# LuoweiZhou/VLP

Measured on AMD Instinct MI355X. Metric: samples/sec/node (COCO 100-region, seq64, bs64xN) fp16, higher is better.
Workload: dtype f16; 1 GPU; COCO Captions fine-tune shape: BERT-base 12L, 100 regions x 2048-d, seq_len 64 (L=167), bs 64/GPU, fwd+bwd+FP16 FusedAdam, dropout 0.1, dynamic loss scale; global_batch=64, parallelism=dp1, batch_pool=8, skipped_steps=0, rccl_ranks=1, optimizer=replicated, first_leg_packed=False

## Files before the change

include/vlp_hip.h:

```cpp
#ifndef VLP_HIP_H
#define VLP_HIP_H

#include <stdint.h>

#ifdef __cplusplus
extern "C" {
#endif

#define VLP_ABI_VERSION 5

typedef enum {
    VLP_OK = 0,
    VLP_ERR_BAD_ARG = -1,
    VLP_ERR_HIP = -2,
    VLP_ERR_WORKSPACE = -3
} vlp_status;

enum { VLP_ACT_NONE = 0, VLP_ACT_GELU = 1, VLP_ACT_RELU = 2, VLP_ACT_TANH = 3,
       VLP_ACT_GELU_SAVE_GRAD = 4  };
enum { VLP_MUL_NONE = 0, VLP_MUL_GELU_GRAD = 1, VLP_MUL_RELU_MASK = 2, VLP_MUL_PLAIN = 3  };

int vlp_version(void);
const char* vlp_last_error_string(void);
int vlp_lab_build(void);
void vlp_debug_device_lookup_stats(unsigned long long* lookups, unsigned long long* driver_queries);

typedef struct {
    const void* X; int64_t ldx;
    const void* W; int64_t ldw;
    void* Y; int64_t ldy;
    const void* bias;
    const void* residual; int64_t ldr;
    void* preact; int64_t ldp;
    const void* mul_src; int64_t ldm;
    int32_t M, N, K;
    int32_t act;
    int32_t mul_mode;
    float alpha;
    float dropout_p; uint64_t seed; uint32_t rng_stream;
    int32_t variant;
    const int32_t* row_map;
} vlp_gemm_nt_args;
int vlp_gemm_nt(const vlp_gemm_nt_args* a, void* stream);
int vlp_gemm_nt_resolved_variant(void);
int64_t vlp_gemm_nt_splitk_workspace_bytes(int32_t M, int32_t N, int32_t splits);
int vlp_gemm_nt_splitk(const vlp_gemm_nt_args* a, int32_t splits, void* workspace, int64_t workspace_bytes, void* stream);

typedef struct {
    const void* A; int64_t lda;
    const void* B; int64_t ldb;
    void* C; int64_t ldc;
    int32_t M, N, K;
    int32_t beta;
    void* workspace; int64_t workspace_bytes;
    int32_t variant;
    int32_t splits;
    void* bias_out;
} vlp_gemm_tn_args;
int64_t vlp_gemm_tn_workspace_bytes(int32_t M, int32_t N, int32_t K);
int vlp_gemm_tn(const vlp_gemm_tn_args* a, void* stream);
int vlp_gemm_tn_grouped(const vlp_gemm_tn_args* list, int32_t count, void* stream);
int64_t vlp_gemm_tn_grouped_workspace_bytes(int32_t tiles);

typedef struct {
    const void* A; int64_t lda; int32_t M, N;
    void* out;
    int32_t beta;
    void* workspace; int64_t workspace_bytes;
} vlp_colsum_args;
int64_t vlp_colsum_workspace_bytes(int32_t M, int32_t N);
int vlp_colsum(const vlp_colsum_args* a, void* stream);

typedef struct {
    const void* qkv; int64_t ld_qkv;
    const uint8_t* mask;
    void* ctx; int64_t ld_ctx;
    float* lse;
    int32_t B, L, heads;
    float scale;
    float dropout_p; uint64_t seed; uint32_t rng_stream;
    const int32_t* row_off;
} vlp_attn_fwd_args;
int vlp_attn_fwd(const vlp_attn_fwd_args* a, void* stream);

typedef struct {
    const void* q; int64_t ld_q; int64_t q_rows_per_batch;
    const void* k; const void* v; int64_t ld_kv; int64_t kv_rows_per_batch;
    const uint8_t* mask;
    void* ctx; int64_t ld_ctx;
    int32_t B, Lq, Lk, heads;
    float scale;
    const void* k_prefix; const void* v_prefix;
    int64_t prefix_rows_per_batch;
    int32_t n_prefix, beams;
} vlp_attn_decode_args;
int vlp_attn_decode(const vlp_attn_decode_args* a, void* stream);

typedef struct {
    const void* qkv; int64_t ld_qkv;
    const uint8_t* mask;
    const uint8_t* mask_t;
    const void* ctx; int64_t ld_ctx;
    const void* dctx; int64_t ld_dctx;
    const float* lse;
    void* dqkv; int64_t ld_dqkv;
    float* delta;
    int32_t B, L, heads;
    float scale;
    float dropout_p; uint64_t seed; uint32_t rng_stream;
    const int32_t* row_off;
} vlp_attn_bwd_args;
int vlp_attn_bwd(const vlp_attn_bwd_args* a, void* stream);

int vlp_mask_pack(const int64_t* mask, uint8_t* out, uint8_t* out_t, int32_t B, int32_t L, int32_t Lp, void* stream);

typedef struct {
    const void* x; int64_t ldx;
    const void* gamma; const void* beta;
    void* y; int64_t ldy;
    float* mean; float* rstd;
    int32_t M, H; float eps;
    float dropout_p; uint64_t seed; uint32_t rng_stream;
    const int32_t* row_map;
} vlp_layernorm_fwd_args;
int vlp_layernorm_fwd(const vlp_layernorm_fwd_args* a, void* stream);

typedef struct {
    const void* dy; int64_t lddy;
    const void* x; int64_t ldx;
    const void* gamma;
    const float* mean; const float* rstd;
    void* dx; int64_t lddx;
    void* dx_drop; int64_t lddxd;
    void* dgamma; void* dbeta;
    int32_t M, H; int32_t beta;
    float dy_drop_p; uint64_t dy_seed; uint32_t dy_stream;
    float out_drop_p; uint64_t out_seed; uint32_t out_stream;
    void* workspace; int64_t workspace_bytes;
    int32_t defer_reduce;
    const int32_t* row_map;
} vlp_layernorm_bwd_args;
int64_t vlp_layernorm_bwd_workspace_bytes(int32_t H);
int vlp_layernorm_bwd(const vlp_layernorm_bwd_args* a, void* stream);
int vlp_layernorm_bwd_reduce_batched(const float* parts, const void* const* dst, int32_t count, int32_t M, int32_t H, int32_t beta, void* stream);

int vlp_region_mask_build(const int64_t* vis_masked_pos, int32_t B, int32_t Pm, int32_t Nv, uint8_t* out, void* stream);
typedef struct {
    const void* vis_h; const void* vispe_h;
    const void* pooled;
    const int64_t* vis_masked_pos;
    float* probs;
    float* sample_loss;
    float* loss;
    int32_t B, Nv, Pm, H;
} vlp_pretext_fwd_args;
int vlp_pretext_fwd(const vlp_pretext_fwd_args* a, void* stream);
typedef struct {
    const void* vis_h; const void* vispe_h; const void* pooled;
    const int64_t* vis_masked_pos;
    const float* probs;
    const float* gscale;
    void* d_vis_h; void* d_vispe_h;
    void* d_pooled_pre;
    int32_t B, Nv, Pm, H;
    float drop_p; uint64_t seed; uint32_t vis_stream; uint32_t vispe_stream;
} vlp_pretext_bwd_args;
int vlp_pretext_bwd(const vlp_pretext_bwd_args* a, void* stream);

typedef struct {
    const int64_t* input_ids; const int64_t* segment_ids;
    const void* word_emb; const void* pos_emb; const void* type_emb;
    const void* vis_h; const void* vispe_h;
    void* pre;
    int32_t B, L, Nv, H, vocab, type_vocab;
    const int64_t* position_ids;
    int32_t max_pos;
    const uint8_t* region_mask;
    const int32_t* row_map; int32_t rows;
} vlp_embed_fwd_args;
int vlp_embed_fwd(const vlp_embed_fwd_args* a, void* stream);

int64_t vlp_embed_bwd_workspace_floats(int32_t B, int32_t L, int32_t Nv, int32_t H);
typedef struct {
    const void* dpre;
    const int64_t* input_ids; const int64_t* segment_ids;
    const void* vis_h; const void* vispe_h;
    void* d_word_emb; void* d_pos_emb; void* d_type_emb;
    void* d_vis_h; void* d_vispe_h;
    float* acc32;
    int32_t B, L, Nv, H, vocab, type_vocab;
    float drop_p; uint64_t seed; uint32_t vis_stream; uint32_t vispe_stream;
    const uint8_t* region_mask;
    int32_t parts;
} vlp_embed_bwd_args;
int vlp_embed_bwd(const vlp_embed_bwd_args* a, void* stream);
typedef struct {
    vlp_embed_bwd_args base;
    const int64_t* position_ids;
    int32_t max_pos;
} vlp_embed_bwd_pos_args;
int vlp_embed_bwd_pos(const vlp_embed_bwd_pos_args* a, void* stream);

int vlp_copy2d(const void* src, int64_t lds, int32_t src_f32, void* dst, int64_t ldd, int32_t rows,
               int32_t cols_src, int32_t cols_dst, int32_t beta, void* stream);
int vlp_transpose(const void* src, int64_t lds, void* dst, int64_t ldd, int32_t rows, int32_t cols,
                  int32_t rows_pad, void* stream);
typedef struct {
    const void* src; void* dst;
    int64_t lds, ldd;
    int32_t rows, cols, rows_pad, reserved;
} vlp_transpose_desc;
int vlp_transpose_batched(const vlp_transpose_desc* descs_dev, const int32_t* tile_start_dev, int32_t n, int32_t total_tiles, void* stream);
int vlp_gather_rows(const void* src, int64_t lds, const int64_t* pos, void* out, int64_t ldo,
                    int32_t B, int32_t P, int32_t L, int32_t H, const int32_t* row_off, void* stream);
int vlp_scatter_add_rows(const void* src, int64_t lds, const int64_t* pos, void* dst, int64_t ldd,
                         int32_t B, int32_t P, int32_t L, int32_t H, const int32_t* row_off, void* stream);
int vlp_rowmap_build(const int32_t* row_off, int32_t B, int32_t L, int32_t* row_map, void* stream);
int vlp_rows_unpack(const void* src, int64_t lds, const int32_t* row_map, int32_t rows, void* dst, int64_t ldd, int32_t H, void* stream);
int vlp_rows_pack(const void* src, int64_t lds, const int32_t* row_map, int32_t rows, void* dst, int64_t ldd, int32_t H, void* stream);
int vlp_mask_pack_rect(const int64_t* mask, int64_t batch_stride, int64_t row_stride, uint8_t* out, int32_t B, int32_t Lq, int32_t Lk,
                       int32_t Lkp, void* stream);
int vlp_kv_append(const void* qkv_new, int64_t ld, void* cache, int32_t Lcap, int32_t B, int32_t T, int32_t start, int32_t H, void* stream);
int vlp_argmax_rows(const void* logits, int64_t ld, int32_t rows, int32_t V, int64_t* ids, int64_t ids_stride, float* vals, int64_t vals_stride,
                    void* stream);
typedef struct {
    const void* X; int64_t ldx;
    const void* W; int64_t ldw;
    const void* bias;
    void* Y; int64_t ldy;
    float* slab; int64_t ldslab;
    void* kv_cache; int64_t kv_ld;
    int32_t kv_col0, kv_Lcap, kv_T, kv_start;
    int32_t M, N, K, splits;
    int32_t act;
    const void* residual; int64_t ldr;
    const void* ln_gamma; const void* ln_beta; float ln_eps;
    void* ln_out; int64_t ld_ln_out;
} vlp_dec_gemm_args;
int vlp_dec_gemm(const vlp_dec_gemm_args* a, void* stream);
typedef struct {
    const float* slab; int64_t ldslab; int32_t splits;
    const void* bias;
    const void* residual; int64_t ldr;
    const void* gamma; const void* beta;
    float eps;
    void* Y; int64_t ldy;
    int32_t M, H;
} vlp_dec_reduce_ln_args;
int vlp_dec_reduce_ln(const vlp_dec_reduce_ln_args* a, void* stream);
int vlp_argmax_rows2(const void* logits, int64_t ld, int32_t rows, int32_t V, int64_t* ids_a, int64_t ids_a_stride, int64_t* ids_b, int64_t ids_b_stride,
                     float* vals, int64_t vals_stride, void* stream);
int vlp_mask_build(const int32_t* second_st, const int32_t* second_end, const int32_t* is_s2s, uint8_t* out, uint8_t* out_t, int32_t B, int32_t L,
                   int32_t Lp, const uint8_t* region_mask, int32_t Nv, void* stream);
typedef struct {
    const float* bbox;
    const void* cls;
    int64_t ld_cls;
    void* out;
    int64_t ld_out;
    int32_t B, Nv, n_cls, pad_to, cls_is_f32;
    float eps;
} vlp_vis_pe_prep_args;
int vlp_vis_pe_prep(const vlp_vis_pe_prep_args* a, void* stream);
int vlp_sample_rows(const void* logits, int64_t ld, int32_t rows, int32_t V, uint64_t seed, uint32_t rng_stream, int64_t* ids,
                    int64_t ids_stride, float* logp, int64_t logp_stride, void* stream);
typedef struct {
    const int64_t* prefix_ids; const int64_t* sample_ids;
    const int64_t* segment_ids; const int64_t* position_ids; const int64_t* mask;
    int64_t* out_ids; int64_t* out_segment_ids; int64_t* out_position_ids; int64_t* out_mask; int64_t* masked_pos;
    int32_t B, L, in_len, T;
    int64_t mask_word_id;
} vlp_scst_layout_args;
int vlp_scst_layout(const vlp_scst_layout_args* a, void* stream);
int vlp_logsoftmax_topk(const void* logits, int64_t ld, int32_t rows, int32_t V, int32_t K, const uint8_t* forbid, int32_t eos_id,
                        int32_t block_eos, float* out_scores, int64_t* out_ids, void* stream);
typedef struct {
    const float* kk_scores;
    const int64_t* kk_ids;
    const float* last_total;
    const float* last_eos;
    float* out_scores;
    int64_t* out_ids;
    int64_t* out_ptrs;
    float* out_eos;
    int64_t* src_rows;
    int64_t* next_ids;
    int64_t next_ids_stride;
    int32_t B, K, first;
    int64_t eos_id;
} vlp_beam_select_args;
int vlp_beam_select(const vlp_beam_select_args* a, void* stream);
int vlp_ngram_candidates(const int64_t* wids, const int64_t* ptrs, int32_t B, int32_t K, int32_t s, int32_t ngram_size, const int64_t* ignore_ids,
                         int32_t n_ignore, int32_t* cand_ids, int64_t cand_ld, int32_t* cand_cnt, void* stream);
int vlp_logsoftmax_topk_list(const void* logits, int64_t ld, int32_t rows, int32_t V, int32_t K, const int32_t* cand_ids, int64_t cand_ld,
                             const int32_t* cand_cnt, int32_t eos_id, int32_t block_eos, float* out_scores, int64_t* out_ids, void* stream);
int vlp_kv_gather(const void* src, int64_t src_rows_per_batch, void* dst, int64_t dst_rows_per_batch, const int64_t* idx, int32_t R, int32_t lo,
                  int32_t hi, int32_t row_elems, void* stream);
int vlp_vqa_mul_fwd(const void* h, void* out, int32_t B, int32_t L, int32_t Nv, int32_t H, const int32_t* row_off, void* stream);
int vlp_vqa_mul_bwd(const void* h, const void* dout, void* dh, int32_t B, int32_t L, int32_t Nv, int32_t H, const int32_t* row_off, void* stream);
int vlp_relu_dropout_bwd(const void* dy, const void* y, void* dz, int64_t n, int64_t ncols, float drop_p,
                         uint64_t seed, uint32_t rng_stream, void* stream);

int vlp_gelu_bwd(const void* dy, const void* z, void* dz, int64_t n, void* stream);

typedef struct {
    const void* logits; int64_t ld_logits;
    const int64_t* labels;
    const int64_t* weights;
    float* loss;
    float* lse; float* coef;
    float* row_loss;
    int32_t B, P, V;
    float drop_worst_ratio;
} vlp_mlm_loss_fwd_args;
int vlp_mlm_loss_fwd(const vlp_mlm_loss_fwd_args* a, void* stream);
typedef struct {
    const void* logits; int64_t ld_logits;
    const int64_t* labels;
    const float* lse; const float* coef;
    const float* grad_scale;
    void* dlogits; int64_t ld_dlogits;
    int32_t rows, V;
} vlp_mlm_loss_bwd_args;
int vlp_mlm_loss_bwd(const vlp_mlm_loss_bwd_args* a, void* stream);

typedef struct {
    const void* logits; int64_t ld_logits;
    const int64_t* labels;
    const int64_t* weights;
    float* loss;
    float* lse; float* coef;
    float* row_loss;
    int32_t B, P, V;
    float drop_worst_ratio;
    float smooth, confidence, q_sum, q_log_q;
    int32_t ignore_index;
} vlp_mlm_loss_ls_fwd_args;
int vlp_mlm_loss_ls_fwd(const vlp_mlm_loss_ls_fwd_args* a, void* stream);
typedef struct {
    const void* logits; int64_t ld_logits;
    const int64_t* labels;
    const float* lse; const float* coef;
    const float* grad_scale;
    void* dlogits; int64_t ld_dlogits;
    int32_t rows, V;
    float smooth, confidence, q_sum;
    int32_t ignore_index;
} vlp_mlm_loss_ls_bwd_args;
int vlp_mlm_loss_ls_bwd(const vlp_mlm_loss_ls_bwd_args* a, void* stream);

typedef struct {
    const void* logits; int64_t ld_logits;
    const int64_t* ids;
    float* logp; float* lse;
    int32_t rows, V;
} vlp_token_logprob_fwd_args;
int vlp_token_logprob_fwd(const vlp_token_logprob_fwd_args* a, void* stream);
typedef struct {
    const void* logits; int64_t ld_logits;
    const int64_t* ids;
    const float* lse;
    const float* g;
    void* dlogits; int64_t ld_dlogits;
    int32_t rows, V;
} vlp_token_logprob_bwd_args;
int vlp_token_logprob_bwd(const vlp_token_logprob_bwd_args* a, void* stream);

typedef struct {
    const int64_t* hyp; int64_t hyp_ld;
    const int64_t* ref; int64_t ref_group_stride, ref_ld;
    const int32_t* ref_count;
    int32_t G, R, T, mult;
    float sigma;
    float* scores;
    float* reward;
    void* workspace; int64_t workspace_bytes;
} vlp_cider_d_args;
int64_t vlp_cider_d_workspace_bytes(int32_t G, int32_t R, int32_t T, int32_t mult);
int vlp_cider_d(const vlp_cider_d_args* a, void* stream);

typedef struct {
    vlp_cider_d_args s;
    const uint64_t* df_keys;
    const int32_t* df_vals;
    int64_t df_n;
    int64_t n_docs;
} vlp_cider_d_df_args;
int64_t vlp_cider_d_df_workspace_bytes(int32_t G, int32_t R, int32_t T, int32_t mult);
int vlp_cider_d_df(const vlp_cider_d_df_args* a, void* stream);

int vlp_bce_loss_fwd(const void* logits, int64_t ld, const void* labels_f32, int64_t ldl, int32_t B, int32_t N,
                     float* loss, void* stream);
int vlp_bce_loss_bwd(const void* logits, int64_t ld, const void* labels_f32, int64_t ldl, int32_t B, int32_t N,
                     const float* grad_scale, void* dlogits, int64_t ldd, void* stream);
int vlp_bce_sparse_loss_fwd(const void* logits, int64_t ld, const int32_t* ans_idx, const float* ans_score, int32_t S, int32_t B, int32_t N,
                            float* loss, void* stream);
int vlp_bce_sparse_loss_bwd(const void* logits, int64_t ld, const int32_t* ans_idx, const float* ans_score, int32_t S, int32_t B, int32_t N,
                            const float* grad_scale, void* dlogits, int64_t ldd, void* stream);
int vlp_vqa_answer_rows(const void* logits, int64_t ld, int32_t rows, int32_t N, int32_t first_col, const int32_t* ans_idx,
                        const float* ans_score, int32_t S, int64_t* out_ids, float* out_vals, float* out_scores, void* stream);

int vlp_sumsq(const void* g_f16, int64_t n, float* out2, float* partial, void* stream);
int vlp_sumsq_acc(const void* g_f16, int64_t n, float* out2, float* partial, void* stream);

typedef struct {
    float* p32; float* m; float* v;
    const void* g16;
    void* p16;
    int64_t n;
    float b1, b2, eps, decay;
    int32_t eps_inside_sqrt;
    const float* hyper;
} vlp_fused_adam_args;
int vlp_fused_adam(const vlp_fused_adam_args* a, void* stream);
int vlp_adam_hyper(const float* sumsq2, const float* any_overflow, const float* scale_state, float max_grad_norm,
                   float step_size, float* hyper3, void* stream);
int vlp_loss_scale_update(float* scale_state, const float* overflow, void* stream);

int64_t vlp_bert_adam_norms_floats(int64_t n, int32_t ntensors);
typedef struct {
    float* p32; float* m; float* v;
    const void* g; int32_t g_is_f32;
    void* p16;
    const int64_t* seg_off; int32_t ntensors; int64_t n;
    float* norms; int64_t norms_floats;
    float lr, b1, b2, eps, decay, max_grad_norm;
    float grad_scale;
    const int32_t* active;
} vlp_bert_adam_args;
int vlp_bert_adam(const vlp_bert_adam_args* a, void* stream);

#ifdef __cplusplus
}
#endif
#endif
```

vlp_amd/_lib.py:

```python
import ctypes as C
import os

import torch

_HERE = os.path.dirname(os.path.abspath(__file__))
LIB_PATH = os.environ.get("VLP_HIP_LIB") or os.path.join(_HERE, "libvlp_hip.so")

ACT_NONE, ACT_GELU, ACT_RELU, ACT_TANH, ACT_GELU_SAVE_GRAD = 0, 1, 2, 3, 4
MUL_NONE, MUL_GELU_GRAD, MUL_RELU_MASK, MUL_PLAIN = 0, 1, 2, 3

vp, i64, i32, f32, u64, u32 = C.c_void_p, C.c_int64, C.c_int32, C.c_float, C.c_uint64, C.c_uint32


class GemmNtArgs(C.Structure):
    _fields_ = [("X", vp), ("ldx", i64), ("W", vp), ("ldw", i64), ("Y", vp), ("ldy", i64), ("bias", vp),
                ("residual", vp), ("ldr", i64), ("preact", vp), ("ldp", i64), ("mul_src", vp), ("ldm", i64),
                ("M", i32), ("N", i32), ("K", i32), ("act", i32), ("mul_mode", i32), ("alpha", f32),
                ("dropout_p", f32), ("seed", u64), ("rng_stream", u32), ("variant", i32), ("row_map", vp)]


class GemmTnArgs(C.Structure):
    _fields_ = [("A", vp), ("lda", i64), ("B", vp), ("ldb", i64), ("C", vp), ("ldc", i64),
                ("M", i32), ("N", i32), ("K", i32), ("beta", i32), ("workspace", vp), ("workspace_bytes", i64),
                ("variant", i32), ("splits", i32), ("bias_out", vp)]


class ColsumArgs(C.Structure):
    _fields_ = [("A", vp), ("lda", i64), ("M", i32), ("N", i32), ("out", vp), ("beta", i32),
                ("workspace", vp), ("workspace_bytes", i64)]


class AttnFwdArgs(C.Structure):
    _fields_ = [("qkv", vp), ("ld_qkv", i64), ("mask", vp), ("ctx", vp), ("ld_ctx", i64), ("lse", vp),
                ("B", i32), ("L", i32), ("heads", i32), ("scale", f32),
                ("dropout_p", f32), ("seed", u64), ("rng_stream", u32), ("row_off", vp)]


class AttnBwdArgs(C.Structure):
    _fields_ = [("qkv", vp), ("ld_qkv", i64), ("mask", vp), ("mask_t", vp), ("ctx", vp), ("ld_ctx", i64), ("dctx", vp), ("ld_dctx", i64),
                ("lse", vp), ("dqkv", vp), ("ld_dqkv", i64), ("delta", vp),
                ("B", i32), ("L", i32), ("heads", i32), ("scale", f32),
                ("dropout_p", f32), ("seed", u64), ("rng_stream", u32), ("row_off", vp)]


class LayerNormFwdArgs(C.Structure):
    _fields_ = [("x", vp), ("ldx", i64), ("gamma", vp), ("beta", vp), ("y", vp), ("ldy", i64), ("mean", vp), ("rstd", vp),
                ("M", i32), ("H", i32), ("eps", f32), ("dropout_p", f32), ("seed", u64), ("rng_stream", u32), ("row_map", vp)]


class LayerNormBwdArgs(C.Structure):
    _fields_ = [("dy", vp), ("lddy", i64), ("x", vp), ("ldx", i64), ("gamma", vp), ("mean", vp), ("rstd", vp),
                ("dx", vp), ("lddx", i64), ("dx_drop", vp), ("lddxd", i64), ("dgamma", vp), ("dbeta", vp),
                ("M", i32), ("H", i32), ("beta", i32),
                ("dy_drop_p", f32), ("dy_seed", u64), ("dy_stream", u32),
                ("out_drop_p", f32), ("out_seed", u64), ("out_stream", u32),
                ("workspace", vp), ("workspace_bytes", i64), ("defer_reduce", i32), ("row_map", vp)]


class EmbedFwdArgs(C.Structure):
    _fields_ = [("input_ids", vp), ("segment_ids", vp), ("word_emb", vp), ("pos_emb", vp), ("type_emb", vp),
                ("vis_h", vp), ("vispe_h", vp), ("pre", vp),
                ("B", i32), ("L", i32), ("Nv", i32), ("H", i32), ("vocab", i32), ("type_vocab", i32),
                ("position_ids", vp), ("max_pos", i32), ("region_mask", vp), ("row_map", vp), ("rows", i32)]


class AttnDecodeArgs(C.Structure):
    _fields_ = [("q", vp), ("ld_q", i64), ("q_rows_per_batch", i64), ("k", vp), ("v", vp), ("ld_kv", i64), ("kv_rows_per_batch", i64),
                ("mask", vp), ("ctx", vp), ("ld_ctx", i64), ("B", i32), ("Lq", i32), ("Lk", i32), ("heads", i32), ("scale", f32),
                ("k_prefix", vp), ("v_prefix", vp), ("prefix_rows_per_batch", i64), ("n_prefix", i32), ("beams", i32)]


class DecGemmArgs(C.Structure):
    _fields_ = [("X", vp), ("ldx", i64), ("W", vp), ("ldw", i64), ("bias", vp), ("Y", vp), ("ldy", i64), ("slab", vp), ("ldslab", i64),
                ("kv_cache", vp), ("kv_ld", i64), ("kv_col0", i32), ("kv_Lcap", i32), ("kv_T", i32), ("kv_start", i32),
                ("M", i32), ("N", i32), ("K", i32), ("splits", i32), ("act", i32),
                ("residual", vp), ("ldr", i64), ("ln_gamma", vp), ("ln_beta", vp), ("ln_eps", f32), ("ln_out", vp), ("ld_ln_out", i64)]


class DecReduceLnArgs(C.Structure):
    _fields_ = [("slab", vp), ("ldslab", i64), ("splits", i32), ("bias", vp), ("residual", vp), ("ldr", i64), ("gamma", vp), ("beta", vp),
                ("eps", f32), ("Y", vp), ("ldy", i64), ("M", i32), ("H", i32)]


class VisPePrepArgs(C.Structure):
    _fields_ = [("bbox", vp), ("cls", vp), ("ld_cls", i64), ("out", vp), ("ld_out", i64), ("B", i32), ("Nv", i32), ("n_cls", i32),
                ("pad_to", i32), ("cls_is_f32", i32), ("eps", f32)]


class BeamSelectArgs(C.Structure):
    _fields_ = [("kk_scores", vp), ("kk_ids", vp), ("last_total", vp), ("last_eos", vp), ("out_scores", vp), ("out_ids", vp),
                ("out_ptrs", vp), ("out_eos", vp), ("src_rows", vp), ("next_ids", vp), ("next_ids_stride", i64),
                ("B", i32), ("K", i32), ("first", i32), ("eos_id", i64)]


class EmbedBwdArgs(C.Structure):
    _fields_ = [("dpre", vp), ("input_ids", vp), ("segment_ids", vp), ("vis_h", vp), ("vispe_h", vp),
                ("d_word_emb", vp), ("d_pos_emb", vp), ("d_type_emb", vp), ("d_vis_h", vp), ("d_vispe_h", vp), ("acc32", vp),
                ("B", i32), ("L", i32), ("Nv", i32), ("H", i32), ("vocab", i32), ("type_vocab", i32),
                ("drop_p", f32), ("seed", u64), ("vis_stream", u32), ("vispe_stream", u32), ("region_mask", vp), ("parts", i32)]


class EmbedBwdPosArgs(C.Structure):
    _fields_ = [("base", EmbedBwdArgs), ("position_ids", vp), ("max_pos", i32)]


class ScstLayoutArgs(C.Structure):
    _fields_ = [("prefix_ids", vp), ("sample_ids", vp), ("segment_ids", vp), ("position_ids", vp), ("mask", vp),
                ("out_ids", vp), ("out_segment_ids", vp), ("out_position_ids", vp), ("out_mask", vp), ("masked_pos", vp),
                ("B", i32), ("L", i32), ("in_len", i32), ("T", i32), ("mask_word_id", i64)]


class TokenLogprobFwdArgs(C.Structure):
    _fields_ = [("logits", vp), ("ld_logits", i64), ("ids", vp), ("logp", vp), ("lse", vp), ("rows", i32), ("V", i32)]


class TokenLogprobBwdArgs(C.Structure):
    _fields_ = [("logits", vp), ("ld_logits", i64), ("ids", vp), ("lse", vp), ("g", vp), ("dlogits", vp), ("ld_dlogits", i64),
                ("rows", i32), ("V", i32)]


class PretextFwdArgs(C.Structure):
    _fields_ = [("vis_h", vp), ("vispe_h", vp), ("pooled", vp), ("vis_masked_pos", vp), ("probs", vp), ("sample_loss", vp), ("loss", vp),
                ("B", i32), ("Nv", i32), ("Pm", i32), ("H", i32)]


class PretextBwdArgs(C.Structure):
    _fields_ = [("vis_h", vp), ("vispe_h", vp), ("pooled", vp), ("vis_masked_pos", vp), ("probs", vp), ("gscale", vp),
                ("d_vis_h", vp), ("d_vispe_h", vp), ("d_pooled_pre", vp), ("B", i32), ("Nv", i32), ("Pm", i32), ("H", i32),
                ("drop_p", f32), ("seed", u64), ("vis_stream", u32), ("vispe_stream", u32)]


class TransposeDesc(C.Structure):
    _fields_ = [("src", vp), ("dst", vp), ("lds", i64), ("ldd", i64), ("rows", i32), ("cols", i32), ("rows_pad", i32), ("reserved", i32)]


class CiderDArgs(C.Structure):
    _fields_ = [("hyp", vp), ("hyp_ld", i64), ("ref", vp), ("ref_group_stride", i64), ("ref_ld", i64), ("ref_count", vp),
                ("G", i32), ("R", i32), ("T", i32), ("mult", i32), ("sigma", f32), ("scores", vp), ("reward", vp),
                ("workspace", vp), ("workspace_bytes", i64)]


class CiderDDfArgs(C.Structure):
    _fields_ = [("s", CiderDArgs), ("df_keys", vp), ("df_vals", vp), ("df_n", i64), ("n_docs", i64)]


class MlmLossFwdArgs(C.Structure):
    _fields_ = [("logits", vp), ("ld_logits", i64), ("labels", vp), ("weights", vp), ("loss", vp), ("lse", vp), ("coef", vp),
                ("row_loss", vp), ("B", i32), ("P", i32), ("V", i32), ("drop_worst_ratio", f32)]


class MlmLossBwdArgs(C.Structure):
    _fields_ = [("logits", vp), ("ld_logits", i64), ("labels", vp), ("lse", vp), ("coef", vp), ("grad_scale", vp),
                ("dlogits", vp), ("ld_dlogits", i64), ("rows", i32), ("V", i32)]


class MlmLossLsFwdArgs(C.Structure):
    _fields_ = MlmLossFwdArgs._fields_ + [("smooth", f32), ("confidence", f32), ("q_sum", f32), ("q_log_q", f32), ("ignore_index", i32)]


class MlmLossLsBwdArgs(C.Structure):
    _fields_ = MlmLossBwdArgs._fields_ + [("smooth", f32), ("confidence", f32), ("q_sum", f32), ("ignore_index", i32)]


class FusedAdamArgs(C.Structure):
    _fields_ = [("p32", vp), ("m", vp), ("v", vp), ("g16", vp), ("p16", vp), ("n", i64),
                ("b1", f32), ("b2", f32), ("eps", f32), ("decay", f32), ("eps_inside_sqrt", i32), ("hyper", vp)]


class BertAdamArgs(C.Structure):
    _fields_ = [("p32", vp), ("m", vp), ("v", vp), ("g", vp), ("g_is_f32", i32), ("p16", vp),
                ("seg_off", vp), ("ntensors", i32), ("n", i64), ("norms", vp), ("norms_floats", i64),
                ("lr", f32), ("b1", f32), ("b2", f32), ("eps", f32), ("decay", f32), ("max_grad_norm", f32), ("grad_scale", f32),
                ("active", vp)]


SYMBOLS = {
    "vlp_version": (C.c_int, []),
    "vlp_last_error_string": (C.c_char_p, []),
    "vlp_lab_build": (C.c_int, []),
    "vlp_debug_device_lookup_stats": (None, [vp, vp]),
    "vlp_gemm_nt": (C.c_int, [C.POINTER(GemmNtArgs), vp]),
    "vlp_gemm_nt_resolved_variant": (C.c_int, []),
    "vlp_gemm_nt_splitk_workspace_bytes": (C.c_int64, [i32, i32, i32]),
    "vlp_gemm_nt_splitk": (C.c_int, [C.POINTER(GemmNtArgs), i32, vp, i64, vp]),
    "vlp_gemm_tn_workspace_bytes": (i64, [i32, i32, i32]),
    "vlp_gemm_tn": (C.c_int, [C.POINTER(GemmTnArgs), vp]),
    "vlp_gemm_tn_grouped": (C.c_int, [C.POINTER(GemmTnArgs), i32, vp]),
    "vlp_gemm_tn_grouped_workspace_bytes": (i64, [i32]),
    "vlp_colsum_workspace_bytes": (i64, [i32, i32]),
    "vlp_colsum": (C.c_int, [C.POINTER(ColsumArgs), vp]),
    "vlp_attn_fwd": (C.c_int, [C.POINTER(AttnFwdArgs), vp]),
    "vlp_attn_bwd": (C.c_int, [C.POINTER(AttnBwdArgs), vp]),
    "vlp_attn_decode": (C.c_int, [C.POINTER(AttnDecodeArgs), vp]),
    "vlp_mask_pack_rect": (C.c_int, [vp, i64, i64, vp, i32, i32, i32, i32, vp]),
    "vlp_kv_append": (C.c_int, [vp, i64, vp, i32, i32, i32, i32, i32, vp]),
    "vlp_dec_gemm": (C.c_int, [C.POINTER(DecGemmArgs), vp]),
    "vlp_dec_reduce_ln": (C.c_int, [C.POINTER(DecReduceLnArgs), vp]),
    "vlp_argmax_rows2": (C.c_int, [vp, i64, i32, i32, vp, i64, vp, i64, vp, i64, vp]),
    "vlp_logsoftmax_topk": (C.c_int, [vp, i64, i32, i32, i32, vp, i32, i32, vp, vp, vp]),
    "vlp_beam_select": (C.c_int, [C.POINTER(BeamSelectArgs), vp]),
    "vlp_ngram_candidates": (C.c_int, [vp, vp, i32, i32, i32, i32, vp, i32, vp, i64, vp, vp]),
    "vlp_logsoftmax_topk_list": (C.c_int, [vp, i64, i32, i32, i32, vp, i64, vp, i32, i32, vp, vp, vp]),
    "vlp_kv_gather": (C.c_int, [vp, i64, vp, i64, vp, i32, i32, i32, i32, vp]),
    "vlp_embed_bwd_workspace_floats": (C.c_int64, [i32, i32, i32, i32]),
    "vlp_mask_build": (C.c_int, [vp, vp, vp, vp, vp, i32, i32, i32, vp, i32, vp]),
    "vlp_vis_pe_prep": (C.c_int, [C.POINTER(VisPePrepArgs), vp]),
    "vlp_sample_rows": (C.c_int, [vp, i64, i32, i32, C.c_uint64, C.c_uint32, vp, i64, vp, i64, vp]),
    "vlp_argmax_rows": (C.c_int, [vp, i64, i32, i32, vp, i64, vp, i64, vp]),
    "vlp_mask_pack": (C.c_int, [vp, vp, vp, i32, i32, i32, vp]),
    "vlp_layernorm_fwd": (C.c_int, [C.POINTER(LayerNormFwdArgs), vp]),
    "vlp_layernorm_bwd_workspace_bytes": (i64, [i32]),
    "vlp_layernorm_bwd": (C.c_int, [C.POINTER(LayerNormBwdArgs), vp]),
    "vlp_layernorm_bwd_reduce_batched": (C.c_int, [vp, vp, i32, i32, i32, i32, vp]),
    "vlp_embed_fwd": (C.c_int, [C.POINTER(EmbedFwdArgs), vp]),
    "vlp_embed_bwd": (C.c_int, [C.POINTER(EmbedBwdArgs), vp]),
    "vlp_embed_bwd_pos": (C.c_int, [C.POINTER(EmbedBwdPosArgs), vp]),
    "vlp_scst_layout": (C.c_int, [C.POINTER(ScstLayoutArgs), vp]),
    "vlp_token_logprob_fwd": (C.c_int, [C.POINTER(TokenLogprobFwdArgs), vp]),
    "vlp_token_logprob_bwd": (C.c_int, [C.POINTER(TokenLogprobBwdArgs), vp]),
    "vlp_region_mask_build": (C.c_int, [vp, i32, i32, i32, vp, vp]),
    "vlp_pretext_fwd": (C.c_int, [C.POINTER(PretextFwdArgs), vp]),
    "vlp_pretext_bwd": (C.c_int, [C.POINTER(PretextBwdArgs), vp]),
    "vlp_copy2d": (C.c_int, [vp, i64, i32, vp, i64, i32, i32, i32, i32, vp]),
    "vlp_transpose": (C.c_int, [vp, i64, vp, i64, i32, i32, i32, vp]),
    "vlp_transpose_batched": (C.c_int, [vp, vp, i32, i32, vp]),
    "vlp_gather_rows": (C.c_int, [vp, i64, vp, vp, i64, i32, i32, i32, i32, vp, vp]),
    "vlp_scatter_add_rows": (C.c_int, [vp, i64, vp, vp, i64, i32, i32, i32, i32, vp, vp]),
    "vlp_rowmap_build": (C.c_int, [vp, i32, i32, vp, vp]),
    "vlp_rows_unpack": (C.c_int, [vp, i64, vp, i32, vp, i64, i32, vp]),
    "vlp_rows_pack": (C.c_int, [vp, i64, vp, i32, vp, i64, i32, vp]),
    "vlp_vqa_mul_fwd": (C.c_int, [vp, vp, i32, i32, i32, i32, vp, vp]),
    "vlp_vqa_mul_bwd": (C.c_int, [vp, vp, vp, i32, i32, i32, i32, vp, vp]),
    "vlp_relu_dropout_bwd": (C.c_int, [vp, vp, vp, i64, i64, f32, u64, u32, vp]),
    "vlp_gelu_bwd": (C.c_int, [vp, vp, vp, i64, vp]),
    "vlp_cider_d_workspace_bytes": (i64, [i32, i32, i32, i32]),
    "vlp_cider_d": (C.c_int, [C.POINTER(CiderDArgs), vp]),
    "vlp_cider_d_df_workspace_bytes": (i64, [i32, i32, i32, i32]),
    "vlp_cider_d_df": (C.c_int, [C.POINTER(CiderDDfArgs), vp]),
    "vlp_mlm_loss_fwd": (C.c_int, [C.POINTER(MlmLossFwdArgs), vp]),
    "vlp_mlm_loss_bwd": (C.c_int, [C.POINTER(MlmLossBwdArgs), vp]),
    "vlp_mlm_loss_ls_fwd": (C.c_int, [C.POINTER(MlmLossLsFwdArgs), vp]),
    "vlp_mlm_loss_ls_bwd": (C.c_int, [C.POINTER(MlmLossLsBwdArgs), vp]),
    "vlp_bce_loss_fwd": (C.c_int, [vp, i64, vp, i64, i32, i32, vp, vp]),
    "vlp_bce_loss_bwd": (C.c_int, [vp, i64, vp, i64, i32, i32, vp, vp, i64, vp]),
    "vlp_bce_sparse_loss_fwd": (C.c_int, [vp, i64, vp, vp, i32, i32, i32, vp, vp]),
    "vlp_bce_sparse_loss_bwd": (C.c_int, [vp, i64, vp, vp, i32, i32, i32, vp, vp, i64, vp]),
    "vlp_vqa_answer_rows": (C.c_int, [vp, i64, i32, i32, i32, vp, vp, i32, vp, vp, vp, vp]),
    "vlp_sumsq": (C.c_int, [vp, i64, vp, vp, vp]),
    "vlp_sumsq_acc": (C.c_int, [vp, i64, vp, vp, vp]),
    "vlp_fused_adam": (C.c_int, [C.POINTER(FusedAdamArgs), vp]),
    "vlp_adam_hyper": (C.c_int, [vp, vp, vp, f32, f32, vp, vp]),
    "vlp_loss_scale_update": (C.c_int, [vp, vp, vp]),
    "vlp_bert_adam": (C.c_int, [C.POINTER(BertAdamArgs), vp]),
    "vlp_bert_adam_norms_floats": (i64, [i64, i32]),
}

_lib = None


_recording = None


class _Recorder(object):

    def __init__(self, lib, plan):
        self._lib, self._plan = lib, plan

    def __getattr__(self, name):
        fn = getattr(self._lib, name)

        def call(*args):
            self._plan.append((fn, args))
            return fn(*args)
        return call


class record(object):

    def __enter__(self):
        global _recording
        if _recording is not None:
            raise RuntimeError("vlp_amd._lib.record(): already recording")
        self.plan = []
        _recording = _Recorder(load(), self.plan)
        return self.plan

    def __exit__(self, *exc):
        global _recording
        _recording = None
        return False


def replay(plan):
    for fn, args in plan:
        rc = fn(*args)
        if rc:
            _check(rc)


def load():
    global _lib
    if _recording is not None:
        return _recording
    if _lib is not None:
        return _lib
    if not os.path.exists(LIB_PATH):
        raise RuntimeError("libvlp_hip.so not found at %s -- run `python -m vlp_amd.build` (or "
                           "__graft_entry__.build()).  vlp_amd has no CPU / torch fallback." % LIB_PATH)
    lib = C.CDLL(LIB_PATH)
    for name, (res, args) in SYMBOLS.items():
        fn = getattr(lib, name)
        fn.restype = res
        fn.argtypes = args
    if lib.vlp_version() != 5:
        raise RuntimeError("libvlp_hip.so ABI version mismatch")
    _lib = lib
    return lib


def lab_build():
    return bool(load().vlp_lab_build())


def _check(rc):
    if rc != 0:
        lib = _lib if _lib is not None else load()
        raise RuntimeError("libvlp_hip: %s (status %d)" % (lib.vlp_last_error_string().decode(), rc))


def stream_ptr():
    return C.c_void_p(torch.cuda.current_stream().cuda_stream)


def ptr(t):
    return None if t is None else C.c_void_p(t.data_ptr())


def _nbytes(t):
    return 0 if t is None else t.numel() * t.element_size()


def _req_cuda(*ts):
    for t in ts:
        if t is not None and not t.is_cuda:
            raise RuntimeError("vlp_amd kernels need device tensors (got a CPU tensor); there is no CPU fallback")


def _gemm_nt_args(x, w, y, M, N, K, ldx, ldw, ldy, bias, residual, ldr, preact, ldp, mul_src, ldm, act, mul_mode, alpha, dropout_p, seed, rng_stream,
                  variant=0, row_map=None):
    return GemmNtArgs(ptr(x), ldx if ldx is not None else x.stride(0), ptr(w), ldw if ldw is not None else w.stride(0),
                      ptr(y), ldy if ldy is not None else y.stride(0), ptr(bias),
                      ptr(residual), (ldr if ldr is not None else (residual.stride(0) if residual is not None else 0)),
                      ptr(preact), (ldp if ldp is not None else (preact.stride(0) if preact is not None else 0)),
                      ptr(mul_src), (ldm if ldm is not None else (mul_src.stride(0) if mul_src is not None else 0)),
                      M, N, K, act, mul_mode, alpha, dropout_p, seed, rng_stream, variant, ptr(row_map))


def gemm_nt(x, w, y, M, N, K, ldx=None, ldw=None, ldy=None, bias=None, residual=None, ldr=None, preact=None, ldp=None,
            mul_src=None, ldm=None, act=ACT_NONE, mul_mode=MUL_NONE, alpha=1.0, dropout_p=0.0, seed=0, rng_stream=0,
            variant=0, row_map=None):
    _req_cuda(x, w, y, row_map)
    a = _gemm_nt_args(x, w, y, M, N, K, ldx, ldw, ldy, bias, residual, ldr, preact, ldp, mul_src, ldm, act, mul_mode, alpha, dropout_p, seed,
                      rng_stream, variant, row_map)
    _check(load().vlp_gemm_nt(C.byref(a), stream_ptr()))


def gemm_nt_resolved_variant():
    return int(load().vlp_gemm_nt_resolved_variant())


def gemm_nt_splitk_workspace_bytes(M, N, splits):
    return int(load().vlp_gemm_nt_splitk_workspace_bytes(M, N, splits))


def gemm_nt_splitk(x, w, y, M, N, K, splits, workspace, ldx=None, ldw=None, ldy=None, bias=None, residual=None, ldr=None, preact=None, ldp=None,
                   mul_src=None, ldm=None, act=ACT_NONE, mul_mode=MUL_NONE, alpha=1.0, dropout_p=0.0, seed=0, rng_stream=0):
    _req_cuda(x, w, y, workspace)
    a = _gemm_nt_args(x, w, y, M, N, K, ldx, ldw, ldy, bias, residual, ldr, preact, ldp, mul_src, ldm, act, mul_mode, alpha, dropout_p, seed,
                      rng_stream)
    _check(load().vlp_gemm_nt_splitk(C.byref(a), splits, ptr(workspace), _nbytes(workspace), stream_ptr()))


def gemm_tn_workspace_bytes(M, N, K):
    return int(load().vlp_gemm_tn_workspace_bytes(M, N, K))


def gemm_tn(a_, b_, c_, M, N, K, lda=None, ldb=None, ldc=None, beta=0, workspace=None, variant=0, splits=0, bias_out=None):
    _req_cuda(a_, b_, c_)
    a = GemmTnArgs(ptr(a_), lda if lda is not None else a_.stride(0), ptr(b_), ldb if ldb is not None else b_.stride(0),
                   ptr(c_), ldc if ldc is not None else c_.stride(0), M, N, K, beta,
                   ptr(workspace), _nbytes(workspace), variant, splits,
                   ptr(bias_out))
    _check(load().vlp_gemm_tn(C.byref(a), stream_ptr()))


def gemm_tn_grouped_workspace_bytes(tiles):
    return int(load().vlp_gemm_tn_grouped_workspace_bytes(tiles))


def gemm_tn_grouped(problems, workspace=None):
    arr = (GemmTnArgs * len(problems))()
    for i, (a_, b_, c_, M, N, K, beta, bias_out) in enumerate(problems):
        _req_cuda(a_, b_, c_, bias_out)
        w = workspace if i == 0 else None
        if w is not None:
            _req_cuda(w)
        arr[i] = GemmTnArgs(ptr(a_), a_.stride(0), ptr(b_), b_.stride(0), ptr(c_), c_.stride(0), M, N, K, beta, ptr(w),
                            _nbytes(w), 0, 0, ptr(bias_out))
    _check(load().vlp_gemm_tn_grouped(arr, len(problems), stream_ptr()))


def colsum_workspace_bytes(M, N):
    return int(load().vlp_colsum_workspace_bytes(M, N))


def colsum(a_, out, M, N, lda=None, beta=0, workspace=None):
    _req_cuda(a_, out)
    a = ColsumArgs(ptr(a_), lda if lda is not None else a_.stride(0), M, N, ptr(out), beta, ptr(workspace),
                   _nbytes(workspace))
    _check(load().vlp_colsum(C.byref(a), stream_ptr()))


def attn_fwd(qkv, mask, ctx, lse, B, L, heads, scale, dropout_p=0.0, seed=0, rng_stream=0, row_off=None):
    _req_cuda(qkv, mask, ctx, lse, row_off)
    a = AttnFwdArgs(ptr(qkv), qkv.stride(0), ptr(mask), ptr(ctx), ctx.stride(0), ptr(lse), B, L, heads, scale, dropout_p, seed, rng_stream,
                    ptr(row_off))
    _check(load().vlp_attn_fwd(C.byref(a), stream_ptr()))


def attn_bwd(qkv, mask, mask_t, ctx, dctx, lse, dqkv, delta, B, L, heads, scale, dropout_p=0.0, seed=0, rng_stream=0, row_off=None):
    _req_cuda(qkv, mask, mask_t, ctx, dctx, lse, dqkv, delta, row_off)
    a = AttnBwdArgs(ptr(qkv), qkv.stride(0), ptr(mask), ptr(mask_t), ptr(ctx), ctx.stride(0), ptr(dctx), dctx.stride(0), ptr(lse),
                    ptr(dqkv), dqkv.stride(0), ptr(delta), B, L, heads, scale, dropout_p, seed, rng_stream, ptr(row_off))
    _check(load().vlp_attn_bwd(C.byref(a), stream_ptr()))


def attn_decode(q, ld_q, q_rows, k, v, ld_kv, kv_rows, mask, ctx, B, Lq, Lk, heads, scale, k_prefix=None, v_prefix=None, prefix_rows=0,
                n_prefix=0, beams=1):
    _req_cuda(q, k, v, mask, ctx, k_prefix, v_prefix)
    a = AttnDecodeArgs(ptr(q), ld_q, q_rows, ptr(k), ptr(v), ld_kv, kv_rows, ptr(mask), ptr(ctx), ctx.stride(0), B, Lq, Lk, heads, scale,
                       ptr(k_prefix), ptr(v_prefix), prefix_rows, n_prefix, beams)
    _check(load().vlp_attn_decode(C.byref(a), stream_ptr()))


def dec_gemm(x, w, M, N, Kd, y=None, bias=None, act=0, slab=None, splits=1, kv_cache=None, kv_col0=0, kv_Lcap=0, kv_T=1, kv_start=0,
             residual=None, ln_gamma=None, ln_beta=None, ln_eps=1e-5, ln_out=None):
    _req_cuda(x, w, y, bias, slab, kv_cache, residual, ln_gamma, ln_beta, ln_out)
    a = DecGemmArgs(ptr(x), x.stride(0), ptr(w), w.stride(0), ptr(bias), ptr(y), y.stride(0) if y is not None else 0,
                    ptr(slab), slab.stride(1) if slab is not None else 0, ptr(kv_cache), kv_cache.stride(1) if kv_cache is not None else 0,
                    kv_col0, kv_Lcap, kv_T, kv_start, M, N, Kd, splits, act,
                    ptr(residual), residual.stride(0) if residual is not None else 0, ptr(ln_gamma), ptr(ln_beta), ln_eps,
                    ptr(ln_out), ln_out.stride(0) if ln_out is not None else 0)
    _check(load().vlp_dec_gemm(C.byref(a), stream_ptr()))


def dec_reduce_ln(slab, splits, bias, residual, gamma, beta, y, M, H, eps=1e-5):
    _req_cuda(slab, bias, residual, gamma, beta, y)
    a = DecReduceLnArgs(ptr(slab), slab.stride(1), splits, ptr(bias), ptr(residual), residual.stride(0) if residual is not None else 0,
                        ptr(gamma), ptr(beta), eps, ptr(y), y.stride(0), M, H)
    _check(load().vlp_dec_reduce_ln(C.byref(a), stream_ptr()))


def argmax_rows2(logits, ld, rows, V, ids_a, ids_b, vals):
    _req_cuda(logits, ids_a, ids_b, vals)
    _check(load().vlp_argmax_rows2(ptr(logits), ld, rows, V, ptr(ids_a), ids_a.stride(0), ptr(ids_b), ids_b.stride(0) if ids_b is not None else 0,
                                   ptr(vals), vals.stride(0), stream_ptr()))


def mask_pack_rect(mask_view, out_u8, B, Lq, Lk, Lkp):
    _req_cuda(mask_view, out_u8)
    assert mask_view.stride(2) == 1 and mask_view.dtype == torch.int64
    _check(load().vlp_mask_pack_rect(ptr(mask_view), mask_view.stride(0), mask_view.stride(1), ptr(out_u8), B, Lq, Lk, Lkp, stream_ptr()))


def kv_append(qkv_new, ld, cache, Lcap, B, T, start, H):
    _req_cuda(qkv_new, cache)
    _check(load().vlp_kv_append(ptr(qkv_new), ld, ptr(cache), Lcap, B, T, start, H, stream_ptr()))


def argmax_rows(logits, ld, rows, V, ids, vals):
    _req_cuda(logits, ids, vals)
    _check(load().vlp_argmax_rows(ptr(logits), ld, rows, V, ptr(ids), ids.stride(0), ptr(vals), vals.stride(0), stream_ptr()))


def logsoftmax_topk(logits, ld, rows, V, K, out_scores, out_ids, forbid=None, eos_id=0, block_eos=False):
    _req_cuda(logits, out_scores, out_ids, forbid)
    _check(load().vlp_logsoftmax_topk(ptr(logits), ld, rows, V, K, ptr(forbid), eos_id, 1 if block_eos else 0, ptr(out_scores), ptr(out_ids),
                                      stream_ptr()))


def ngram_candidates(wids, ptrs, B, K, s, ngram_size, cand_ids, cand_cnt, ignore_ids=None):
    _req_cuda(wids, ptrs, cand_ids, cand_cnt, ignore_ids)
    assert wids.dtype == torch.int64 and ptrs.dtype == torch.int64 and wids.is_contiguous() and ptrs.is_contiguous()
    assert tuple(wids.shape[1:]) == (B, K) and tuple(ptrs.shape[1:]) == (B, K) and s < wids.shape[0] and s < ptrs.shape[0]
    assert cand_ids.dtype == torch.int32 and cand_cnt.dtype == torch.int32 and cand_ids.stride(1) == 1 and cand_cnt.is_contiguous()
    assert cand_ids.shape[0] >= B * K and cand_cnt.numel() >= B * K
    n_ignore = 0
    if ignore_ids is not None:
        assert ignore_ids.dtype == torch.int64 and ignore_ids.is_contiguous()
        n_ignore = ignore_ids.numel()
    _check(load().vlp_ngram_candidates(ptr(wids), ptr(ptrs), B, K, s, ngram_size, ptr(ignore_ids) if n_ignore else None, n_ignore, ptr(cand_ids),
                                       cand_ids.stride(0), ptr(cand_cnt), stream_ptr()))


def logsoftmax_topk_list(logits, ld, rows, V, K, out_scores, out_ids, cand_ids, cand_cnt, eos_id=0, block_eos=False):
    _req_cuda(logits, out_scores, out_ids, cand_ids, cand_cnt)
    assert cand_ids.dtype == torch.int32 and cand_cnt.dtype == torch.int32 and cand_ids.stride(1) == 1 and cand_cnt.is_contiguous()
    assert cand_ids.shape[0] >= rows and cand_cnt.numel() >= rows
    _check(load().vlp_logsoftmax_topk_list(ptr(logits), ld, rows, V, K, ptr(cand_ids), cand_ids.stride(0), ptr(cand_cnt), eos_id, 1 if block_eos else 0,
                                           ptr(out_scores), ptr(out_ids), stream_ptr()))


def beam_select(kk_scores, kk_ids, last_total, last_eos, out_scores, out_ids, out_ptrs, out_eos, src_rows, next_ids, B, K, first, eos_id):
    _req_cuda(kk_scores, kk_ids, last_total, last_eos, out_scores, out_ids, out_ptrs, out_eos, src_rows, next_ids)
    a = BeamSelectArgs(ptr(kk_scores), ptr(kk_ids), ptr(last_total), ptr(last_eos), ptr(out_scores), ptr(out_ids), ptr(out_ptrs), ptr(out_eos),
                       ptr(src_rows), ptr(next_ids), next_ids.stride(0), B, K, 1 if first else 0, eos_id)
    _check(load().vlp_beam_select(C.byref(a), stream_ptr()))


def kv_gather(src, src_rows, dst, dst_rows, idx, R, lo, hi, row_elems):
    _req_cuda(src, dst, idx)
    _check(load().vlp_kv_gather(ptr(src), src_rows, ptr(dst), dst_rows, ptr(idx), R, lo, hi, row_elems, stream_ptr()))


def mask_build(second_st, second_end, is_s2s, out_u8, B, L, Lp, out_t=None, region_mask=None, Nv=0):
    _req_cuda(second_st, second_end, is_s2s, out_u8, out_t, region_mask)
    for t in (second_st, second_end, is_s2s):
        assert t.dtype == torch.int32 and t.is_contiguous() and t.numel() == B
    _check(load().vlp_mask_build(ptr(second_st), ptr(second_end), ptr(is_s2s), ptr(out_u8), ptr(out_t), B, L, Lp, ptr(region_mask), Nv, stream_ptr()))


def vis_pe_prep(bbox, cls, out, B, Nv, n_cls, pad_to, eps=1e-5):
    _req_cuda(bbox, cls, out)
    assert bbox.dtype == torch.float32 and bbox.is_contiguous() and cls.dtype in (torch.float16, torch.float32) and cls.stride(-1) == 1
    a = VisPePrepArgs(ptr(bbox), ptr(cls), cls.stride(0), ptr(out), out.stride(0), B, Nv, n_cls, pad_to, 1 if cls.dtype == torch.float32 else 0, eps)
    _check(load().vlp_vis_pe_prep(C.byref(a), stream_ptr()))


def sample_rows(logits, ld, rows, V, seed, rng_stream, ids, logp):
    _req_cuda(logits, ids, logp)
    _check(load().vlp_sample_rows(ptr(logits), ld, rows, V, seed, rng_stream, ptr(ids), ids.stride(0), ptr(logp), logp.stride(0), stream_ptr()))


def mask_pack(mask_i64, out_u8, B, L, Lp, out_t=None):
    _req_cuda(mask_i64, out_u8, out_t)
    _check(load().vlp_mask_pack(ptr(mask_i64), ptr(out_u8), ptr(out_t), B, L, Lp, stream_ptr()))


def layernorm_fwd(x, gamma, beta, y, M, H, mean=None, rstd=None, eps=1e-5, dropout_p=0.0, seed=0, rng_stream=0, ldx=None, ldy=None, row_map=None):
    _req_cuda(x, gamma, beta, y, row_map)
    a = LayerNormFwdArgs(ptr(x), ldx if ldx is not None else x.stride(0), ptr(gamma), ptr(beta), ptr(y),
                         ldy if ldy is not None else y.stride(0), ptr(mean), ptr(rstd), M, H, eps, dropout_p, seed, rng_stream, ptr(row_map))
    _check(load().vlp_layernorm_fwd(C.byref(a), stream_ptr()))


def layernorm_bwd_workspace_bytes(H):
    return int(load().vlp_layernorm_bwd_workspace_bytes(H))


def layernorm_bwd(dy, x, gamma, mean, rstd, dx, dgamma, dbeta, M, H, workspace, beta=0, dx_drop=None,
                  dy_drop=(0.0, 0, 0), out_drop=(0.0, 0, 0), defer_reduce=False, row_map=None):
    _req_cuda(dy, x, gamma, mean, rstd, dx, dgamma, dbeta, workspace, row_map)
    a = LayerNormBwdArgs(ptr(dy), dy.stride(0), ptr(x), x.stride(0), ptr(gamma), ptr(mean), ptr(rstd), ptr(dx), dx.stride(0),
                         ptr(dx_drop), dx_drop.stride(0) if dx_drop is not None else 0, ptr(dgamma), ptr(dbeta), M, H, beta,
                         dy_drop[0], dy_drop[1], dy_drop[2], out_drop[0], out_drop[1], out_drop[2],
                         ptr(workspace), _nbytes(workspace), 1 if defer_reduce else 0, ptr(row_map))
    _check(load().vlp_layernorm_bwd(C.byref(a), stream_ptr()))


def layernorm_bwd_reduce_batched(parts, dst_table, count, M, H, beta=0):
    _req_cuda(parts, dst_table)
    _check(load().vlp_layernorm_bwd_reduce_batched(ptr(parts), ptr(dst_table), count, M, H, beta, stream_ptr()))


def embed_fwd(input_ids, segment_ids, word_emb, pos_emb, type_emb, vis_h, vispe_h, pre, B, L, Nv, H, position_ids=None, region_mask=None,
              row_map=None, rows=0):
    _req_cuda(input_ids, segment_ids, word_emb, pos_emb, type_emb, pre, position_ids, region_mask, row_map)
    a = EmbedFwdArgs(ptr(input_ids), ptr(segment_ids), ptr(word_emb), ptr(pos_emb), ptr(type_emb), ptr(vis_h), ptr(vispe_h),
                     ptr(pre), B, L, Nv, H, word_emb.shape[0], type_emb.shape[0], ptr(position_ids), pos_emb.shape[0], ptr(region_mask),
                     ptr(row_map), rows)
    _check(load().vlp_embed_fwd(C.byref(a), stream_ptr()))


def embed_bwd_workspace_floats(B, L, Nv, H):
    return int(load().vlp_embed_bwd_workspace_floats(B, L, Nv, H))


def _embed_bwd_args(dpre, input_ids, segment_ids, vis_h, vispe_h, d_word, d_pos, d_type, d_vis_h, d_vispe_h, acc32,
                    B, L, Nv, H, vocab, type_vocab, drop_p, seed, vis_stream, vispe_stream, region_mask, parts):
    _req_cuda(dpre, input_ids, segment_ids, d_word, d_pos, d_type, acc32, region_mask)
    return EmbedBwdArgs(ptr(dpre), ptr(input_ids), ptr(segment_ids), ptr(vis_h), ptr(vispe_h), ptr(d_word), ptr(d_pos), ptr(d_type),
                        ptr(d_vis_h), ptr(d_vispe_h), ptr(acc32), B, L, Nv, H, vocab, type_vocab, drop_p, seed, vis_stream, vispe_stream,
                        ptr(region_mask), parts)


def embed_bwd(dpre, input_ids, segment_ids, vis_h, vispe_h, d_word, d_pos, d_type, d_vis_h, d_vispe_h, acc32,
              B, L, Nv, H, vocab, type_vocab, drop_p=0.0, seed=0, vis_stream=0, vispe_stream=0, region_mask=None, parts=0):
    a = _embed_bwd_args(dpre, input_ids, segment_ids, vis_h, vispe_h, d_word, d_pos, d_type, d_vis_h, d_vispe_h, acc32,
                        B, L, Nv, H, vocab, type_vocab, drop_p, seed, vis_stream, vispe_stream, region_mask, parts)
    _check(load().vlp_embed_bwd(C.byref(a), stream_ptr()))


def embed_bwd_pos(dpre, input_ids, segment_ids, position_ids, vis_h, vispe_h, d_word, d_pos, d_type, d_vis_h, d_vispe_h, acc32,
                  B, L, Nv, H, vocab, type_vocab, drop_p=0.0, seed=0, vis_stream=0, vispe_stream=0, region_mask=None, parts=0):
    _req_cuda(position_ids)
    base = _embed_bwd_args(dpre, input_ids, segment_ids, vis_h, vispe_h, d_word, d_pos, d_type, d_vis_h, d_vispe_h, acc32,
                           B, L, Nv, H, vocab, type_vocab, drop_p, seed, vis_stream, vispe_stream, region_mask, parts)
    a = EmbedBwdPosArgs(base, ptr(position_ids), d_pos.shape[0])
    _check(load().vlp_embed_bwd_pos(C.byref(a), stream_ptr()))


def scst_layout(prefix_ids, sample_ids, segment_ids, position_ids, mask, out_ids, out_segment_ids, out_position_ids, out_mask, masked_pos,
                mask_word_id):
    _req_cuda(prefix_ids, sample_ids, segment_ids, position_ids, mask, out_ids, out_segment_ids, out_position_ids, out_mask, masked_pos)
    B, in_len = prefix_ids.shape
    T, L = sample_ids.shape[1], segment_ids.shape[1]
    for t in (prefix_ids, sample_ids, segment_ids, position_ids, mask, out_ids, out_segment_ids, out_position_ids, out_mask, masked_pos):
        if t.dtype != torch.long or not t.is_contiguous():
            raise RuntimeError("vlp_amd.scst_layout: operands must be contiguous int64")
    Lo = in_len + 2 * T - 1
    if (tuple(sample_ids.shape) != (B, T) or tuple(position_ids.shape) != (B, L) or tuple(mask.shape) != (B, L, L) or
            tuple(out_ids.shape) != (B, Lo) or tuple(out_segment_ids.shape) != (B, Lo) or tuple(out_position_ids.shape) != (B, Lo) or
            tuple(out_mask.shape) != (B, Lo, Lo) or tuple(masked_pos.shape) != (B, T)):
        raise RuntimeError("vlp_amd.scst_layout: shape mismatch")
    a = ScstLayoutArgs(ptr(prefix_ids), ptr(sample_ids), ptr(segment_ids), ptr(position_ids), ptr(mask), ptr(out_ids), ptr(out_segment_ids),
                       ptr(out_position_ids), ptr(out_mask), ptr(masked_pos), B, L, in_len, T, int(mask_word_id))
    _check(load().vlp_scst_layout(C.byref(a), stream_ptr()))


def token_logprob_fwd(logits, ld, ids, logp, lse, rows, V):
    _req_cuda(logits, ids, logp, lse)
    a = TokenLogprobFwdArgs(ptr(logits), ld, ptr(ids), ptr(logp), ptr(lse), rows, V)
    _check(load().vlp_token_logprob_fwd(C.byref(a), stream_ptr()))


def token_logprob_bwd(logits, ld, ids, lse, g, dlogits, ldd, rows, V):
    _req_cuda(logits, ids, lse, g, dlogits)
    a = TokenLogprobBwdArgs(ptr(logits), ld, ptr(ids), ptr(lse), ptr(g), ptr(dlogits), ldd, rows, V)
    _check(load().vlp_token_logprob_bwd(C.byref(a), stream_ptr()))


def cider_d_workspace_bytes(G, R, T, mult):
    return int(load().vlp_cider_d_workspace_bytes(G, R, T, mult))


def cider_d(hyp, ref, ref_count, mult, scores, reward=None, sigma=6.0, workspace=None):
    a = _cider_d_args(hyp, ref, ref_count, mult, scores, reward, sigma, workspace, cider_d_workspace_bytes)
    _check(load().vlp_cider_d(C.byref(a), stream_ptr()))


def _cider_d_args(hyp, ref, ref_count, mult, scores, reward, sigma, workspace, workspace_bytes):
    _req_cuda(hyp, ref, ref_count, scores, reward, workspace)
    if hyp.dtype != torch.int64 or ref.dtype != torch.int64 or hyp.dim() != 2 or ref.dim() != 3 or hyp.stride(1) != 1 or ref.stride(2) != 1:
        raise RuntimeError("vlp_amd.cider_d: hyp int64 [mult*G, T] and ref int64 [G, R, T] with contiguous rows")
    G, R, T = ref.shape
    if hyp.shape[0] != mult * G or hyp.shape[1] != T:
        raise RuntimeError("vlp_amd.cider_d: hyp must be [%d, %d]" % (mult * G, T))
    if ref_count is not None and (ref_count.dtype != torch.int32 or not ref_count.is_contiguous() or ref_count.numel() != G):
        raise RuntimeError("vlp_amd.cider_d: ref_count must be contiguous int32 [%d]" % G)
    if scores.dtype != torch.float32 or not scores.is_contiguous() or scores.numel() < mult * G:
        raise RuntimeError("vlp_amd.cider_d: scores must be contiguous f32 [%d]" % (mult * G))
    if reward is not None and (reward.dtype != torch.float32 or not reward.is_contiguous() or reward.numel() < G):
        raise RuntimeError("vlp_amd.cider_d: reward must be contiguous f32 [%d]" % G)
    if workspace is None:
        workspace = torch.empty(max(workspace_bytes(G, R, T, mult), 1), device=hyp.device, dtype=torch.uint8)
    a = CiderDArgs(ptr(hyp), hyp.stride(0), ptr(ref), ref.stride(0), ref.stride(1), ptr(ref_count), G, R, T, mult, sigma, ptr(scores), ptr(reward),
                   ptr(workspace), _nbytes(workspace))
    a._keep = workspace
    return a


def cider_d_df_workspace_bytes(G, R, T, mult):
    return int(load().vlp_cider_d_df_workspace_bytes(G, R, T, mult))


def cider_d_df(hyp, ref, ref_count, mult, scores, df_keys, df_vals, n_docs, reward=None, sigma=6.0, workspace=None):
    _req_cuda(df_keys, df_vals)
    if (df_keys.dtype not in (torch.int64, torch.uint64) or df_vals.dtype != torch.int32 or df_keys.dim() != 1 or df_vals.dim() != 1
            or not df_keys.is_contiguous() or not df_vals.is_contiguous() or df_keys.numel() != df_vals.numel()):
        raise RuntimeError("vlp_amd.cider_d_df: df_keys int64 [N] (the uint64 keys' bits) and df_vals int32 [N], contiguous")
    s = _cider_d_args(hyp, ref, ref_count, mult, scores, reward, sigma, workspace, cider_d_df_workspace_bytes)
    n = df_keys.numel()
    a = CiderDDfArgs(s, ptr(df_keys) if n else None, ptr(df_vals) if n else None, n, int(n_docs))
    _check(load().vlp_cider_d_df(C.byref(a), stream_ptr()))


def region_mask_build(vis_masked_pos, out, B, Pm, Nv):
    _req_cuda(vis_masked_pos, out)
    _check(load().vlp_region_mask_build(ptr(vis_masked_pos), B, Pm, Nv, ptr(out), stream_ptr()))


def pretext_fwd(vis_h, vispe_h, pooled, vis_masked_pos, probs, sample_loss, loss, B, Nv, Pm, H):
    _req_cuda(vis_h, vispe_h, pooled, vis_masked_pos, probs, sample_loss, loss)
    a = PretextFwdArgs(ptr(vis_h), ptr(vispe_h), ptr(pooled), ptr(vis_masked_pos), ptr(probs), ptr(sample_loss), ptr(loss), B, Nv, Pm, H)
    _check(load().vlp_pretext_fwd(C.byref(a), stream_ptr()))


def pretext_bwd(vis_h, vispe_h, pooled, vis_masked_pos, probs, gscale, d_vis_h, d_vispe_h, d_pooled_pre, B, Nv, Pm, H,
                drop_p=0.0, seed=0, vis_stream=0, vispe_stream=0):
    _req_cuda(vis_h, vispe_h, pooled, vis_masked_pos, probs, gscale, d_vis_h, d_vispe_h, d_pooled_pre)
    a = PretextBwdArgs(ptr(vis_h), ptr(vispe_h), ptr(pooled), ptr(vis_masked_pos), ptr(probs), ptr(gscale), ptr(d_vis_h), ptr(d_vispe_h),
                       ptr(d_pooled_pre), B, Nv, Pm, H, drop_p, seed, vis_stream, vispe_stream)
    _check(load().vlp_pretext_bwd(C.byref(a), stream_ptr()))


def copy2d(src, lds, src_f32, dst, ldd, rows, cols_src, cols_dst, beta=0):
    _req_cuda(src, dst)
    _check(load().vlp_copy2d(ptr(src), lds, int(src_f32), ptr(dst), ldd, rows, cols_src, cols_dst, beta, stream_ptr()))


def transpose(src, lds, dst, ldd, rows, cols, rows_pad):
    _req_cuda(src, dst)
    _check(load().vlp_transpose(ptr(src), lds, ptr(dst), ldd, rows, cols, rows_pad, stream_ptr()))


def make_transpose_batch(items, device):
    import numpy as np
    arr = (TransposeDesc * len(items))()
    starts, tot = [], 0
    for i, (src, lds, dst, ldd, rows, cols, rows_pad) in enumerate(items):
        _req_cuda(src, dst)
        arr[i] = TransposeDesc(src.data_ptr(), dst.data_ptr(), lds, ldd, rows, cols, rows_pad, 0)
        starts.append(tot)
        tot += ((rows_pad + 63) // 64) * ((cols + 63) // 64)
    raw = np.frombuffer(bytes(arr), dtype=np.uint8).copy()
    descs = torch.from_numpy(raw).to(device)
    ts = torch.tensor(starts, dtype=torch.int32, device=device)
    return descs, ts, len(items), tot


def transpose_batched(batch):
    descs, ts, n, tot = batch
    _check(load().vlp_transpose_batched(ptr(descs), ptr(ts), n, tot, stream_ptr()))


def gather_rows(src, lds, pos, out, ldo, B, P, L, H, row_off=None):
    _req_cuda(src, pos, out, row_off)
    _check(load().vlp_gather_rows(ptr(src), lds, ptr(pos), ptr(out), ldo, B, P, L, H, ptr(row_off), stream_ptr()))


def scatter_add_rows(src, lds, pos, dst, ldd, B, P, L, H, row_off=None):
    _req_cuda(src, pos, dst, row_off)
    _check(load().vlp_scatter_add_rows(ptr(src), lds, ptr(pos), ptr(dst), ldd, B, P, L, H, ptr(row_off), stream_ptr()))


def rowmap_build(row_off, B, L, row_map):
    _req_cuda(row_off, row_map)
    _check(load().vlp_rowmap_build(ptr(row_off), B, L, ptr(row_map), stream_ptr()))


def rows_unpack(src, row_map, rows, dst, H):
    _req_cuda(src, row_map, dst)
    _check(load().vlp_rows_unpack(ptr(src), src.stride(0), ptr(row_map), rows, ptr(dst), dst.stride(0), H, stream_ptr()))


def rows_pack(src, row_map, rows, dst, H):
    _req_cuda(src, row_map, dst)
    _check(load().vlp_rows_pack(ptr(src), src.stride(0), ptr(row_map), rows, ptr(dst), dst.stride(0), H, stream_ptr()))


def vqa_mul_fwd(h, out, B, L, Nv, H, row_off=None):
    _req_cuda(h, out, row_off)
    _check(load().vlp_vqa_mul_fwd(ptr(h), ptr(out), B, L, Nv, H, ptr(row_off), stream_ptr()))


def vqa_mul_bwd(h, dout, dh, B, L, Nv, H, row_off=None):
    _req_cuda(h, dout, dh, row_off)
    _check(load().vlp_vqa_mul_bwd(ptr(h), ptr(dout), ptr(dh), B, L, Nv, H, ptr(row_off), stream_ptr()))


def relu_dropout_bwd(dy, y, dz, n, ncols, drop_p=0.0, seed=0, rng_stream=0):
    _req_cuda(dy, y, dz)
    _check(load().vlp_relu_dropout_bwd(ptr(dy), ptr(y), ptr(dz), n, ncols, drop_p, seed, rng_stream, stream_ptr()))


def gelu_bwd(dy, z, dz, n):
    _req_cuda(dy, z, dz)
    _check(load().vlp_gelu_bwd(ptr(dy), ptr(z), ptr(dz), n, stream_ptr()))


def mlm_loss_fwd(logits, ld, labels, weights, loss, lse, coef, row_loss, B, P, V, drop_worst_ratio=0.0):
    _req_cuda(logits, labels, weights, loss, lse, coef, row_loss)
    a = MlmLossFwdArgs(ptr(logits), ld, ptr(labels), ptr(weights), ptr(loss), ptr(lse), ptr(coef), ptr(row_loss), B, P, V, drop_worst_ratio)
    _check(load().vlp_mlm_loss_fwd(C.byref(a), stream_ptr()))


def mlm_loss_bwd(logits, ld, labels, lse, coef, grad_scale, dlogits, ldd, rows, V):
    _req_cuda(logits, labels, lse, coef, grad_scale, dlogits)
    a = MlmLossBwdArgs(ptr(logits), ld, ptr(labels), ptr(lse), ptr(coef), ptr(grad_scale), ptr(dlogits), ldd, rows, V)
    _check(load().vlp_mlm_loss_bwd(C.byref(a), stream_ptr()))


def mlm_loss_ls_fwd(logits, ld, labels, weights, loss, lse, coef, row_loss, B, P, V, smooth, confidence, q_sum, q_log_q, ignore_index=0,
                    drop_worst_ratio=0.0):
    _req_cuda(logits, labels, weights, loss, lse, coef, row_loss)
    a = MlmLossLsFwdArgs(ptr(logits), ld, ptr(labels), ptr(weights), ptr(loss), ptr(lse), ptr(coef), ptr(row_loss), B, P, V, drop_worst_ratio,
                         smooth, confidence, q_sum, q_log_q, ignore_index)
    _check(load().vlp_mlm_loss_ls_fwd(C.byref(a), stream_ptr()))


def mlm_loss_ls_bwd(logits, ld, labels, lse, coef, grad_scale, dlogits, ldd, rows, V, smooth, confidence, q_sum, ignore_index=0):
    _req_cuda(logits, labels, lse, coef, grad_scale, dlogits)
    a = MlmLossLsBwdArgs(ptr(logits), ld, ptr(labels), ptr(lse), ptr(coef), ptr(grad_scale), ptr(dlogits), ldd, rows, V,
                         smooth, confidence, q_sum, ignore_index)
    _check(load().vlp_mlm_loss_ls_bwd(C.byref(a), stream_ptr()))


def bce_loss_fwd(logits, ld, labels, ldl, B, N, loss257):
    _req_cuda(logits, labels, loss257)
    _check(load().vlp_bce_loss_fwd(ptr(logits), ld, ptr(labels), ldl, B, N, ptr(loss257), stream_ptr()))


def bce_loss_bwd(logits, ld, labels, ldl, B, N, grad_scale, dlogits, ldd):
    _req_cuda(logits, labels, grad_scale, dlogits)
    _check(load().vlp_bce_loss_bwd(ptr(logits), ld, ptr(labels), ldl, B, N, ptr(grad_scale), ptr(dlogits), ldd, stream_ptr()))


def _req_answers(ans_idx, ans_score, B):
    _req_cuda(ans_idx, ans_score)
    if ans_idx.dtype != torch.int32 or ans_score.dtype != torch.float32 or ans_idx.dim() != 2 or ans_idx.shape != ans_score.shape \
            or ans_idx.shape[0] != B or not (ans_idx.is_contiguous() and ans_score.is_contiguous()):
        raise RuntimeError("vlp_amd: sparse answers must be contiguous idx int32 / score f32 [%d, S]" % B)
    return ans_idx.shape[1]


def bce_sparse_loss_fwd(logits, ld, ans_idx, ans_score, B, N, loss257):
    _req_cuda(logits, loss257)
    S = _req_answers(ans_idx, ans_score, B)
    _check(load().vlp_bce_sparse_loss_fwd(ptr(logits), ld, ptr(ans_idx), ptr(ans_score), S, B, N, ptr(loss257), stream_ptr()))


def bce_sparse_loss_bwd(logits, ld, ans_idx, ans_score, B, N, grad_scale, dlogits, ldd):
    _req_cuda(logits, grad_scale, dlogits)
    S = _req_answers(ans_idx, ans_score, B)
    _check(load().vlp_bce_sparse_loss_bwd(ptr(logits), ld, ptr(ans_idx), ptr(ans_score), S, B, N, ptr(grad_scale), ptr(dlogits), ldd, stream_ptr()))


def vqa_answer_rows(logits, ld, rows, N, first_col, out_ids, out_vals, ans_idx=None, ans_score=None, out_scores=None):
    _req_cuda(logits, out_ids, out_vals)
    if out_ids.dtype != torch.int64 or out_vals.dtype != torch.float32 or out_ids.numel() < rows or out_vals.numel() < rows \
            or not (out_ids.is_contiguous() and out_vals.is_contiguous()):
        raise RuntimeError("vlp_amd: vqa_answer_rows needs contiguous out_ids int64 [rows] and out_vals f32 [rows]")
    S = 0
    if ans_idx is not None:
        S = _req_answers(ans_idx, ans_score, rows)
        _req_cuda(out_scores)
        if out_scores.dtype != torch.float32 or out_scores.numel() < rows or not out_scores.is_contiguous():
            raise RuntimeError("vlp_amd: vqa_answer_rows needs contiguous out_scores f32 [rows]")
    _check(load().vlp_vqa_answer_rows(ptr(logits), ld, rows, N, first_col, ptr(ans_idx), ptr(ans_score) if ans_idx is not None else None, S,
                                      ptr(out_ids), ptr(out_vals), ptr(out_scores) if ans_idx is not None else None, stream_ptr()))


def sumsq(g16, n, out2, partial, accumulate=False):
    _req_cuda(g16, out2, partial)
    fn = load().vlp_sumsq_acc if accumulate else load().vlp_sumsq
    _check(fn(ptr(g16), n, ptr(out2), ptr(partial), stream_ptr()))


def adam_hyper(sumsq2, any_overflow, scale_state, max_grad_norm, step_size, hyper3):
    _req_cuda(sumsq2, hyper3, scale_state)
    _check(load().vlp_adam_hyper(ptr(sumsq2), ptr(any_overflow), ptr(scale_state), max_grad_norm, step_size, ptr(hyper3), stream_ptr()))


def loss_scale_update(scale_state, overflow):
    _req_cuda(scale_state, overflow)
    _check(load().vlp_loss_scale_update(ptr(scale_state), ptr(overflow), stream_ptr()))


def fused_adam(p32, m, v, g16, p16, n, hyper, b1=0.9, b2=0.999, eps=1e-8, decay=0.0, eps_inside_sqrt=False):
    _req_cuda(p32, m, v, g16, p16, hyper)
    a = FusedAdamArgs(ptr(p32), ptr(m), ptr(v), ptr(g16), ptr(p16), n, b1, b2, eps, decay, int(eps_inside_sqrt), ptr(hyper))
    _check(load().vlp_fused_adam(C.byref(a), stream_ptr()))


def bert_adam_norms_floats(n, ntensors):
    return int(load().vlp_bert_adam_norms_floats(n, ntensors))


def bert_adam(p32, m, v, g, g_is_f32, p16, seg_off, ntensors, n, norms, lr, b1=0.9, b2=0.999, eps=1e-6, decay=0.01,
              max_grad_norm=1.0, grad_scale=1.0, active=None):
    _req_cuda(p32, m, v, g, seg_off, norms)
    a = BertAdamArgs(ptr(p32), ptr(m), ptr(v), ptr(g), int(g_is_f32), ptr(p16), ptr(seg_off), ntensors, n, ptr(norms), norms.numel(),
                     lr, b1, b2, eps, decay, max_grad_norm, grad_scale, ptr(active))
    _check(load().vlp_bert_adam(C.byref(a), stream_ptr()))
```

vlp_amd/csrc/adam.hip:

```cpp
#include "common.h"
#include <stdlib.h>

#define SQ_BLOCKS 1024

__global__ __launch_bounds__(256) void sumsq_kernel(const f16* __restrict__ g, int64_t n, float* __restrict__ partial) {
    __shared__ float sh[4], shb[4];
    float s = 0.f, bad = 0.f;
    const int64_t n8 = n >> 3;
    for (int64_t i = (int64_t)blockIdx.x * blockDim.x + threadIdx.x; i < n8; i += (int64_t)gridDim.x * blockDim.x) {
        f16x8 v = ld8(g + i * 8);
#pragma unroll
        for (int e = 0; e < 8; ++e) {
            const float f = (float)v[e];
            s += f * f;
            if (!(fabsf(f) <= 65504.f)) bad = 1.f;
        }
    }
    if (blockIdx.x == 0)
        for (int64_t i = n8 * 8 + threadIdx.x; i < n; i += blockDim.x) {
            const float f = (float)g[i];
            s += f * f;
            if (!(fabsf(f) <= 65504.f)) bad = 1.f;
        }
    s = wave_sum(s);
    bad = wave_max(bad);
    const int w = threadIdx.x >> 6, l = threadIdx.x & 63;
    if (l == 0) { sh[w] = s; shb[w] = bad; }
    __syncthreads();
    if (threadIdx.x == 0) {
        partial[blockIdx.x] = sh[0] + sh[1] + sh[2] + sh[3];
        partial[SQ_BLOCKS + blockIdx.x] = fmaxf(fmaxf(shb[0], shb[1]), fmaxf(shb[2], shb[3]));
    }
}
__global__ __launch_bounds__(256) void sumsq_finish_kernel(const float* __restrict__ partial, int nblocks, float* __restrict__ out2, int accumulate) {
    __shared__ float sh[4], shb[4];
    float s = 0.f, bad = 0.f;
    for (int i = threadIdx.x; i < nblocks; i += blockDim.x) { s += partial[i]; bad = fmaxf(bad, partial[SQ_BLOCKS + i]); }
    s = wave_sum(s);
    bad = wave_max(bad);
    const int w = threadIdx.x >> 6, l = threadIdx.x & 63;
    if (l == 0) { sh[w] = s; shb[w] = bad; }
    __syncthreads();
    if (threadIdx.x == 0) {
        const float tot = sh[0] + sh[1] + sh[2] + sh[3];
        float b = fmaxf(fmaxf(shb[0], shb[1]), fmaxf(shb[2], shb[3]));
        if (!(tot <= 3.0e38f)) b = 1.f;
        out2[0] = accumulate ? out2[0] + tot : tot;
        out2[1] = accumulate ? fmaxf(out2[1], b) : b;
    }
}
static int sumsq_launch(const void* g, int64_t n, float* out2, float* partial, int accumulate, void* stream);
extern "C" int vlp_sumsq(const void* g, int64_t n, float* out2, float* partial, void* stream) { return sumsq_launch(g, n, out2, partial, 0, stream); }
extern "C" int vlp_sumsq_acc(const void* g, int64_t n, float* out2, float* partial, void* stream) { return sumsq_launch(g, n, out2, partial, 1, stream); }
static int sumsq_launch(const void* g, int64_t n, float* out2, float* partial, int accumulate, void* stream) {
    VLP_CHECK_ARG(g && out2 && partial && n > 0 && (uintptr_t)g % 16 == 0, "vlp_sumsq: bad args (partial must hold 2048 floats)");
    VLP_ENTER(g, "vlp_sumsq");
    int blocks = (int)((n / 8 + 255) / 256);
    if (blocks > SQ_BLOCKS) blocks = SQ_BLOCKS;
    if (blocks < 1) blocks = 1;
    hipStream_t s = (hipStream_t)stream;
    hipLaunchKernelGGL(sumsq_kernel, dim3(blocks), dim3(256), 0, s, (const f16*)g, n, partial);
    VLP_CHECK_LAUNCH("vlp_sumsq");
    hipLaunchKernelGGL(sumsq_finish_kernel, dim3(1), dim3(256), 0, s, partial, blocks, out2, accumulate);
    VLP_CHECK_LAUNCH("vlp_sumsq(finish)");
    return VLP_OK;
}

__global__ void adam_hyper_kernel(const float* sumsq2, const float* any_overflow, const float* scale_state, float max_grad_norm, float step_size,
                                  float* hyper) {
    if (threadIdx.x != 0 || blockIdx.x != 0) return;
    const float scale = scale_state[0];
    float overflow = sumsq2[1];
    if (any_overflow) overflow = fmaxf(overflow, any_overflow[0]);
    const float norm = sqrtf(sumsq2[0]);
    float combined = scale;
    if (max_grad_norm > 0.f) {
        const float clip = (norm / scale + 1e-6f) / max_grad_norm;
        if (clip > 1.f) combined = clip * scale;
    }
    hyper[0] = combined;
    hyper[1] = step_size;
    hyper[2] = overflow;
}
extern "C" int vlp_adam_hyper(const float* sumsq2, const float* any_overflow, const float* scale_state, float max_grad_norm, float step_size,
                              float* hyper3, void* stream) {
    VLP_CHECK_ARG(sumsq2 && hyper3 && scale_state, "vlp_adam_hyper: bad args");
    VLP_ENTER(sumsq2, "vlp_adam_hyper");
    hipLaunchKernelGGL(adam_hyper_kernel, dim3(1), dim3(64), 0, (hipStream_t)stream, sumsq2, any_overflow, scale_state, max_grad_norm, step_size, hyper3);
    VLP_CHECK_LAUNCH("vlp_adam_hyper");
    return VLP_OK;
}

__global__ void loss_scale_update_kernel(float* st, const float* overflow) {
    if (threadIdx.x != 0 || blockIdx.x != 0) return;
    const bool skip = overflow[0] != 0.f;
    if (st[5] != 0.f) {
        if (skip) {
            st[0] = fmaxf(st[0] / st[3], 1.f);
            st[2] = st[1];
        } else if (fmodf(st[1] - st[2], st[4]) == 0.f) {
            st[0] = st[0] * st[3];
        }
    }
    if (skip) st[6] += 1.f;
    st[1] += 1.f;
}
extern "C" int vlp_loss_scale_update(float* scale_state, const float* overflow, void* stream) {
    VLP_CHECK_ARG(scale_state && overflow, "vlp_loss_scale_update: bad args");
    VLP_ENTER(scale_state, "vlp_loss_scale_update");
    hipLaunchKernelGGL(loss_scale_update_kernel, dim3(1), dim3(64), 0, (hipStream_t)stream, scale_state, overflow);
    VLP_CHECK_LAUNCH("vlp_loss_scale_update");
    return VLP_OK;
}

DEVFN f32x4 adam_ld4(const float* p) { return __builtin_nontemporal_load(reinterpret_cast<const f32x4*>(p)); }
DEVFN void adam_st4(float* p, f32x4 v) { __builtin_nontemporal_store(v, reinterpret_cast<f32x4*>(p)); }
__global__ __launch_bounds__(256) void fused_adam_kernel(vlp_fused_adam_args a) {
    const float combined = a.hyper[0], step_size = a.hyper[1], skip = a.hyper[2];
    if (skip != 0.f) return;
    const float inv = 1.f / combined;
    const f16* g = (const f16*)a.g16;
    f16* p16 = (f16*)a.p16;
    const int lane = threadIdx.x & 63;
    const int64_t wave = ((int64_t)blockIdx.x * blockDim.x + threadIdx.x) >> 6, nwaves = ((int64_t)gridDim.x * blockDim.x) >> 6;
    for (int64_t base = wave * 512; base < a.n; base += nwaves * 512) {
        f16x4 gv[2];
        f32x4 p0[2], m0[2], v0[2];
        bool ok[2];
#pragma unroll
        for (int h = 0; h < 2; ++h) {
            const int64_t i = base + 256 * h + 4 * lane;
            ok[h] = i < a.n;
            if (ok[h]) {
                gv[h] = __builtin_nontemporal_load(reinterpret_cast<const f16x4*>(g + i));
                p0[h] = adam_ld4(a.p32 + i);
                m0[h] = adam_ld4(a.m + i);
                v0[h] = adam_ld4(a.v + i);
            }
        }
#pragma unroll
        for (int h = 0; h < 2; ++h) {
            if (!ok[h]) continue;
            const int64_t i = base + 256 * h + 4 * lane;
            float pp[4], mm[4], vv[4];
#pragma unroll
            for (int e = 0; e < 4; ++e) { pp[e] = p0[h][e]; mm[e] = m0[h][e]; vv[e] = v0[h][e]; }
            f16x4 o;
#pragma unroll
            for (int e = 0; e < 4; ++e) {
                const float sg = (float)gv[h][e] * inv;
                mm[e] = a.b1 * mm[e] + (1.f - a.b1) * sg;
                vv[e] = a.b2 * vv[e] + (1.f - a.b2) * sg * sg;
                const float denom = a.eps_inside_sqrt ? sqrtf(vv[e] + a.eps) : sqrtf(vv[e]) + a.eps;
                pp[e] = pp[e] - step_size * (mm[e] / denom + a.decay * pp[e]);
                asm volatile("" : "+v"(pp[e]));
                o[e] = (f16)pp[e];
            }
            adam_st4(a.p32 + i, (f32x4){pp[0], pp[1], pp[2], pp[3]});
            adam_st4(a.m + i, (f32x4){mm[0], mm[1], mm[2], mm[3]});
            adam_st4(a.v + i, (f32x4){vv[0], vv[1], vv[2], vv[3]});
            st4(p16 + i, o);
        }
    }
}
extern "C" int vlp_fused_adam(const vlp_fused_adam_args* a, void* stream) {
    VLP_CHECK_ARG(a && a->p32 && a->m && a->v && a->g16 && a->p16 && a->hyper, "vlp_fused_adam: null operand");
    VLP_ENTER(a->p32, "vlp_fused_adam");
    VLP_CHECK_ARG(a->n > 0 && a->n % 8 == 0, "vlp_fused_adam: n must be a positive multiple of 8 (pad the flat buffer)");
    VLP_CHECK_ARG(((uintptr_t)a->p32 | (uintptr_t)a->m | (uintptr_t)a->v | (uintptr_t)a->g16 | (uintptr_t)a->p16) % 16 == 0, "vlp_fused_adam: alignment");
    static const int ncu = [] { int dev = 0, n = 256; (void)hipGetDevice(&dev); if (hipDeviceGetAttribute(&n, hipDeviceAttributeMultiprocessorCount, dev) != hipSuccess) n = 256; return n; }();
    int blocks = (int)((a->n / 8 + 255) / 256);
    if (blocks > 2 * ncu) blocks = 2 * ncu;
    hipLaunchKernelGGL(fused_adam_kernel, dim3(blocks), dim3(256), 0, (hipStream_t)stream, *a);
    VLP_CHECK_LAUNCH("vlp_fused_adam");
    return VLP_OK;
}

#define BA_CHUNK 4096

DEVFN float ba_load(const void* g, int g_is_f32, int64_t i) { return g_is_f32 ? ((const float*)g)[i] : (float)((const f16*)g)[i]; }

DEVFN int ba_find(const int64_t* seg_off, int nt, int64_t i) {
    int lo = 0, hi = nt - 1;
    while (lo < hi) {
        const int mid = (lo + hi + 1) >> 1;
        if (seg_off[mid] <= i) lo = mid; else hi = mid - 1;
    }
    return lo;
}

__global__ __launch_bounds__(256) void bert_adam_norm_kernel(vlp_bert_adam_args a) {
    __shared__ float sh[4];
    const int64_t start = (int64_t)blockIdx.x * BA_CHUNK;
    const int64_t end = min(a.n, start + BA_CHUNK);
    int t = ba_find(a.seg_off, a.ntensors, start);
    int64_t pos = start;
    while (pos < end) {
        if (t >= a.ntensors) break;
        const int64_t tend = min(end, a.seg_off[t + 1]);
        if (a.active && !a.active[t]) { pos = tend; ++t; continue; }
        float s = 0.f;
        for (int64_t i = pos + threadIdx.x; i < tend; i += blockDim.x) {
            const float f = ba_load(a.g, a.g_is_f32, i) / a.grad_scale;
            s += f * f;
        }
        s = wave_sum(s);
        const int w = threadIdx.x >> 6, l = threadIdx.x & 63;
        __syncthreads();
        if (l == 0) sh[w] = s;
        __syncthreads();
        if (threadIdx.x == 0) a.norms[a.ntensors + (int64_t)blockIdx.x + t] = sh[0] + sh[1] + sh[2] + sh[3];
        pos = tend;
        ++t;
    }
}
__global__ __launch_bounds__(64) void bert_adam_norm_finish_kernel(vlp_bert_adam_args a) {
    const int t = blockIdx.x;
    if (a.active && !a.active[t]) { if (threadIdx.x == 0) a.norms[t] = 0.f; return; }
    const int64_t lo = a.seg_off[t], hi = a.seg_off[t + 1];
    if (hi <= lo) { if (threadIdx.x == 0) a.norms[t] = 0.f; return; }
    const int64_t c0 = lo / BA_CHUNK, c1 = (hi - 1) / BA_CHUNK;
    const float* part = a.norms + a.ntensors + t;
    float s = 0.f;
    for (int64_t c = c0 + threadIdx.x; c <= c1; c += 64) s += part[c];
    s = wave_sum(s);
    if (threadIdx.x == 0) a.norms[t] = s;
}
extern "C" int64_t vlp_bert_adam_norms_floats(int64_t n, int32_t ntensors) {
    return (int64_t)ntensors + (n + BA_CHUNK - 1) / BA_CHUNK + (int64_t)ntensors;
}
__global__ __launch_bounds__(256) void bert_adam_update_kernel(vlp_bert_adam_args a) {
    const int64_t start = (int64_t)blockIdx.x * BA_CHUNK;
    const int64_t end = min(a.n, start + BA_CHUNK);
    int t = ba_find(a.seg_off, a.ntensors, start);
    int64_t pos = start;
    f16* p16 = (f16*)a.p16;
    while (pos < end) {
        if (t >= a.ntensors) break;
        const int64_t tend = min(end, a.seg_off[t + 1]);
        if (a.active && !a.active[t]) { pos = tend; ++t; continue; }
        float coef = 1.f;
        if (a.max_grad_norm > 0.f) {
            const float c = a.max_grad_norm / (sqrtf(a.norms[t]) + 1e-6f);
            if (c < 1.f) coef = c;
        }
        coef /= a.grad_scale;
        for (int64_t i = pos + threadIdx.x; i < tend; i += blockDim.x) {
            const float g = ba_load(a.g, a.g_is_f32, i) * coef;
            const float m = a.b1 * a.m[i] + (1.f - a.b1) * g;
            const float v = a.b2 * a.v[i] + (1.f - a.b2) * g * g;
            float p = a.p32[i];
            float upd = m / (sqrtf(v) + a.eps);
            if (a.decay > 0.f) upd += a.decay * p;
            p -= a.lr * upd;
            a.m[i] = m; a.v[i] = v; a.p32[i] = p;
            if (p16) p16[i] = (f16)p;
        }
        pos = tend;
        ++t;
    }
}
extern "C" int vlp_bert_adam(const vlp_bert_adam_args* a, void* stream) {
    VLP_CHECK_ARG(a && a->p32 && a->m && a->v && a->g && a->seg_off && a->norms, "vlp_bert_adam: null operand");
    VLP_ENTER(a->p32, "vlp_bert_adam");
    VLP_CHECK_ARG(a->n > 0 && a->ntensors > 0 && a->grad_scale > 0.f, "vlp_bert_adam: bad sizes");
    VLP_CHECK_ARG(a->norms_floats >= vlp_bert_adam_norms_floats(a->n, a->ntensors),
                  "vlp_bert_adam: norms_floats=%lld < vlp_bert_adam_norms_floats(n, ntensors)=%lld", (long long)a->norms_floats,
                  (long long)vlp_bert_adam_norms_floats(a->n, a->ntensors));
    hipStream_t s = (hipStream_t)stream;
    const int blocks = (int)((a->n + BA_CHUNK - 1) / BA_CHUNK);
    if (a->max_grad_norm > 0.f) {
        hipLaunchKernelGGL(bert_adam_norm_kernel, dim3(blocks), dim3(256), 0, s, *a);
        hipLaunchKernelGGL(bert_adam_norm_finish_kernel, dim3(a->ntensors), dim3(64), 0, s, *a);
        VLP_CHECK_LAUNCH("vlp_bert_adam(norm)");
    }
    hipLaunchKernelGGL(bert_adam_update_kernel, dim3(blocks), dim3(256), 0, s, *a);
    VLP_CHECK_LAUNCH("vlp_bert_adam(update)");
    return VLP_OK;
}
```

vlp_amd/csrc/elementwise.hip:

```cpp
#include <hip/hip_fp16.h>
#include "vocab_row.h"

__global__ __launch_bounds__(256) void embed_fwd_kernel(vlp_embed_fwd_args a) {
    const int nch = a.H >> 3;
    const int64_t total = (a.row_map ? (int64_t)a.rows : (int64_t)a.B * a.L) * nch;
    const f16* word = (const f16*)a.word_emb;
    const f16* pos = (const f16*)a.pos_emb;
    const f16* typ = (const f16*)a.type_emb;
    const f16* vis = (const f16*)a.vis_h;
    const f16* vpe = (const f16*)a.vispe_h;
    f16* pre = (f16*)a.pre;
    for (int64_t i = (int64_t)blockIdx.x * blockDim.x + threadIdx.x; i < total; i += (int64_t)gridDim.x * blockDim.x) {
        const int c = (int)(i % nch);
        const int64_t prow = i / nch;
        const int64_t row = a.row_map ? (int64_t)a.row_map[prow] : prow;
        const int l = (int)(row % a.L);
        const int b = (int)(row / a.L);
        f16x8 w, p;
        if (l >= 1 && l <= a.Nv) {
            const int64_t vr = (int64_t)b * a.Nv + (l - 1);
            if (a.region_mask && a.region_mask[vr]) {
#pragma unroll
                for (int e = 0; e < 8; ++e) { w[e] = (f16)0.f; p[e] = (f16)0.f; }
            } else {
                w = ld8(vis + vr * a.H + c * 8);
                p = ld8(vpe + vr * a.H + c * 8);
            }
        } else {
            int64_t id = a.input_ids[row];
            id = id < 0 ? 0 : (id >= a.vocab ? a.vocab - 1 : id);
            w = ld8(word + id * a.H + c * 8);
            int64_t pi = a.position_ids ? a.position_ids[row] : (int64_t)l;
            pi = pi < 0 ? 0 : (pi >= a.max_pos ? a.max_pos - 1 : pi);
            p = ld8(pos + pi * a.H + c * 8);
        }
        int64_t sg = a.segment_ids[row];
        sg = sg < 0 ? 0 : (sg >= a.type_vocab ? a.type_vocab - 1 : sg);
        f16x8 t = ld8(typ + sg * a.H + c * 8), o;
#pragma unroll
        for (int e = 0; e < 8; ++e) o[e] = (f16)((float)w[e] + (float)p[e] + (float)t[e]);
        st8(pre + prow * a.H + c * 8, o);
    }
}
extern "C" int vlp_embed_fwd(const vlp_embed_fwd_args* a, void* stream) {
    VLP_CHECK_ARG(a && a->input_ids && a->segment_ids && a->word_emb && a->pos_emb && a->type_emb && a->pre, "vlp_embed_fwd: null operand");
    VLP_ENTER(a->pre, "vlp_embed_fwd");
    VLP_CHECK_ARG(a->H % 8 == 0 && a->B > 0 && a->L > 0 && a->Nv >= 0 && a->Nv + 1 < a->L + 1, "vlp_embed_fwd: bad shape");
    VLP_CHECK_ARG(a->Nv == 0 || (a->vis_h && a->vispe_h), "vlp_embed_fwd: region rows need vis_h / vispe_h");
    VLP_CHECK_ARG(a->row_map == nullptr || (a->rows > 0 && (int64_t)a->rows <= (int64_t)a->B * a->L), "vlp_embed_fwd: packed output needs 0 < rows <= B*L");
    const int64_t total = (a->row_map ? (int64_t)a->rows : (int64_t)a->B * a->L) * (a->H / 8);
    int blocks = (int)((total + 255) / 256);
    if (blocks > 4096) blocks = 4096;
    hipLaunchKernelGGL(embed_fwd_kernel, dim3(blocks), dim3(256), 0, (hipStream_t)stream, *a);
    VLP_CHECK_LAUNCH("vlp_embed_fwd");
    return VLP_OK;
}

#define EMB_TSPLITS 64
#define EMB_MAXT 8
__global__ __launch_bounds__(256) void embed_bwd_kernel(vlp_embed_bwd_args a, DropCtx dvis, DropCtx dvpe) {
    const int nch = a.H >> 3;
    const int64_t total = (int64_t)a.B * a.L * nch;
    const f16* dpre = (const f16*)a.dpre;
    for (int64_t i = (int64_t)blockIdx.x * blockDim.x + threadIdx.x; i < total; i += (int64_t)gridDim.x * blockDim.x) {
        const int c = (int)(i % nch);
        const int64_t row = i / nch;
        const int l = (int)(row % a.L);
        const int b = (int)(row / a.L);
        const f16x8 d = ld8(dpre + row * a.H + c * 8);
        if (l >= 1 && l <= a.Nv) {
            const int64_t vr = (int64_t)b * a.Nv + (l - 1);
            if (a.region_mask && a.region_mask[vr]) continue;
            const f16x8 yv = ld8((const f16*)a.vis_h + vr * a.H + c * 8);
            const f16x8 yp = ld8((const f16*)a.vispe_h + vr * a.H + c * 8);
            f16x8 ov, op;
            const uint32_t kv = dvis.thresh ? drop_rowkey(dvis, (uint64_t)vr) : 0u;
            const uint32_t kp = dvpe.thresh ? drop_rowkey(dvpe, (uint64_t)vr) : 0u;
#pragma unroll
            for (int e = 0; e < 8; ++e) {
                const uint32_t col = (uint32_t)(c * 8 + e);
                float gv = ((float)yv[e] > 0.f) ? (float)d[e] : 0.f;
                float gp = ((float)yp[e] > 0.f) ? (float)d[e] : 0.f;
                if (dvis.thresh) gv *= drop_mult(dvis, kv, col);
                if (dvpe.thresh) gp *= drop_mult(dvpe, kp, col);
                ov[e] = (f16)gv;
                op[e] = (f16)gp;
            }
            st8((f16*)a.d_vis_h + vr * a.H + c * 8, ov);
            st8((f16*)a.d_vispe_h + vr * a.H + c * 8, op);
        }
    }
}
#define EWB_G 32
#define EWB_LIST 1024
struct EwbGeom {
    const int64_t* ids;
    int L, Nv, T, NT, vocab;
    DEVFN int64_t row_of(int u) const { const int b = u / T, j = u - b * T; return (int64_t)b * L + (j == 0 ? 0 : Nv + j); }
    DEVFN int id_of(int u) const { const int64_t id = ids[row_of(u)]; return (int)(id < 0 ? 0 : (id >= vocab ? vocab - 1 : id)); }
};
template <typename Pred>
DEVFN int ewb_compact(int* list, int* wcnt, int n, int u0, int NT, Pred pred) {
    const int tid = threadIdx.x, lane = tid & 63, wv = tid >> 6;
    const int u = u0 + tid;
    const bool m = u < NT && pred(u);
    const uint64_t bal = __ballot(m);
    if (lane == 0) wcnt[wv] = __popcll(bal);
    __syncthreads();
    int off = n;
    for (int w = 0; w < wv; ++w) off += wcnt[w];
    if (m) list[off + __popcll(bal & ((1ull << lane) - 1ull))] = u;
    n += wcnt[0] + wcnt[1] + wcnt[2] + wcnt[3];
    __syncthreads();
    return n;
}
__global__ __launch_bounds__(256) void embed_word_partial_kernel(EwbGeom g, const f16* dpre, int H, int* rank, float* partial) {
    __shared__ int list[256 + EWB_G];
    __shared__ int wcnt[4];
    __shared__ float wsum[4];
    const int tid = threadIdx.x, t = blockIdx.x;
    const int id = g.id_of(t);
    float c = 0.f;
    for (int u = tid; u < t; u += 256) c += (g.id_of(u) == id) ? 1.f : 0.f;
    c = wave_sum(c);
    if ((tid & 63) == 0) wsum[tid >> 6] = c;
    __syncthreads();
    const int r = (int)(wsum[0] + wsum[1] + wsum[2] + wsum[3]);
    if (tid == 0) rank[t] = r;
    if (r % EWB_G) return;
    int n = 0;
    for (int u0 = t; u0 < g.NT && n < EWB_G; u0 += 256) n = ewb_compact(list, wcnt, n, u0, g.NT, [&](int u) { return g.id_of(u) == id; });
    n = min(n, EWB_G);
    const int nch = H >> 3;
    if (tid < nch) {
        float acc[8];
#pragma unroll
        for (int e = 0; e < 8; ++e) acc[e] = 0.f;
        int i = 0;
        for (; i + 4 <= n; i += 4) {
            f16x8 d[4];
#pragma unroll
            for (int k = 0; k < 4; ++k) d[k] = ld8(dpre + g.row_of(list[i + k]) * H + tid * 8);
#pragma unroll
            for (int k = 0; k < 4; ++k)
#pragma unroll
                for (int e = 0; e < 8; ++e) acc[e] += (float)d[k][e];
        }
        for (; i < n; ++i) {
            const f16x8 d = ld8(dpre + g.row_of(list[i]) * H + tid * 8);
#pragma unroll
            for (int e = 0; e < 8; ++e) acc[e] += (float)d[e];
        }
        float* dst = partial + (int64_t)t * H + tid * 8;
        *reinterpret_cast<f32x4*>(dst) = (f32x4){acc[0], acc[1], acc[2], acc[3]};
        *reinterpret_cast<f32x4*>(dst + 4) = (f32x4){acc[4], acc[5], acc[6], acc[7]};
    }
}
__global__ __launch_bounds__(256) void embed_word_reduce_kernel(EwbGeom g, int H, const int* rank, const float* partial, f16* dword) {
    __shared__ int list[EWB_LIST + 256];
    __shared__ int wcnt[4];
    const int tid = threadIdx.x, t = blockIdx.x;
    if (rank[t] != 0) return;
    const int id = g.id_of(t);
    const int nch = H >> 3;
    float acc[8];
#pragma unroll
    for (int e = 0; e < 8; ++e) acc[e] = 0.f;
    int start = t;
    while (start < g.NT) {
        int n = 0, u0 = start;
        for (; u0 < g.NT && n < EWB_LIST; u0 += 256)
            n = ewb_compact(list, wcnt, n, u0, g.NT, [&](int u) { return (rank[u] % EWB_G) == 0 && g.id_of(u) == id; });
        start = u0;
        if (tid < nch) {
            for (int i = 0; i < n; ++i) {
                const float* src = partial + (int64_t)list[i] * H + tid * 8;
                const f32x4 a0 = *reinterpret_cast<const f32x4*>(src), a1 = *reinterpret_cast<const f32x4*>(src + 4);
#pragma unroll
                for (int e = 0; e < 4; ++e) { acc[e] += a0[e]; acc[4 + e] += a1[e]; }
            }
        }
        __syncthreads();
    }
    if (tid < nch) {
        f16* dst = dword + (int64_t)id * H + tid * 8;
        f16x8 o = ld8(dst);
#pragma unroll
        for (int e = 0; e < 8; ++e) o[e] = (f16)((float)o[e] + acc[e]);
        st8(dst, o);
    }
}
__global__ void embed_bwd_pos_kernel(const f16* dpre, f16* dpos, int B, int L, int Nv, int H) {
    const int nch = H >> 3;
    const int64_t total = (int64_t)L * nch;
    for (int64_t i = (int64_t)blockIdx.x * blockDim.x + threadIdx.x; i < total; i += (int64_t)gridDim.x * blockDim.x) {
        const int c = (int)(i % nch);
        const int l = (int)(i / nch);
        if (l >= 1 && l <= Nv) continue;
        float acc[8];
#pragma unroll
        for (int e = 0; e < 8; ++e) acc[e] = 0.f;
        for (int b = 0; b < B; ++b) {
            const f16x8 d = ld8(dpre + ((int64_t)b * L + l) * H + c * 8);
#pragma unroll
            for (int e = 0; e < 8; ++e) acc[e] += (float)d[e];
        }
        f16* dst = dpos + (int64_t)l * H + c * 8;
        f16x8 o = ld8(dst);
#pragma unroll
        for (int e = 0; e < 8; ++e) o[e] = (f16)((float)o[e] + acc[e]);
        st8(dst, o);
    }
}
__global__ __launch_bounds__(256) void embed_bwd_type_kernel(const f16* dpre, const int64_t* seg, float* part, int64_t rows, int H, int T) {
    __shared__ float red[8][256];
    const int tx = threadIdx.x & 31, ty = threadIdx.x >> 5;
    const int c0 = blockIdx.x * 256 + tx * 8;
    const int64_t rows_per = (rows + gridDim.y - 1) / gridDim.y;
    const int64_t r0 = blockIdx.y * rows_per, r1 = min(rows, r0 + rows_per);
    float acc[EMB_MAXT][8];
#pragma unroll
    for (int t = 0; t < EMB_MAXT; ++t)
#pragma unroll
        for (int e = 0; e < 8; ++e) acc[t][e] = 0.f;
    if (c0 < H) {
        for (int64_t r = r0 + ty; r < r1; r += 8) {
            int64_t sg = seg[r];
            sg = sg < 0 ? 0 : (sg >= T ? T - 1 : sg);
            const f16x8 d = ld8(dpre + r * H + c0);
#pragma unroll
            for (int t = 0; t < EMB_MAXT; ++t) {
                const float m = (sg == t) ? 1.f : 0.f;
#pragma unroll
                for (int e = 0; e < 8; ++e) acc[t][e] += m * (float)d[e];
            }
        }
    }
#pragma unroll
    for (int t = 0; t < EMB_MAXT; ++t) {
        __syncthreads();
#pragma unroll
        for (int e = 0; e < 8; ++e) red[ty][tx * 8 + e] = acc[t][e];
        __syncthreads();
        float s = 0.f;
#pragma unroll
        for (int y = 0; y < 8; ++y) s += red[y][threadIdx.x];
        const int col = blockIdx.x * 256 + threadIdx.x;
        if (col < H && t < T) part[((int64_t)blockIdx.y * EMB_MAXT + t) * H + col] = s;
    }
}
__global__ void embed_bwd_type_reduce_kernel(const float* part, int nsplits, f16* dtyp, int T, int H) {
    const int i = blockIdx.x * blockDim.x + threadIdx.x;
    if (i >= T * H) return;
    const int t = i / H, c = i % H;
    float s = 0.f;
    for (int p = 0; p < nsplits; ++p) s += part[((int64_t)p * EMB_MAXT + t) * H + c];
    dtyp[i] = (f16)((float)dtyp[i] + s);
}
extern "C" int64_t vlp_embed_bwd_workspace_floats(int32_t B, int32_t L, int32_t Nv, int32_t H) {
    const int64_t nt = (int64_t)B * (L - Nv);
    return (int64_t)EMB_TSPLITS * EMB_MAXT * H + nt * H + nt;
}
__global__ __launch_bounds__(256) void embed_bwd_pos_ids_kernel(const f16* dpre, const int64_t* pid, f16* dpos, int B, int L, int Nv, int H, int max_pos) {
    __shared__ int list[256];
    __shared__ int wcnt[4];
    const int r = blockIdx.x, tid = threadIdx.x, nch = H >> 3;
    const int NT = B * L;
    auto pred = [&](int u) {
        const int l = u % L;
        if (l >= 1 && l <= Nv) return false;
        int64_t pi = pid[u];
        pi = pi < 0 ? 0 : (pi >= max_pos ? max_pos - 1 : pi);
        return pi == (int64_t)r;
    };
    float acc[8];
#pragma unroll
    for (int e = 0; e < 8; ++e) acc[e] = 0.f;
    int total = 0;
    for (int u0 = 0; u0 < NT; u0 += 256) {
        const int n = ewb_compact(list, wcnt, 0, u0, NT, pred);
        total += n;
        if (tid < nch) {
            for (int i = 0; i < n; ++i) {
                const f16x8 d = ld8(dpre + (int64_t)list[i] * H + tid * 8);
#pragma unroll
                for (int e = 0; e < 8; ++e) acc[e] += (float)d[e];
            }
        }
    }
    if (total == 0 || tid >= nch) return;
    f16* dst = dpos + (int64_t)r * H + tid * 8;
    f16x8 o = ld8(dst);
#pragma unroll
    for (int e = 0; e < 8; ++e) o[e] = (f16)((float)o[e] + acc[e]);
    st8(dst, o);
}
static int embed_bwd_run(const vlp_embed_bwd_args* a, const int64_t* position_ids, int max_pos, void* stream) {
    VLP_CHECK_ARG(a && a->dpre && a->input_ids && a->segment_ids && a->d_word_emb && a->d_pos_emb && a->d_type_emb && a->acc32, "vlp_embed_bwd: null operand");
    VLP_ENTER(a->dpre, "vlp_embed_bwd");
    VLP_CHECK_ARG(a->H % 8 == 0 && a->H <= 2048 && a->B > 0 && a->L > a->Nv && a->type_vocab >= 1 && a->type_vocab <= EMB_MAXT,
                  "vlp_embed_bwd: bad shape (H % 8 == 0, H <= 2048, L > Nv, type_vocab <= 8)");
    VLP_CHECK_ARG(a->Nv == 0 || (a->vis_h && a->vispe_h && a->d_vis_h && a->d_vispe_h), "vlp_embed_bwd: region buffers");
    hipStream_t s = (hipStream_t)stream;
    const int64_t total = (int64_t)a->B * a->L * (a->H / 8);
    int blocks = (int)((total + 255) / 256);
    if (blocks > 4096) blocks = 4096;
    VLP_CHECK_ARG(a->parts >= 0 && a->parts <= 2, "vlp_embed_bwd: parts must be 0 (all), 1 (region rows) or 2 (tables)");
    if (a->parts != 2 && a->Nv > 0) {
        hipLaunchKernelGGL(embed_bwd_kernel, dim3(blocks), dim3(256), 0, s, *a, make_drop(a->drop_p, a->seed, a->vis_stream),
                           make_drop(a->drop_p, a->seed, a->vispe_stream));
        VLP_CHECK_LAUNCH("vlp_embed_bwd");
    }
    if (a->parts == 1) return VLP_OK;
    {
        EwbGeom g;
        g.ids = a->input_ids; g.L = a->L; g.Nv = a->Nv; g.T = a->L - a->Nv; g.NT = a->B * g.T; g.vocab = a->vocab;
        float* partial = a->acc32 + (int64_t)EMB_TSPLITS * EMB_MAXT * a->H;
        int* rank = reinterpret_cast<int*>(partial + (int64_t)g.NT * a->H);
        hipLaunchKernelGGL(embed_word_partial_kernel, dim3(g.NT), dim3(256), 0, s, g, (const f16*)a->dpre, a->H, rank, partial);
        VLP_CHECK_LAUNCH("vlp_embed_word_partial");
        hipLaunchKernelGGL(embed_word_reduce_kernel, dim3(g.NT), dim3(256), 0, s, g, a->H, (const int*)rank, (const float*)partial, (f16*)a->d_word_emb);
        VLP_CHECK_LAUNCH("vlp_embed_word_reduce");
    }
    if (position_ids) {
        hipLaunchKernelGGL(embed_bwd_pos_ids_kernel, dim3(max_pos), dim3(256), 0, s, (const f16*)a->dpre, position_ids, (f16*)a->d_pos_emb,
                           a->B, a->L, a->Nv, a->H, max_pos);
        VLP_CHECK_LAUNCH("vlp_embed_bwd_pos(ids)");
    } else {
        hipLaunchKernelGGL(embed_bwd_pos_kernel, dim3(cdiv((int64_t)a->L * (a->H / 8), 256)), dim3(256), 0, s, (const f16*)a->dpre,
                           (f16*)a->d_pos_emb, a->B, a->L, a->Nv, a->H);
        VLP_CHECK_LAUNCH("vlp_embed_bwd_pos");
    }
    const int64_t rows = (int64_t)a->B * a->L;
    int splits = rows >= EMB_TSPLITS * 8 ? EMB_TSPLITS : (int)((rows + 7) / 8);
    hipLaunchKernelGGL(embed_bwd_type_kernel, dim3(cdiv(a->H, 256), splits), dim3(256), 0, s, (const f16*)a->dpre, a->segment_ids, a->acc32,
                       rows, a->H, a->type_vocab);
    VLP_CHECK_LAUNCH("vlp_embed_bwd_type");
    hipLaunchKernelGGL(embed_bwd_type_reduce_kernel, dim3(cdiv((int64_t)a->type_vocab * a->H, 256)), dim3(256), 0, s, a->acc32, splits,
                       (f16*)a->d_type_emb, a->type_vocab, a->H);
    VLP_CHECK_LAUNCH("vlp_embed_bwd_type_reduce");
    return VLP_OK;
}
extern "C" int vlp_embed_bwd(const vlp_embed_bwd_args* a, void* stream) { return embed_bwd_run(a, nullptr, 0, stream); }
extern "C" int vlp_embed_bwd_pos(const vlp_embed_bwd_pos_args* a, void* stream) {
    VLP_CHECK_ARG(a && a->position_ids, "vlp_embed_bwd_pos: null position_ids");
    VLP_CHECK_ARG(a->max_pos > 0 && (int64_t)a->base.B * a->base.L <= (1ll << 30), "vlp_embed_bwd_pos: bad shape (max_pos > 0)");
    return embed_bwd_run(&a->base, a->position_ids, a->max_pos, stream);
}

__global__ void copy2d_kernel(const void* src, int64_t lds, int src_f32, f16* dst, int64_t ldd, int rows, int cols_src, int cols_dst, int beta) {
    const int64_t total = (int64_t)rows * cols_dst;
    for (int64_t i = (int64_t)blockIdx.x * blockDim.x + threadIdx.x; i < total; i += (int64_t)gridDim.x * blockDim.x) {
        const int64_t r = i / cols_dst;
        const int c = (int)(i % cols_dst);
        float v = 0.f;
        if (c < cols_src) v = src_f32 ? ((const float*)src)[r * lds + c] : (float)((const f16*)src)[r * lds + c];
        f16* d = dst + r * ldd + c;
        *d = (f16)(beta ? (float)*d + v : v);
    }
}
extern "C" int vlp_copy2d(const void* src, int64_t lds, int32_t src_f32, void* dst, int64_t ldd, int32_t rows, int32_t cols_src,
                          int32_t cols_dst, int32_t beta, void* stream) {
    VLP_CHECK_ARG(src && dst && rows > 0 && cols_src > 0 && cols_dst > 0, "vlp_copy2d: bad args");
    VLP_ENTER(src, "vlp_copy2d");
    VLP_CHECK_ARG(lds >= (cols_src < cols_dst ? cols_src : cols_dst) && ldd >= cols_dst, "vlp_copy2d: leading dims");
    const int64_t total = (int64_t)rows * cols_dst;
    int blocks = (int)((total + 255) / 256);
    if (blocks > 8192) blocks = 8192;
    hipLaunchKernelGGL(copy2d_kernel, dim3(blocks), dim3(256), 0, (hipStream_t)stream, src, lds, src_f32, (f16*)dst, ldd, rows,
                       cols_src < cols_dst ? cols_src : cols_dst, cols_dst, beta);
    VLP_CHECK_LAUNCH("vlp_copy2d");
    return VLP_OK;
}

__global__ __launch_bounds__(256) void transpose_kernel(const f16* __restrict__ src, int64_t lds, f16* __restrict__ dst, int64_t ldd, int rows, int cols, int rows_pad) {
    __shared__ f16 tile[64][66];
    const int r0 = blockIdx.y * 64, c0 = blockIdx.x * 64;
    const int tx = threadIdx.x & 63, ty = threadIdx.x >> 6;
    for (int i = ty; i < 64; i += 4) {
        const int r = r0 + i, c = c0 + tx;
        tile[i][tx] = (r < rows && c < cols) ? src[(int64_t)r * lds + c] : (f16)0.f;
    }
    __syncthreads();
    for (int i = ty; i < 64; i += 4) {
        const int c = c0 + i, r = r0 + tx;
        if (c < cols && r < rows_pad) dst[(int64_t)c * ldd + r] = tile[tx][i];
    }
}
extern "C" int vlp_transpose(const void* src, int64_t lds, void* dst, int64_t ldd, int32_t rows, int32_t cols, int32_t rows_pad, void* stream) {
    VLP_CHECK_ARG(src && dst && rows > 0 && cols > 0 && rows_pad >= rows && ldd >= rows_pad && lds >= cols, "vlp_transpose: bad args");
    VLP_ENTER(src, "vlp_transpose");
    dim3 grid(cdiv(cols, 64), cdiv(rows_pad, 64));
    hipLaunchKernelGGL(transpose_kernel, grid, dim3(256), 0, (hipStream_t)stream, (const f16*)src, lds, (f16*)dst, ldd, rows, cols, rows_pad);
    VLP_CHECK_LAUNCH("vlp_transpose");
    return VLP_OK;
}

DEVFN int64_t sample_base(const int32_t* row_off, int64_t b, int L, int& n) {
    if (row_off) { const int lo = row_off[b]; n = row_off[b + 1] - lo; return lo; }
    n = L;
    return b * L;
}
__global__ void gather_rows_kernel(const f16* src, int64_t lds, const int64_t* pos, f16* out, int64_t ldo, int B, int P, int L, int H, const int32_t* row_off) {
    const int nch = H >> 3;
    const int64_t total = (int64_t)B * P * nch;
    for (int64_t i = (int64_t)blockIdx.x * blockDim.x + threadIdx.x; i < total; i += (int64_t)gridDim.x * blockDim.x) {
        const int c = (int)(i % nch);
        const int64_t r = i / nch;
        int n;
        const int64_t base = sample_base(row_off, r / P, L, n);
        int64_t ps = pos[r];
        ps = ps < 0 ? 0 : (ps >= n ? n - 1 : ps);
        st8(out + r * ldo + c * 8, ld8(src + (base + ps) * lds + c * 8));
    }
}
extern "C" int vlp_gather_rows(const void* src, int64_t lds, const int64_t* pos, void* out, int64_t ldo, int32_t B, int32_t P, int32_t L,
                               int32_t H, const int32_t* row_off, void* stream) {
    VLP_CHECK_ARG(src && pos && out && B > 0 && P > 0 && L > 0 && H % 8 == 0 && lds % 8 == 0 && ldo % 8 == 0, "vlp_gather_rows: bad args");
    VLP_ENTER(src, "vlp_gather_rows");
    const int64_t total = (int64_t)B * P * (H / 8);
    hipLaunchKernelGGL(gather_rows_kernel, dim3((int)((total + 255) / 256)), dim3(256), 0, (hipStream_t)stream, (const f16*)src, lds, pos,
                       (f16*)out, ldo, B, P, L, H, row_off);
    VLP_CHECK_LAUNCH("vlp_gather_rows");
    return VLP_OK;
}
__global__ void scatter_add_rows_kernel(const f16* src, int64_t lds, const int64_t* pos, f16* dst, int64_t ldd, int B, int P, int L, int H, const int32_t* row_off) {
    const int nch = H >> 3;
    const int64_t total = (int64_t)B * P * nch;
    for (int64_t i = (int64_t)blockIdx.x * blockDim.x + threadIdx.x; i < total; i += (int64_t)gridDim.x * blockDim.x) {
        const int c = (int)(i % nch);
        const int64_t r = i / nch;
        int n;
        const int64_t base = sample_base(row_off, r / P, L, n);
        int64_t ps = pos[r];
        ps = ps < 0 ? 0 : (ps >= n ? n - 1 : ps);
        const f16x8 v = ld8(src + r * lds + c * 8);
        __half2* d = reinterpret_cast<__half2*>(dst + (base + ps) * ldd + c * 8);
#pragma unroll
        for (int e = 0; e < 4; ++e) unsafeAtomicAdd(d + e, __floats2half2_rn((float)v[2 * e], (float)v[2 * e + 1]));
    }
}
extern "C" int vlp_scatter_add_rows(const void* src, int64_t lds, const int64_t* pos, void* dst, int64_t ldd, int32_t B, int32_t P, int32_t L,
                                    int32_t H, const int32_t* row_off, void* stream) {
    VLP_CHECK_ARG(src && pos && dst && B > 0 && P > 0 && L > 0 && H % 8 == 0 && lds % 8 == 0 && ldd % 8 == 0, "vlp_scatter_add_rows: bad args");
    VLP_ENTER(src, "vlp_scatter_add_rows");
    const int64_t total = (int64_t)B * P * (H / 8);
    hipLaunchKernelGGL(scatter_add_rows_kernel, dim3((int)((total + 255) / 256)), dim3(256), 0, (hipStream_t)stream, (const f16*)src, lds,
                       pos, (f16*)dst, ldd, B, P, L, H, row_off);
    VLP_CHECK_LAUNCH("vlp_scatter_add_rows");
    return VLP_OK;
}

__global__ void vqa_mul_fwd_kernel(const f16* h, f16* out, int B, int L, int Nv, int H, const int32_t* row_off) {
    const int64_t total = (int64_t)B * H;
    for (int64_t i = (int64_t)blockIdx.x * blockDim.x + threadIdx.x; i < total; i += (int64_t)gridDim.x * blockDim.x) {
        const int64_t b = i / H;
        const int c = (int)(i % H);
        const int64_t r0 = row_off ? (int64_t)row_off[b] : b * L;
        const float a0 = (float)h[r0 * H + c], a1 = (float)h[(r0 + Nv + 1) * H + c];
        out[i] = (f16)(a0 * a1);
    }
}
extern "C" int vlp_vqa_mul_fwd(const void* h, void* out, int32_t B, int32_t L, int32_t Nv, int32_t H, const int32_t* row_off, void* stream) {
    VLP_CHECK_ARG(h && out && B > 0 && Nv + 1 < L, "vlp_vqa_mul_fwd: bad args");
    VLP_ENTER(h, "vlp_vqa_mul_fwd");
    hipLaunchKernelGGL(vqa_mul_fwd_kernel, dim3(cdiv((int64_t)B * H, 256)), dim3(256), 0, (hipStream_t)stream, (const f16*)h, (f16*)out, B, L, Nv, H, row_off);
    VLP_CHECK_LAUNCH("vlp_vqa_mul_fwd");
    return VLP_OK;
}
__global__ void vqa_mul_bwd_kernel(const f16* h, const f16* dout, f16* dh, int B, int L, int Nv, int H, const int32_t* row_off) {
    const int64_t total = (int64_t)B * H;
    for (int64_t i = (int64_t)blockIdx.x * blockDim.x + threadIdx.x; i < total; i += (int64_t)gridDim.x * blockDim.x) {
        const int64_t b = i / H;
        const int c = (int)(i % H);
        const int64_t r0 = row_off ? (int64_t)row_off[b] : b * L;
        const int64_t i0 = r0 * H + c, i1 = (r0 + Nv + 1) * H + c;
        const float d = (float)dout[i], a0 = (float)h[i0], a1 = (float)h[i1];
        dh[i0] = (f16)((float)dh[i0] + d * a1);
        dh[i1] = (f16)((float)dh[i1] + d * a0);
    }
}
extern "C" int vlp_vqa_mul_bwd(const void* h, const void* dout, void* dh, int32_t B, int32_t L, int32_t Nv, int32_t H, const int32_t* row_off, void* stream) {
    VLP_CHECK_ARG(h && dout && dh && B > 0 && Nv + 1 < L, "vlp_vqa_mul_bwd: bad args");
    VLP_ENTER(h, "vlp_vqa_mul_bwd");
    hipLaunchKernelGGL(vqa_mul_bwd_kernel, dim3(cdiv((int64_t)B * H, 256)), dim3(256), 0, (hipStream_t)stream, (const f16*)h, (const f16*)dout,
                       (f16*)dh, B, L, Nv, H, row_off);
    VLP_CHECK_LAUNCH("vlp_vqa_mul_bwd");
    return VLP_OK;
}

__global__ void rowmap_build_kernel(const int32_t* row_off, int L, int32_t* row_map) {
    const int b = blockIdx.x;
    const int lo = row_off[b], n = row_off[b + 1] - lo;
    for (int l = threadIdx.x; l < n; l += blockDim.x) row_map[lo + l] = b * L + l;
}
extern "C" int vlp_rowmap_build(const int32_t* row_off, int32_t B, int32_t L, int32_t* row_map, void* stream) {
    VLP_CHECK_ARG(row_off && row_map && B > 0 && L > 0, "vlp_rowmap_build: bad args");
    VLP_ENTER(row_off, "vlp_rowmap_build");
    hipLaunchKernelGGL(rowmap_build_kernel, dim3(B), dim3(256), 0, (hipStream_t)stream, row_off, L, row_map);
    VLP_CHECK_LAUNCH("vlp_rowmap_build");
    return VLP_OK;
}
template <bool UNPACK>
__global__ void rows_move_kernel(const f16* src, int64_t lds, const int32_t* row_map, int rows, f16* dst, int64_t ldd, int H) {
    const int nch = H >> 3;
    const int64_t total = (int64_t)rows * nch;
    for (int64_t i = (int64_t)blockIdx.x * blockDim.x + threadIdx.x; i < total; i += (int64_t)gridDim.x * blockDim.x) {
        const int c = (int)(i % nch);
        const int64_t p = i / nch, r = row_map[p];
        if (UNPACK) st8(dst + r * ldd + c * 8, ld8(src + p * lds + c * 8));
        else st8(dst + p * ldd + c * 8, ld8(src + r * lds + c * 8));
    }
}
static int rows_move(bool unpack, const void* src, int64_t lds, const int32_t* row_map, int32_t rows, void* dst, int64_t ldd, int32_t H, void* stream) {
    VLP_CHECK_ARG(src && dst && row_map && rows > 0 && H > 0 && H % 8 == 0 && lds % 8 == 0 && ldd % 8 == 0 && lds >= H && ldd >= H, "vlp_rows_pack/unpack: bad args");
    VLP_ENTER(src, "vlp_rows_pack/unpack");
    const int64_t total = (int64_t)rows * (H / 8);
    int blocks = (int)((total + 255) / 256);
    if (blocks > 8192) blocks = 8192;
    if (unpack) hipLaunchKernelGGL(rows_move_kernel<true>, dim3(blocks), dim3(256), 0, (hipStream_t)stream, (const f16*)src, lds, row_map, rows, (f16*)dst, ldd, H);
    else hipLaunchKernelGGL(rows_move_kernel<false>, dim3(blocks), dim3(256), 0, (hipStream_t)stream, (const f16*)src, lds, row_map, rows, (f16*)dst, ldd, H);
    VLP_CHECK_LAUNCH("vlp_rows_pack/unpack");
    return VLP_OK;
}
extern "C" int vlp_rows_unpack(const void* src, int64_t lds, const int32_t* row_map, int32_t rows, void* dst, int64_t ldd, int32_t H, void* stream) {
    return rows_move(true, src, lds, row_map, rows, dst, ldd, H, stream);
}
extern "C" int vlp_rows_pack(const void* src, int64_t lds, const int32_t* row_map, int32_t rows, void* dst, int64_t ldd, int32_t H, void* stream) {
    return rows_move(false, src, lds, row_map, rows, dst, ldd, H, stream);
}

__global__ void relu_dropout_bwd_kernel(const f16* dy, const f16* y, f16* dz, int64_t n8, int64_t ncols, DropCtx d) {
    for (int64_t i = (int64_t)blockIdx.x * blockDim.x + threadIdx.x; i < n8; i += (int64_t)gridDim.x * blockDim.x) {
        const f16x8 g = ld8(dy + i * 8), yv = ld8(y + i * 8);
        const int64_t row = (i * 8) / ncols;
        const uint32_t col0 = (uint32_t)((i * 8) % ncols);
        const uint32_t rk = d.thresh ? drop_rowkey(d, (uint64_t)row) : 0u;
        f16x8 o;
#pragma unroll
        for (int e = 0; e < 8; ++e) {
            float v = ((float)yv[e] > 0.f) ? (float)g[e] : 0.f;
            if (d.thresh) v *= drop_mult(d, rk, col0 + (uint32_t)e);
            o[e] = (f16)v;
        }
        st8(dz + i * 8, o);
    }
}
extern "C" int vlp_relu_dropout_bwd(const void* dy, const void* y, void* dz, int64_t n, int64_t ncols, float drop_p, uint64_t seed,
                                    uint32_t rng_stream, void* stream) {
    VLP_CHECK_ARG(dy && y && dz && n > 0 && ncols > 0 && ncols % 8 == 0 && n % ncols == 0, "vlp_relu_dropout_bwd: contiguous [rows, ncols], ncols % 8 == 0");
    VLP_ENTER(dy, "vlp_relu_dropout_bwd");
    int blocks = (int)((n / 8 + 255) / 256);
    if (blocks > 4096) blocks = 4096;
    hipLaunchKernelGGL(relu_dropout_bwd_kernel, dim3(blocks), dim3(256), 0, (hipStream_t)stream, (const f16*)dy, (const f16*)y, (f16*)dz, n / 8, ncols,
                       make_drop(drop_p, seed, rng_stream));
    VLP_CHECK_LAUNCH("vlp_relu_dropout_bwd");
    return VLP_OK;
}

__global__ void gelu_bwd_kernel(const f16* dy, const f16* z, f16* dz, int64_t n8) {
    for (int64_t i = (int64_t)blockIdx.x * blockDim.x + threadIdx.x; i < n8; i += (int64_t)gridDim.x * blockDim.x) {
        const f16x8 g = ld8(dy + i * 8), zv = ld8(z + i * 8);
        f16x8 o;
#pragma unroll
        for (int e = 0; e < 8; ++e) o[e] = (f16)((float)g[e] * gelu_grad_f((float)zv[e]));
        st8(dz + i * 8, o);
    }
}
extern "C" int vlp_gelu_bwd(const void* dy, const void* z, void* dz, int64_t n, void* stream) {
    VLP_CHECK_ARG(dy && z && dz && n > 0 && n % 8 == 0, "vlp_gelu_bwd: n must be a positive multiple of 8");
    VLP_ENTER(dy, "vlp_gelu_bwd");
    int blocks = (int)((n / 8 + 255) / 256);
    if (blocks > 4096) blocks = 4096;
    hipLaunchKernelGGL(gelu_bwd_kernel, dim3(blocks), dim3(256), 0, (hipStream_t)stream, (const f16*)dy, (const f16*)z, (f16*)dz, n / 8);
    VLP_CHECK_LAUNCH("vlp_gelu_bwd");
    return VLP_OK;
}

__global__ __launch_bounds__(256) void transpose_batched_kernel(const vlp_transpose_desc* __restrict__ descs, const int32_t* __restrict__ tile_start, int n) {
    __shared__ f16 tile[64][72];
    int mi = 0;
    const int t = blockIdx.x;
    while (mi + 1 < n && tile_start[mi + 1] <= t) ++mi;
    const vlp_transpose_desc d = descs[mi];
    const f16* src = (const f16*)d.src;
    f16* dst = (f16*)d.dst;
    const int tiles_c = (d.cols + 63) / 64;
    const int lt = t - tile_start[mi];
    const int r0 = (lt / tiles_c) * 64, c0 = (lt % tiles_c) * 64;
    const int tr = threadIdx.x >> 3, tc = (threadIdx.x & 7) * 8;
#pragma unroll
    for (int i = 0; i < 2; ++i) {
        const int r = r0 + tr + 32 * i, c = c0 + tc;
        f16x8 v = (f16x8){0, 0, 0, 0, 0, 0, 0, 0};
        if (r < d.rows) {
            if (c + 8 <= d.cols) v = ld8(src + (int64_t)r * d.lds + c);
            else
#pragma unroll
                for (int e = 0; e < 8; ++e) if (c + e < d.cols) v[e] = src[(int64_t)r * d.lds + c + e];
        }
        *reinterpret_cast<f16x8*>(&tile[tr + 32 * i][tc]) = v;
    }
    __syncthreads();
#pragma unroll
    for (int i = 0; i < 2; ++i) {
        const int c = c0 + tr + 32 * i;
        const int r = r0 + tc;
        if (c >= d.cols || r >= d.rows_pad) continue;
        f16x8 v;
#pragma unroll
        for (int e = 0; e < 8; ++e) v[e] = tile[tc + e][tr + 32 * i];
        if (r + 8 <= d.rows_pad) st8(dst + (int64_t)c * d.ldd + r, v);
        else
#pragma unroll
            for (int e = 0; e < 8; ++e) if (r + e < d.rows_pad) dst[(int64_t)c * d.ldd + r + e] = v[e];
    }
}
extern "C" int vlp_transpose_batched(const vlp_transpose_desc* descs_dev, const int32_t* tile_start_dev, int32_t n, int32_t total_tiles, void* stream) {
    VLP_CHECK_ARG(descs_dev && tile_start_dev && n > 0 && total_tiles > 0, "vlp_transpose_batched: bad args");
    VLP_ENTER(descs_dev, "vlp_transpose_batched");
    hipLaunchKernelGGL(transpose_batched_kernel, dim3(total_tiles), dim3(256), 0, (hipStream_t)stream, descs_dev, tile_start_dev, n);
    VLP_CHECK_LAUNCH("vlp_transpose_batched");
    return VLP_OK;
}

__global__ void kv_append_kernel(const f16* qkv, int64_t ld, f16* cache, int Lcap, int B, int T, int start, int H) {
    const int nch = (2 * H) >> 3;
    const int64_t total = (int64_t)B * T * nch;
    for (int64_t i = (int64_t)blockIdx.x * blockDim.x + threadIdx.x; i < total; i += (int64_t)gridDim.x * blockDim.x) {
        const int c = (int)(i % nch);
        const int64_t r = i / nch;
        const int t = (int)(r % T);
        const int64_t b = r / T;
        st8(cache + ((b * Lcap + start + t) * 2 * (int64_t)H) + c * 8, ld8(qkv + r * ld + H + c * 8));
    }
}
extern "C" int vlp_kv_append(const void* qkv_new, int64_t ld, void* cache, int32_t Lcap, int32_t B, int32_t T, int32_t start, int32_t H, void* stream) {
    VLP_CHECK_ARG(qkv_new && cache && B > 0 && T > 0 && start >= 0 && start + T <= Lcap && H % 8 == 0 && ld % 8 == 0, "vlp_kv_append: bad args");
    VLP_ENTER(qkv_new, "vlp_kv_append");
    const int64_t total = (int64_t)B * T * (2 * H / 8);
    int blocks = (int)((total + 255) / 256);
    if (blocks > 4096) blocks = 4096;
    hipLaunchKernelGGL(kv_append_kernel, dim3(blocks), dim3(256), 0, (hipStream_t)stream, (const f16*)qkv_new, ld, (f16*)cache, Lcap, B, T, start, H);
    VLP_CHECK_LAUNCH("vlp_kv_append");
    return VLP_OK;
}

__global__ __launch_bounds__(256) void argmax_rows_kernel(const f16* logits, int64_t ld, int V, int64_t* ids, int64_t ids_stride, float* vals,
                                                          int64_t vals_stride) {
    __shared__ float sv[256];
    __shared__ int si[256];
    const f16* x = logits + (int64_t)blockIdx.x * ld;
    float best;
    int bi;
    row_first_max<256, false>(x, 0, V, best, bi);
    argmax_block256(best, bi, sv, si);
    if (threadIdx.x == 0) { ids[blockIdx.x * ids_stride] = si[0]; vals[blockIdx.x * vals_stride] = sv[0]; }
}
extern "C" int vlp_argmax_rows(const void* logits, int64_t ld, int32_t rows, int32_t V, int64_t* ids, int64_t ids_stride, float* vals,
                               int64_t vals_stride, void* stream) {
    VLP_CHECK_ARG(logits && ids && vals && rows > 0 && V > 0 && ld >= V, "vlp_argmax_rows: bad args");
    VLP_ENTER(logits, "vlp_argmax_rows");
    hipLaunchKernelGGL(argmax_rows_kernel, dim3(rows), dim3(256), 0, (hipStream_t)stream, (const f16*)logits, ld, V, ids, ids_stride, vals, vals_stride);
    VLP_CHECK_LAUNCH("vlp_argmax_rows");
    return VLP_OK;
}
__global__ __launch_bounds__(256) void vqa_answer_rows_kernel(const f16* logits, int64_t ld, int N, int first_col, const int32_t* ans_idx,
                                                              const float* ans_score, int S, int64_t* out_ids, float* out_vals, float* out_scores) {
    __shared__ float sv[256];
    __shared__ int si[256];
    const f16* x = logits + (int64_t)blockIdx.x * ld;
    float best;
    int bi;
    row_first_max<256, false>(x, first_col, N, best, bi);
    argmax_block256(best, bi, sv, si);
    if (threadIdx.x == 0) {
        const int id = si[0] == 0x7fffffff ? first_col : si[0];
        out_ids[blockIdx.x] = id;
        out_vals[blockIdx.x] = si[0] == 0x7fffffff ? (float)x[first_col] : sv[0];
        if (ans_idx) {
            float sc = 0.f;
            for (int s = 0; s < S; ++s) sc = ans_idx[(int64_t)blockIdx.x * S + s] == id ? ans_score[(int64_t)blockIdx.x * S + s] : sc;
            out_scores[blockIdx.x] = sc;
        }
    }
}
extern "C" int vlp_vqa_answer_rows(const void* logits, int64_t ld, int32_t rows, int32_t N, int32_t first_col, const int32_t* ans_idx,
                                   const float* ans_score, int32_t S, int64_t* out_ids, float* out_vals, float* out_scores, void* stream) {
    VLP_CHECK_ARG(logits && out_ids && out_vals && rows > 0 && first_col >= 0 && N > first_col && ld >= N, "vlp_vqa_answer_rows: bad args");
    VLP_CHECK_ARG(!ans_idx || (ans_score && out_scores && S > 0 && S <= 16), "vlp_vqa_answer_rows: targets need ans_score, out_scores and 0 < S <= 16");
    VLP_ENTER(logits, "vlp_vqa_answer_rows");
    hipLaunchKernelGGL(vqa_answer_rows_kernel, dim3(rows), dim3(256), 0, (hipStream_t)stream, (const f16*)logits, ld, N, first_col, ans_idx, ans_score, S,
                       out_ids, out_vals, out_scores);
    VLP_CHECK_LAUNCH("vlp_vqa_answer_rows");
    return VLP_OK;
}

#define TOPK_LIST_MAX 1024
struct TopkList { const int32_t* ids; int64_t ld; const int32_t* cnt; };
template <int NT>
DEVFN int topk_list_load(const TopkList& tl, int row, int tid, int* lst) {
    int n = tl.cnt[row];
    const int cap = tl.ld < TOPK_LIST_MAX ? (int)tl.ld : TOPK_LIST_MAX;
    n = n < 0 ? 0 : (n > cap ? cap : n);
    for (int j = tid; j < n; j += NT) lst[j] = tl.ids[(int64_t)row * tl.ld + j];
    return n;
}
DEVFN bool topk_list_has(const int* lst, int n, int v) {
    bool hit = false;
    for (int j = 0; j < n; ++j) hit |= lst[j] == v;
    return hit;
}
template <bool LIST>
__global__ __launch_bounds__(256) void logsoftmax_topk_kernel(const f16* logits, int64_t ld, int V, int K, const uint8_t* forbid, TopkList tl, int eos_id,
                                                              int block_eos, float* out_scores, int64_t* out_ids) {
    __shared__ float sv[256];
    __shared__ int si[256];
    __shared__ int lst[LIST ? TOPK_LIST_MAX : 1];
    const int row = blockIdx.x, tid = threadIdx.x;
    const f16* x = logits + (int64_t)row * ld;
    const uint8_t* fb = (!LIST && forbid) ? forbid + (int64_t)row * V : nullptr;
    int ncand = 0;
    if constexpr (LIST) ncand = topk_list_load<256>(tl, row, tid, lst);
    float mx = -INFINITY;
    for (int v = tid; v < V; v += 256) mx = fmaxf(mx, (float)x[v]);
    sv[tid] = mx;
    __syncthreads();
    for (int o = 128; o > 0; o >>= 1) {
        if (tid < o) sv[tid] = fmaxf(sv[tid], sv[tid + o]);
        __syncthreads();
    }
    mx = sv[0];
    __syncthreads();
    float sum = 0.f;
    for (int v = tid; v < V; v += 256) sum += __expf((float)x[v] - mx);
    sv[tid] = sum;
    __syncthreads();
    for (int o = 128; o > 0; o >>= 1) {
        if (tid < o) sv[tid] += sv[tid + o];
        __syncthreads();
    }
    const float lse = mx + __logf(sv[0]);
    __syncthreads();
    float pv = INFINITY;
    int pi = -1;
    for (int k = 0; k < K; ++k) {
        float best = -INFINITY;
        int bi = 0x7fffffff;
        for (int v = tid; v < V; v += 256) {
            float val = (float)x[v] - lse;
            if (fb && fb[v]) val += -10000.0f;
            const bool is_eos = block_eos && v == eos_id;
            if (is_eos) val = -10000.0f;
            if constexpr (LIST) {
                if (!is_eos && (val > best || (val == best && v < bi)) && topk_list_has(lst, ncand, v)) val += -10000.0f;
            }
            const bool after = (val < pv) || (val == pv && v > pi);
            if (after && (val > best || (val == best && v < bi))) { best = val; bi = v; }
        }
        sv[tid] = best;
        si[tid] = bi;
        __syncthreads();
        for (int o = 128; o > 0; o >>= 1) {
            if (tid < o) {
                const float f = sv[tid + o];
                const int j = si[tid + o];
                if (f > sv[tid] || (f == sv[tid] && j < si[tid])) { sv[tid] = f; si[tid] = j; }
            }
            __syncthreads();
        }
        pv = sv[0];
        pi = si[0];
        if (tid == 0) { out_scores[(int64_t)row * K + k] = pv; out_ids[(int64_t)row * K + k] = pi; }
        __syncthreads();
    }
}
template <int KMAX, bool LIST>
__global__ __launch_bounds__(1024) void logsoftmax_topk_small_kernel(const f16* logits, int64_t ld, int V, int K, const uint8_t* forbid, TopkList tl,
                                                                     int eos_id, int block_eos, float* out_scores, int64_t* out_ids) {
    __shared__ float red[16], sv[16];
    __shared__ int si[16];
    __shared__ int lst[LIST ? TOPK_LIST_MAX : 1];
    const int row = blockIdx.x, tid = threadIdx.x;
    const f16* x = logits + (int64_t)row * ld;
    const uint8_t* fb = (!LIST && forbid) ? forbid + (int64_t)row * V : nullptr;
    int ncand = 0;
    if constexpr (LIST) ncand = topk_list_load<1024>(tl, row, tid, lst);
    float mx = -INFINITY;
    row_visit<1024, true>(x, 0, V, [&](float f, int) { mx = fmaxf(mx, f); });
    mx = block_reduce_max<1024>(mx, red);
    float sum = 0.f;
    row_visit<1024, true>(x, 0, V, [&](float f, int) { sum += __expf(f - mx); });
    const float lse = mx + __logf(block_reduce_sum<1024>(sum, red));
    float lv[KMAX];
    int lidx[KMAX];
#pragma unroll
    for (int j = 0; j < KMAX; ++j) { lv[j] = -INFINITY; lidx[j] = 0x7fffffff; }
    auto offer = [&](float raw, int v) {
        float val = raw - lse;
        if (fb && fb[v]) val += -10000.0f;
        const bool is_eos = block_eos && v == eos_id;
        if (is_eos) val = -10000.0f;
        if (val > lv[KMAX - 1] || (val == lv[KMAX - 1] && v < lidx[KMAX - 1])) {
            if constexpr (LIST) {
                if (!is_eos && topk_list_has(lst, ncand, v)) {
                    val += -10000.0f;
                    if (!(val > lv[KMAX - 1] || (val == lv[KMAX - 1] && v < lidx[KMAX - 1]))) return;
                }
            }
            int vi = v;
#pragma unroll
            for (int j = 0; j < KMAX; ++j) {
                const bool better = val > lv[j] || (val == lv[j] && vi < lidx[j]);
                const float tv = better ? lv[j] : val;
                const int ti = better ? lidx[j] : vi;
                lv[j] = better ? val : lv[j];
                lidx[j] = better ? vi : lidx[j];
                val = tv;
                vi = ti;
            }
        }
    };
    row_visit<1024, true>(x, 0, V, offer);
    for (int k = 0; k < K; ++k) {
        float bv = lv[0];
        int bi = lidx[0];
        argmax_block1024(bv, bi, sv, si);
        if (tid == 0) { out_scores[(int64_t)row * K + k] = bv; out_ids[(int64_t)row * K + k] = bi; }
        if (lidx[0] == bi) {
#pragma unroll
            for (int j = 0; j + 1 < KMAX; ++j) { lv[j] = lv[j + 1]; lidx[j] = lidx[j + 1]; }
            lv[KMAX - 1] = -INFINITY;
            lidx[KMAX - 1] = 0x7fffffff;
        }
        __syncthreads();
    }
}
static int topk_launch(const char* who, const void* logits, int64_t ld, int rows, int V, int K, const uint8_t* forbid, const TopkList* tl, int eos_id,
                       int block_eos, float* out_scores, int64_t* out_ids, hipStream_t s) {
    const bool vec_ok = ld % 8 == 0 && (uintptr_t)logits % 16 == 0;
    const TopkList none = {nullptr, 0, nullptr};
#define LAUNCH_TOPK(KM)                                                                                                                          \
    do {                                                                                                                                         \
        if (tl) hipLaunchKernelGGL((logsoftmax_topk_small_kernel<KM, true>), dim3(rows), dim3(1024), 0, s, (const f16*)logits, ld, V, K, nullptr, *tl, \
                                   eos_id, block_eos, out_scores, out_ids);                                                                       \
        else hipLaunchKernelGGL((logsoftmax_topk_small_kernel<KM, false>), dim3(rows), dim3(1024), 0, s, (const f16*)logits, ld, V, K, forbid, none,  \
                                eos_id, block_eos, out_scores, out_ids);                                                                          \
    } while (0)
    if (vec_ok && K <= 4) LAUNCH_TOPK(4);
    else if (vec_ok && K <= 8) LAUNCH_TOPK(8);
    else if (vec_ok && K <= 16) LAUNCH_TOPK(16);
    else if (tl)
        hipLaunchKernelGGL(logsoftmax_topk_kernel<true>, dim3(rows), dim3(256), 0, s, (const f16*)logits, ld, V, K, nullptr, *tl, eos_id, block_eos,
                           out_scores, out_ids);
    else
        hipLaunchKernelGGL(logsoftmax_topk_kernel<false>, dim3(rows), dim3(256), 0, s, (const f16*)logits, ld, V, K, forbid, none, eos_id, block_eos,
                           out_scores, out_ids);
#undef LAUNCH_TOPK
    VLP_CHECK_LAUNCH(who);
    return VLP_OK;
}
extern "C" int vlp_logsoftmax_topk(const void* logits, int64_t ld, int32_t rows, int32_t V, int32_t K, const uint8_t* forbid, int32_t eos_id,
                                   int32_t block_eos, float* out_scores, int64_t* out_ids, void* stream) {
    VLP_CHECK_ARG(logits && out_scores && out_ids && rows > 0 && V > 0 && K > 0 && K <= V && ld >= V, "vlp_logsoftmax_topk: bad args");
    VLP_ENTER(logits, "vlp_logsoftmax_topk");
    return topk_launch("vlp_logsoftmax_topk", logits, ld, rows, V, K, forbid, nullptr, eos_id, block_eos, out_scores, out_ids, (hipStream_t)stream);
}
extern "C" int vlp_logsoftmax_topk_list(const void* logits, int64_t ld, int32_t rows, int32_t V, int32_t K, const int32_t* cand_ids, int64_t cand_ld,
                                        const int32_t* cand_cnt, int32_t eos_id, int32_t block_eos, float* out_scores, int64_t* out_ids, void* stream) {
    VLP_CHECK_ARG(logits && out_scores && out_ids && rows > 0 && V > 0 && K > 0 && K <= V && ld >= V, "vlp_logsoftmax_topk_list: bad args");
    VLP_CHECK_ARG(cand_ids && cand_cnt && cand_ld >= 1 && cand_ld <= TOPK_LIST_MAX, "vlp_logsoftmax_topk_list: needs cand_ids / cand_cnt with 1 <= cand_ld <= %d",
                  TOPK_LIST_MAX);
    VLP_ENTER(logits, "vlp_logsoftmax_topk_list");
    const TopkList tl = {cand_ids, cand_ld, cand_cnt};
    return topk_launch("vlp_logsoftmax_topk_list", logits, ld, rows, V, K, nullptr, &tl, eos_id, block_eos, out_scores, out_ids, (hipStream_t)stream);
}

#define NGRAM_MAX_FRAMES 256
__global__ __launch_bounds__(64) void ngram_candidates_kernel(const int64_t* wids, const int64_t* ptrs, int B, int K, int s, int n, const int64_t* ignore,
                                                              int n_ignore, int32_t* cand_ids, int64_t cand_ld, int32_t* cand_cnt) {
    __shared__ unsigned char bp[NGRAM_MAX_FRAMES * 64];
    __shared__ int path[NGRAM_MAX_FRAMES];
    __shared__ int seq[NGRAM_MAX_FRAMES];
    __shared__ int hit[NGRAM_MAX_FRAMES];
    __shared__ int dead;
    const int r = blockIdx.x, b = r / K, k = r % K, lane = threadIdx.x, L = s + 1;
    if (L < n) {
        if (lane == 0) cand_cnt[r] = 0;
        return;
    }
    for (int i = lane; i < L * K; i += 64) {
        const int f = i / K, j = i - f * K;
        const int64_t p = ptrs[((int64_t)f * B + b) * K + j];
        bp[i] = (unsigned char)((p >= 0 && p < K) ? p : 0);
    }
    if (lane == 0) dead = 0;
    __syncthreads();
    if (lane == 0) {
        int j = k;
        for (int f = s; f >= 0; --f) {
            path[f] = j;
            j = bp[f * K + j];
        }
    }
    __syncthreads();
    for (int f = lane; f < L; f += 64) seq[f] = (int)wids[((int64_t)f * B + b) * K + path[f]];
    __syncthreads();
    const int t0 = L - (n - 1), nm = L - (n - 1);
    for (int i = lane; i < (n - 1) * n_ignore; i += 64)
        if ((int64_t)seq[t0 + i / n_ignore] == ignore[i % n_ignore]) dead = 1;
    for (int i = lane; i < nm; i += 64) {
        bool m = true;
        for (int j = 0; j < n - 1; ++j) m &= seq[i + j] == seq[t0 + j];
        const int nxt = seq[i + n - 1];
        if (m)
            for (int q = 0; q < n_ignore; ++q) m &= ignore[q] != (int64_t)nxt;
        hit[i] = m ? 1 : 0;
    }
    __syncthreads();
    int cnt = 0;
    if (!dead) {
        for (int i0 = 0; i0 < nm; i0 += 64) {
            const int i = i0 + lane;
            bool first = i < nm && hit[i];
            if (first) {
                const int nxt = seq[i + n - 1];
                for (int j = 0; j < i; ++j) first &= !(hit[j] && seq[j + n - 1] == nxt);
            }
            const unsigned long long mask = __ballot(first);
            if (first) cand_ids[(int64_t)r * cand_ld + cnt + __popcll(mask & ((1ull << lane) - 1ull))] = seq[i + n - 1];
            cnt += __popcll(mask);
        }
    }
    if (lane == 0) cand_cnt[r] = cnt;
}
extern "C" int vlp_ngram_candidates(const int64_t* wids, const int64_t* ptrs, int32_t B, int32_t K, int32_t s, int32_t ngram_size, const int64_t* ignore_ids,
                                    int32_t n_ignore, int32_t* cand_ids, int64_t cand_ld, int32_t* cand_cnt, void* stream) {
    VLP_CHECK_ARG(wids && ptrs && cand_ids && cand_cnt, "vlp_ngram_candidates: null operand");
    VLP_ENTER(wids, "vlp_ngram_candidates");
    VLP_CHECK_ARG(B > 0 && K > 0 && K <= 64 && s >= 0 && s + 1 <= NGRAM_MAX_FRAMES && ngram_size >= 2 && cand_ld >= (int64_t)s + 1,
                  "vlp_ngram_candidates: needs B > 0, 0 < K <= 64, 0 <= s < %d, ngram_size >= 2, cand_ld >= s + 1", NGRAM_MAX_FRAMES);
    VLP_CHECK_ARG(n_ignore >= 0 && (n_ignore == 0 || ignore_ids), "vlp_ngram_candidates: n_ignore > 0 needs ignore_ids");
    hipLaunchKernelGGL(ngram_candidates_kernel, dim3(B * K), dim3(64), 0, (hipStream_t)stream, wids, ptrs, B, K, s, ngram_size, ignore_ids, n_ignore, cand_ids,
                       cand_ld, cand_cnt);
    VLP_CHECK_LAUNCH("vlp_ngram_candidates");
    return VLP_OK;
}

__global__ void beam_select_kernel(vlp_beam_select_args a) {
    const int b = blockIdx.x, K = a.K;
    if (threadIdx.x != 0) return;
    float pv = INFINITY;
    int pi = -1;
    for (int k = 0; k < K; ++k) {
        float best = -INFINITY;
        int bi = 0x7fffffff;
        const int ncand = a.first ? K : K * K;
        for (int i = 0; i < ncand; ++i) {
            float val;
            if (a.first) {
                val = a.kk_scores[(int64_t)b * K + i];
            } else {
                const int src = i / K;
                val = a.kk_scores[((int64_t)b * K + src) * K + (i % K)] + a.last_eos[(int64_t)b * K + src] * -10000.0f + a.last_total[(int64_t)b * K + src];
            }
            const bool after = (val < pv) || (val == pv && i > pi);
            if (after && (val > best || (val == best && i < bi))) { best = val; bi = i; }
        }
        pv = best;
        pi = bi;
        const int ptr = a.first ? 0 : bi / K;
        const int64_t id = a.first ? a.kk_ids[(int64_t)b * K + bi] : a.kk_ids[((int64_t)b * K + ptr) * K + (bi % K)];
        const int64_t o = (int64_t)b * K + k;
        a.out_scores[o] = best;
        a.out_ids[o] = id;
        a.out_ptrs[o] = ptr;
        a.out_eos[o] = id == a.eos_id ? 1.0f : 0.0f;
        a.src_rows[o] = a.first ? (int64_t)b : (int64_t)b * K + ptr;
        a.next_ids[o * a.next_ids_stride] = id;
    }
}
extern "C" int vlp_beam_select(const vlp_beam_select_args* a, void* stream) {
    VLP_CHECK_ARG(a && a->kk_scores && a->kk_ids && a->out_scores && a->out_ids && a->out_ptrs && a->out_eos && a->src_rows && a->next_ids,
                  "vlp_beam_select: null operand");
    VLP_ENTER(a->kk_scores, "vlp_beam_select");
    VLP_CHECK_ARG(a->B > 0 && a->K > 0 && a->K <= 64 && (a->first || (a->last_total && a->last_eos)), "vlp_beam_select: bad args");
    hipLaunchKernelGGL(beam_select_kernel, dim3(a->B), dim3(64), 0, (hipStream_t)stream, *a);
    VLP_CHECK_LAUNCH("vlp_beam_select");
    return VLP_OK;
}

__global__ void kv_gather_kernel(const f16* src, int64_t src_rows, f16* dst, int64_t dst_rows, const int64_t* idx, int R, int lo, int hi, int E) {
    const int nch = E >> 3;
    const int64_t total = (int64_t)R * (hi - lo) * nch;
    for (int64_t i = (int64_t)blockIdx.x * blockDim.x + threadIdx.x; i < total; i += (int64_t)gridDim.x * blockDim.x) {
        const int c = (int)(i % nch);
        const int64_t t = i / nch;
        const int pos = lo + (int)(t % (hi - lo));
        const int64_t r = t / (hi - lo);
        st8(dst + ((r * dst_rows + pos) * E) + c * 8, ld8(src + ((idx[r] * src_rows + pos) * E) + c * 8));
    }
}
extern "C" int vlp_kv_gather(const void* src, int64_t src_rows_per_batch, void* dst, int64_t dst_rows_per_batch, const int64_t* idx, int32_t R,
                             int32_t lo, int32_t hi, int32_t row_elems, void* stream) {
    VLP_CHECK_ARG(src && dst && idx && R > 0 && lo >= 0 && hi >= lo && hi <= src_rows_per_batch && hi <= dst_rows_per_batch && row_elems % 8 == 0,
                  "vlp_kv_gather: bad args");
    VLP_ENTER(src, "vlp_kv_gather");
    if (hi == lo) return VLP_OK;
    const int64_t total = (int64_t)R * (hi - lo) * (row_elems / 8);
    int blocks = (int)((total + 255) / 256);
    if (blocks > 8192) blocks = 8192;
    hipLaunchKernelGGL(kv_gather_kernel, dim3(blocks), dim3(256), 0, (hipStream_t)stream, (const f16*)src, src_rows_per_batch, (f16*)dst,
                       dst_rows_per_batch, idx, R, lo, hi, row_elems);
    VLP_CHECK_LAUNCH("vlp_kv_gather");
    return VLP_OK;
}

__global__ __launch_bounds__(256) void sample_rows_kernel(const f16* logits, int64_t ld, int V, DropCtx rng, int64_t* ids, int64_t ids_stride, float* logp,
                                                          int64_t logp_stride) {
    __shared__ float sv[256];
    __shared__ int si[256];
    const int row = blockIdx.x, tid = threadIdx.x;
    const f16* x = logits + (int64_t)row * ld;
    float mx = -INFINITY;
    for (int v = tid; v < V; v += 256) mx = fmaxf(mx, (float)x[v]);
    sv[tid] = mx;
    __syncthreads();
    for (int o = 128; o > 0; o >>= 1) {
        if (tid < o) sv[tid] = fmaxf(sv[tid], sv[tid + o]);
        __syncthreads();
    }
    mx = sv[0];
    __syncthreads();
    const uint32_t rkey = drop_rowkey(rng, (uint64_t)row);
    float sum = 0.f, best = -INFINITY;
    int bi = 0x7fffffff;
    for (int v = tid; v < V; v += 256) {
        const float l = (float)x[v];
        sum += __expf(l - mx);
        const uint32_t h = mix32(rkey + (uint32_t)v * 0x9E3779B9u);
        const float u = ((float)(h >> 8) + 0.5f) * (1.0f / 16777216.0f);
        const float gum = -__logf(-__logf(u));
        const float val = l + gum;
        if (val > best) { best = val; bi = v; }
    }
    sv[tid] = sum;
    __syncthreads();
    for (int o = 128; o > 0; o >>= 1) {
        if (tid < o) sv[tid] += sv[tid + o];
        __syncthreads();
    }
    const float lse = mx + __logf(sv[0]);
    __syncthreads();
    sv[tid] = best;
    si[tid] = bi;
    __syncthreads();
    for (int o = 128; o > 0; o >>= 1) {
        if (tid < o) {
            const float f = sv[tid + o];
            const int j = si[tid + o];
            if (f > sv[tid] || (f == sv[tid] && j < si[tid])) { sv[tid] = f; si[tid] = j; }
        }
        __syncthreads();
    }
    if (tid == 0) {
        ids[row * ids_stride] = si[0];
        logp[row * logp_stride] = (float)x[si[0]] - lse;
    }
}
extern "C" int vlp_sample_rows(const void* logits, int64_t ld, int32_t rows, int32_t V, uint64_t seed, uint32_t rng_stream, int64_t* ids,
                               int64_t ids_stride, float* logp, int64_t logp_stride, void* stream) {
    VLP_CHECK_ARG(logits && ids && logp && rows > 0 && V > 0 && ld >= V, "vlp_sample_rows: bad args");
    VLP_ENTER(logits, "vlp_sample_rows");
    DropCtx rng = make_drop(0.5f, seed, rng_stream);
    hipLaunchKernelGGL(sample_rows_kernel, dim3(rows), dim3(256), 0, (hipStream_t)stream, (const f16*)logits, ld, V, rng, ids, ids_stride, logp, logp_stride);
    VLP_CHECK_LAUNCH("vlp_sample_rows");
    return VLP_OK;
}

__global__ __launch_bounds__(256) void vis_pe_prep_kernel(vlp_vis_pe_prep_args a) {
    const int lane = threadIdx.x & 63;
    const int64_t row = (int64_t)blockIdx.x * 4 + (threadIdx.x >> 6);
    if (row >= (int64_t)a.B * a.Nv) return;
    const int64_t b = row / a.Nv;
    const float* bb = a.bbox + b * a.Nv * 6;
    float wmax = -INFINITY, hmax = -INFINITY;
    for (int j = lane; j < a.Nv; j += 64) {
        wmax = fmaxf(wmax, fmaxf(bb[j * 6 + 0], bb[j * 6 + 2]));
        hmax = fmaxf(hmax, fmaxf(bb[j * 6 + 1], bb[j * 6 + 3]));
    }
    const float w_est = wave_max(wmax) + 1e-5f, h_est = wave_max(hmax) + 1e-5f;
    const float* r = a.bbox + row * 6;
    float six[6];
    six[0] = r[0] / w_est; six[1] = r[1] / h_est; six[2] = r[2] / w_est; six[3] = r[3] / h_est;
    six[4] = fmaxf((six[3] - six[1]) * (six[2] - six[0]), 0.f);
    six[5] = r[5];
    float mu = 0.f;
#pragma unroll
    for (int i = 0; i < 6; ++i) mu += six[i];
    mu *= (1.f / 6.f);
    float var = 0.f;
#pragma unroll
    for (int i = 0; i < 6; ++i) var += (six[i] - mu) * (six[i] - mu);
    const float rs6 = rsqrtf(var * (1.f / 6.f) + a.eps);
    f16* o = (f16*)a.out + row * a.ld_out;
    if (lane < 6) {
        float v = six[0];
#pragma unroll
        for (int i = 1; i < 6; ++i) v = lane == i ? six[i] : v;
        o[lane] = (f16)((v - mu) * rs6);
    }
    constexpr int MAXE = 32;
    float x[MAXE];
    float s = 0.f;
#pragma unroll
    for (int e = 0; e < MAXE; ++e) {
        const int c = lane + 64 * e;
        float v = 0.f;
        if (c < a.n_cls) v = a.cls_is_f32 ? ((const float*)a.cls)[row * a.ld_cls + c] : (float)((const f16*)a.cls)[row * a.ld_cls + c];
        x[e] = v;
        s += v;
    }
    const float cm = wave_sum(s) / (float)a.n_cls;
    float q = 0.f;
#pragma unroll
    for (int e = 0; e < MAXE; ++e) {
        const int c = lane + 64 * e;
        if (c < a.n_cls) q += (x[e] - cm) * (x[e] - cm);
    }
    const float crs = rsqrtf(wave_sum(q) / (float)a.n_cls + a.eps);
#pragma unroll
    for (int e = 0; e < MAXE; ++e) {
        const int c = lane + 64 * e;
        if (c < a.n_cls) o[6 + c] = (f16)((x[e] - cm) * crs);
    }
    for (int c = 6 + a.n_cls + lane; c < a.pad_to; c += 64) o[c] = (f16)0.f;
}
extern "C" int vlp_vis_pe_prep(const vlp_vis_pe_prep_args* a, void* stream) {
    VLP_CHECK_ARG(a && a->bbox && a->cls && a->out && a->B > 0 && a->Nv > 0, "vlp_vis_pe_prep: null operand / bad shape");
    VLP_ENTER(a->out, "vlp_vis_pe_prep");
    VLP_CHECK_ARG(a->n_cls > 0 && a->n_cls <= 2048 && a->ld_cls >= a->n_cls && a->pad_to >= 6 + a->n_cls && a->ld_out >= a->pad_to,
                  "vlp_vis_pe_prep: n_cls <= 2048, ld_cls >= n_cls, ld_out >= pad_to >= 6 + n_cls");
    const int64_t rows = (int64_t)a->B * a->Nv;
    hipLaunchKernelGGL(vis_pe_prep_kernel, dim3((unsigned)((rows + 3) / 4)), dim3(256), 0, (hipStream_t)stream, *a);
    VLP_CHECK_LAUNCH("vlp_vis_pe_prep");
    return VLP_OK;
}
```

vlp_amd/optimization_fp16.py:

```python
import logging
import os

import torch

from . import _lib as K
from .engine import is_no_decay

logger = logging.getLogger(__name__)


class FusedAdam(object):

    def __init__(self, params, lr=1e-3, bias_correction=True, betas=(0.9, 0.999), eps=1e-8, eps_inside_sqrt=False,
                 weight_decay=0., max_grad_norm=0., amsgrad=False):
        if amsgrad:
            raise RuntimeError("FusedAdam does not support the AMSGrad variant.")
        params = list(params)
        if len(params) == 0:
            raise ValueError("optimizer got an empty parameter list")
        if not isinstance(params[0], dict):
            params = [{"params": params}]
        self.defaults = dict(lr=lr, bias_correction=bias_correction, betas=betas, eps=eps, weight_decay=weight_decay, max_grad_norm=max_grad_norm)
        self.param_groups = []
        for g in params:
            g = dict(g)
            g["params"] = list(g["params"])
            for k, v in self.defaults.items():
                g.setdefault(k, v)
            self.param_groups.append(g)
        self.eps_mode = 0 if eps_inside_sqrt else 1
        self.state = {}

    def step(self, *a, **k):
        raise NotImplementedError("vlp_amd.FusedAdam is driven by FP16_Optimizer_State.step() (the only way the reference uses it)")

    def zero_grad(self):
        pass

    def state_dict(self):
        return {"param_groups": [{k: v for k, v in g.items() if k != "params"} for g in self.param_groups], "state": self.state}

    def load_state_dict(self, sd):
        for g, s in zip(self.param_groups, sd["param_groups"]):
            g.update(s)
        self.state = sd.get("state", {})


class FP16_Optimizer_State(object):

    def __init__(self, init_optimizer, static_loss_scale=1.0, dynamic_loss_scale=False, dynamic_loss_args=None, verbose=True):
        if not isinstance(init_optimizer, FusedAdam):
            raise TypeError("FP16_Optimizer_State expects a vlp_amd.optimization_fp16.FusedAdam")
        self.optimizer = init_optimizer
        self.param_groups = init_optimizer.param_groups
        eng = None
        for g in self.param_groups:
            for p in g["params"]:
                eng = eng or getattr(p, "_vlp_engine", None) or getattr(p, "_vlp_owner", None)
        if eng is None:
            raise RuntimeError("FP16_Optimizer_State: parameters do not belong to a vlp_amd model")
        eng.pack()
        self.engine = eng
        name_of = {id(p): n for n, p in eng._params.items()}
        self._group_key = []
        for g in self.param_groups:
            names = [name_of[id(p)] for p in g["params"]]
            kinds = {is_no_decay(n) for n in names}
            if len(kinds) != 1:
                raise RuntimeError("FP16_Optimizer_State: a param group mixes decay / no-decay parameters; use the reference's two groups "
                                   "(run_img2txt_dist.py:394-401)")
            key = "nodecay" if kinds.pop() else "decay"
            if set(names) != set(eng.names[key]):
                raise RuntimeError("FP16_Optimizer_State: group does not cover the model's whole %s set" % key)
            self._group_key.append(key)
        if sorted(self._group_key) != ["decay", "nodecay"]:
            raise RuntimeError("FP16_Optimizer_State: expected exactly one decay and one no-decay group")
        dev = eng.device
        self.fp32_groups_flat = [eng.flat[k].float() for k in self._group_key]
        self._m = [torch.zeros_like(t) for t in self.fp32_groups_flat]
        self._v = [torch.zeros_like(t) for t in self.fp32_groups_flat]
        self._sumsq = [torch.zeros(2, device=dev) for _ in self._group_key]
        self._hyper = [torch.zeros(3, device=dev) for _ in self._group_key]
        self._partial = torch.zeros(2048, device=dev)
        self._ovf = torch.zeros(1, device=dev)
        self.dynamic_loss_scale = bool(dynamic_loss_scale)
        if dynamic_loss_scale:
            args = dynamic_loss_args or {}
            init, factor, window = args.get("init_scale", 2 ** 16), args.get("scale_factor", 2), args.get("scale_window", 1000)
        else:
            init, factor, window = static_loss_scale, 2, 1000
        self._scale_state = torch.tensor([init, 0, -1, factor, window, 1.0 if dynamic_loss_scale else 0.0, 0, 0], device=dev, dtype=torch.float32)
        self.verbose = verbose
        self.pipeline_with_forward = os.environ.get("VLP_ADAM_PIPELINE", "0") == "1"
        self._applied0, self._iter0, self._skipped0 = 0, 0, 0
        self._steps_issued = 0
        self._state_gathered_at = -1

    def _sync(self):
        self.engine.wait_params(host=True)

    @property
    def cur_scale(self):
        self._sync()
        return float(self._scale_state[0])

    @property
    def cur_iter(self):
        self._sync()
        return int(self._scale_state[1])

    @property
    def last_overflow_iter(self):
        self._sync()
        return int(self._scale_state[2])

    @property
    def scale_factor(self):
        self._sync()
        return float(self._scale_state[3])

    @property
    def scale_window(self):
        self._sync()
        return int(self._scale_state[4])

    @property
    def overflow(self):
        self._sync()
        return bool(self._ovf[0] != 0)

    @property
    def skipped_steps(self):
        self._sync()
        return int(self._scale_state[6])

    @property
    def applied_steps(self):
        self._sync()
        st = self._scale_state.tolist()
        return int(self._applied0 + (st[1] - self._iter0) - (st[6] - self._skipped0))

    def backward(self, loss):
        self.engine.wait_params()
        loss = loss.float()
        loss.backward(gradient=self._scale_state[0:1].reshape(loss.shape))

    def zero_grad(self, set_grads_to_None=True):
        self.engine.zero_grad()

    def _step_sharded(self, plan):
        eng = self.engine
        eng.wait_params()
        for i, key in enumerate(self._group_key):
            first = True
            for lo, hi in plan.owned(key):
                K.sumsq(eng.gflat[key][lo:hi], hi - lo, self._sumsq[i], self._partial, accumulate=not first)
                first = False
        stats = torch.cat(self._sumsq)
        plan.exchange_norms(stats)
        for i in range(len(self._group_key)):
            self._sumsq[i].copy_(stats[2 * i:2 * i + 2])
        torch.maximum(self._sumsq[0][1:2], self._sumsq[1][1:2], out=self._ovf)
        for i, key in enumerate(self._group_key):
            g = self.param_groups[i]
            K.adam_hyper(self._sumsq[i], self._ovf, self._scale_state, g["max_grad_norm"], self._step_size(g), self._hyper[i])
            for lo, hi in plan.owned(key):
                self._adam_range(i, key, lo, hi)
        K.loss_scale_update(self._scale_state, self._ovf)
        eng._param_works = plan.gather_params(eng.flat["decay"], eng.flat["nodecay"])

    def consolidate(self):
        self._gather_sharded_state()

    def _gather_sharded_state(self):
        plan = getattr(self.engine, "shard_plan", None)
        if plan is None or self._state_gathered_at == self._steps_issued:
            return
        self._state_gathered_at = self._steps_issued
        self.engine.wait_params()
        i_d, i_nd = self._group_key.index("decay"), self._group_key.index("nodecay")
        plan.gather_state([self.fp32_groups_flat[i_d], self._m[i_d], self._v[i_d]], [self.fp32_groups_flat[i_nd], self._m[i_nd], self._v[i_nd]])

    def step(self, closure=None):
        eng = self.engine
        self._steps_issued += 1
        plan = getattr(eng, "shard_plan", None)
        if plan is not None:
            return self._step_sharded(plan)
        if self.pipeline_with_forward:
            return self._step_pipelined()
        eng.wait_params()
        self._grad_norms()
        torch.maximum(self._sumsq[0][1:2], self._sumsq[1][1:2], out=self._ovf)
        for i, key in enumerate(self._group_key):
            g = self.param_groups[i]
            K.adam_hyper(self._sumsq[i], self._ovf, self._scale_state, g["max_grad_norm"], self._step_size(g), self._hyper[i])
            self._adam_range(i, key, 0, eng.sizes[key])
        K.loss_scale_update(self._scale_state, self._ovf)

    def _grad_norms(self):
        eng = self.engine
        for i, key in enumerate(self._group_key):
            K.sumsq(eng.gflat[key], eng.sizes[key], self._sumsq[i], self._partial)

    def _step_size(self, g):
        if g["bias_correction"]:
            b1, b2 = g["betas"]
            t = self.applied_steps + 1
            return g["lr"] * (1 - b2 ** t) ** 0.5 / (1 - b1 ** t)
        return g["lr"]

    def _adam_range(self, i, key, lo, hi):
        g = self.param_groups[i]
        b1, b2 = g["betas"]
        eng = self.engine
        K.fused_adam(self.fp32_groups_flat[i][lo:hi], self._m[i][lo:hi], self._v[i][lo:hi], eng.gflat[key][lo:hi], eng.flat[key][lo:hi], hi - lo,
                     self._hyper[i], b1=b1, b2=b2, eps=g["eps"], decay=g["weight_decay"], eps_inside_sqrt=(self.optimizer.eps_mode == 0))

    def _step_pipelined(self):
        eng = self.engine
        main = torch.cuda.current_stream()
        st = eng.optimizer_stream()
        eng.wait_params()
        st.wait_stream(main)
        events = {}
        with torch.cuda.stream(st):
            self._grad_norms()
            torch.maximum(self._sumsq[0][1:2], self._sumsq[1][1:2], out=self._ovf)
            for i, key in enumerate(self._group_key):
                g = self.param_groups[i]
                K.adam_hyper(self._sumsq[i], self._ovf, self._scale_state, g["max_grad_norm"], self._step_size(g), self._hyper[i])
            i_nd, i_d = self._group_key.index("nodecay"), self._group_key.index("decay")
            self._adam_range(i_nd, "nodecay", 0, eng.sizes["nodecay"])
            ev = torch.cuda.Event()
            ev.record(st)
            events["nodecay"] = ev
            for b in reversed(range(len(eng.buckets))):
                lo, hi = eng.buckets[b]
                self._adam_range(i_d, "decay", lo, hi)
                ev = torch.cuda.Event()
                ev.record(st)
                events[b] = ev
            K.loss_scale_update(self._scale_state, self._ovf)
            done = torch.cuda.Event()
            done.record(st)
        eng.set_param_events(events, done)

    def state_dict(self):
        self._gather_sharded_state()
        self._sync()
        sd = {"dynamic_loss_scale": self.dynamic_loss_scale, "cur_scale": self.cur_scale, "cur_iter": self.cur_iter}
        if self.dynamic_loss_scale:
            sd.update(last_overflow_iter=self.last_overflow_iter, scale_factor=self.scale_factor, scale_window=self.scale_window)
        inner = self.optimizer.state_dict()
        inner["exp_avg"] = [t.clone() for t in self._m]
        inner["exp_avg_sq"] = [t.clone() for t in self._v]
        inner["step"] = self.applied_steps
        inner["group_keys"] = list(self._group_key)
        sd["optimizer_state_dict"] = inner
        sd["fp32_groups_flat"] = [t.clone() for t in self.fp32_groups_flat]
        sd["vlp_rng"] = {"base_seed": self.engine.base_seed, "step_seed": self.engine.step_seed}
        return sd

    def _group_layout(self, i):
        eng = self.engine
        name_of = {id(p): n for n, p in eng._params.items()}
        offs = eng.offsets[self._group_key[i]]
        return [(offs[name_of[id(p)]], p.numel()) for p in self.param_groups[i]["params"]]

    def _to_dense(self, flat, i):
        return torch.cat([flat[o:o + n] for o, n in self._group_layout(i)])

    def _from_dense(self, dense, flat, i):
        lay = self._group_layout(i)
        if dense.numel() != sum(n for _, n in lay):
            raise ValueError("apex state: group %d holds %d elements, this model's group has %d" % (i, dense.numel(), sum(n for _, n in lay)))
        pos = 0
        for o, n in lay:
            flat[o:o + n].copy_(dense[pos:pos + n])
            pos += n

    def apex_state_dict(self):
        self._gather_sharded_state()
        self._sync()
        sd = {"dynamic_loss_scale": self.dynamic_loss_scale, "cur_scale": self.cur_scale, "cur_iter": self.cur_iter}
        if self.dynamic_loss_scale:
            sd.update(last_overflow_iter=self.last_overflow_iter, scale_factor=self.scale_factor, scale_window=self.scale_window)
        step = self.applied_steps
        state, groups = {}, []
        for i, g in enumerate(self.param_groups):
            state[i] = {"step": step, "exp_avg": self._to_dense(self._m[i], i), "exp_avg_sq": self._to_dense(self._v[i], i)}
            hp = {k: v for k, v in g.items() if k != "params"}
            hp["params"] = [i]
            groups.append(hp)
        sd["optimizer_state_dict"] = {"state": state, "param_groups": groups}
        sd["fp32_groups_flat"] = [self._to_dense(self.fp32_groups_flat[i], i) for i in range(len(self.param_groups))]
        return sd

    def load_apex_state_dict(self, sd):
        self._sync()
        inner = sd["optimizer_state_dict"]
        if len(inner["param_groups"]) != len(self.param_groups):
            raise ValueError("apex state: %d param groups, expected %d" % (len(inner["param_groups"]), len(self.param_groups)))
        self.dynamic_loss_scale = sd["dynamic_loss_scale"]
        st = self._scale_state.cpu()
        st[0], st[1] = sd["cur_scale"], sd["cur_iter"]
        if sd["dynamic_loss_scale"]:
            st[2], st[3], st[4], st[5] = sd["last_overflow_iter"], sd["scale_factor"], sd["scale_window"], 1.0
        self._scale_state.copy_(st)
        step = 0
        for i, (g, saved) in enumerate(zip(self.param_groups, inner["param_groups"])):
            g.update({k: v for k, v in saved.items() if k != "params"})
            pid = saved["params"][0]
            stt = inner["state"].get(pid) or inner["state"].get(str(pid)) or {}
            if stt:
                self._from_dense(stt["exp_avg"].to(self._m[i].device).float().reshape(-1), self._m[i], i)
                self._from_dense(stt["exp_avg_sq"].to(self._v[i].device).float().reshape(-1), self._v[i], i)
                step = max(step, int(stt.get("step", 0)))
            self._from_dense(sd["fp32_groups_flat"][i].detach().to(self._m[i].device).float().reshape(-1), self.fp32_groups_flat[i], i)
        stl = self._scale_state.tolist()
        self._applied0, self._iter0, self._skipped0 = step, stl[1], stl[6]
        for i, key in enumerate(self._group_key):
            self.engine.flat[key].copy_(self.fp32_groups_flat[i])
        logger.info("FP16_Optimizer_State: resumed from an apex-layout file; the dropout stream position is not part of that layout "
                    "(masks restart from base_seed=%d, step_seed=%d)", self.engine.base_seed, self.engine.step_seed)

    def load_state_dict(self, sd):
        inner = sd.get("optimizer_state_dict", {})
        if "state" in inner and "param_groups" in inner and "exp_avg" not in inner and "group_keys" not in inner:
            return self.load_apex_state_dict(sd)
        self._sync()
        self.dynamic_loss_scale = sd["dynamic_loss_scale"]
        st = self._scale_state.cpu()
        st[0], st[1] = sd["cur_scale"], sd["cur_iter"]
        if sd["dynamic_loss_scale"]:
            st[2], st[3], st[4], st[5] = sd["last_overflow_iter"], sd["scale_factor"], sd["scale_window"], 1.0
        self._scale_state.copy_(st)
        inner = sd["optimizer_state_dict"]
        self.optimizer.load_state_dict(inner)
        for cur, saved in zip(self._m, inner["exp_avg"]):
            cur.copy_(saved)
        for cur, saved in zip(self._v, inner["exp_avg_sq"]):
            cur.copy_(saved)
        st = self._scale_state.tolist()
        self._applied0, self._iter0, self._skipped0 = int(inner.get("step", 0)), st[1], st[6]
        for cur, saved in zip(self.fp32_groups_flat, sd["fp32_groups_flat"]):
            cur.data.copy_(saved.data)
        for i, key in enumerate(self._group_key):
            self.engine.flat[key].copy_(self.fp32_groups_flat[i])
        if "vlp_rng" in sd:
            self.engine.base_seed, self.engine.step_seed = int(sd["vlp_rng"]["base_seed"]), int(sd["vlp_rng"]["step_seed"])
```

Baseline: 6839 samples/s.

## Fuse grad-norm reductions and Adam hyper computation; merge embedding-backward kernels; vectorize copy2d

Replaces the per-group sumsq/finish launches, the torch.maximum call and the two adam_hyper launches with a single grad_norms kernel. It covers both parameter groups and uses an atomic ticket so the last block does the final reduction and writes the hyperparameters. It also merges the embedding-backward position/word/type kernels into two combined-stage launches and unrolls the type reduction. copy2d becomes templated and vectorized with 8-wide aligned stores. The aim is to cut small-kernel launch overhead in the optimizer and embedding backward, at the cost of relying on last-block atomic synchronization and a persistent ticket.

```diff
diff --git a/include/vlp_hip.h b/include/vlp_hip.h
--- a/include/vlp_hip.h
+++ b/include/vlp_hip.h
@@ -415,6 +415,18 @@
 int vlp_fused_adam(const vlp_fused_adam_args* a, void* stream);
 int vlp_adam_hyper(const float* sumsq2, const float* any_overflow, const float* scale_state, float max_grad_norm,
                    float step_size, float* hyper3, void* stream);
+typedef struct {
+    const void* g[2];
+    int64_t n[2];
+    float* out2[2];
+    float* hyper[2];
+    float max_grad_norm[2], step_size[2];
+    float* partial;
+    uint32_t* ticket;
+    float* any_overflow;
+    const float* scale_state;
+} vlp_grad_norms_args;
+int vlp_grad_norms(const vlp_grad_norms_args* a, void* stream);
 int vlp_loss_scale_update(float* scale_state, const float* overflow, void* stream);
 
 int64_t vlp_bert_adam_norms_floats(int64_t n, int32_t ntensors);
diff --git a/vlp_amd/_lib.py b/vlp_amd/_lib.py
--- a/vlp_amd/_lib.py
+++ b/vlp_amd/_lib.py
@@ -165,6 +165,11 @@
 class FusedAdamArgs(C.Structure):
     _fields_ = [("p32", vp), ("m", vp), ("v", vp), ("g16", vp), ("p16", vp), ("n", i64),
                 ("b1", f32), ("b2", f32), ("eps", f32), ("decay", f32), ("eps_inside_sqrt", i32), ("hyper", vp)]
+
+
+class GradNormsArgs(C.Structure):
+    _fields_ = [("g", vp * 2), ("n", i64 * 2), ("out2", vp * 2), ("hyper", vp * 2), ("max_grad_norm", f32 * 2), ("step_size", f32 * 2),
+                ("partial", vp), ("ticket", vp), ("any_overflow", vp), ("scale_state", vp)]
 
 
 class BertAdamArgs(C.Structure):
@@ -250,6 +255,7 @@
     "vlp_sumsq_acc": (C.c_int, [vp, i64, vp, vp, vp]),
     "vlp_fused_adam": (C.c_int, [C.POINTER(FusedAdamArgs), vp]),
     "vlp_adam_hyper": (C.c_int, [vp, vp, vp, f32, f32, vp, vp]),
+    "vlp_grad_norms": (C.c_int, [C.POINTER(GradNormsArgs), vp]),
     "vlp_loss_scale_update": (C.c_int, [vp, vp, vp]),
     "vlp_bert_adam": (C.c_int, [C.POINTER(BertAdamArgs), vp]),
     "vlp_bert_adam_norms_floats": (i64, [i64, i32]),
@@ -862,6 +868,17 @@
     _check(load().vlp_adam_hyper(ptr(sumsq2), ptr(any_overflow), ptr(scale_state), max_grad_norm, step_size, ptr(hyper3), stream_ptr()))
 
 
+def grad_norms(g16, n, out2, hyper, max_grad_norm, step_size, partial, ticket, any_overflow, scale_state):
+    _req_cuda(g16[0], g16[1], out2[0], out2[1], hyper[0], hyper[1], partial, ticket, any_overflow, scale_state)
+    if partial.numel() < 4096 or ticket.dtype != torch.int32:
+        raise RuntimeError("vlp_amd: grad_norms needs partial f32 [4096] and an int32 ticket")
+    P2, F2 = vp * 2, f32 * 2
+    a = GradNormsArgs(P2(g16[0].data_ptr(), g16[1].data_ptr()), (i64 * 2)(n[0], n[1]), P2(out2[0].data_ptr(), out2[1].data_ptr()),
+                      P2(hyper[0].data_ptr(), hyper[1].data_ptr()), F2(*max_grad_norm), F2(*step_size), ptr(partial), ptr(ticket),
+                      ptr(any_overflow), ptr(scale_state))
+    _check(load().vlp_grad_norms(C.byref(a), stream_ptr()))
+
+
 def loss_scale_update(scale_state, overflow):
     _req_cuda(scale_state, overflow)
     _check(load().vlp_loss_scale_update(ptr(scale_state), ptr(overflow), stream_ptr()))
diff --git a/vlp_amd/csrc/adam.hip b/vlp_amd/csrc/adam.hip
--- a/vlp_amd/csrc/adam.hip
+++ b/vlp_amd/csrc/adam.hip
@@ -3,51 +3,72 @@
 
 #define SQ_BLOCKS 1024
 
-__global__ __launch_bounds__(256) void sumsq_kernel(const f16* __restrict__ g, int64_t n, float* __restrict__ partial) {
-    __shared__ float sh[4], shb[4];
+DEVFN void sumsq_add8(f16x8 v, float& s, float& bad) {
+#pragma unroll
+    for (int e = 0; e < 8; ++e) {
+        const float f = (float)v[e];
+        float sq = f * f;
+        asm("" : "+v"(sq));
+        s += sq;
+        if (!(fabsf(f) <= 65504.f)) bad = 1.f;
+    }
+}
+template <bool WT>
+DEVFN void sumsq_block(const f16* __restrict__ g, int64_t n, int block, int nblocks, float* partial, float* sh) {
     float s = 0.f, bad = 0.f;
     const int64_t n8 = n >> 3;
-    for (int64_t i = (int64_t)blockIdx.x * blockDim.x + threadIdx.x; i < n8; i += (int64_t)gridDim.x * blockDim.x) {
-        f16x8 v = ld8(g + i * 8);
-#pragma unroll
-        for (int e = 0; e < 8; ++e) {
-            const float f = (float)v[e];
-            s += f * f;
-            if (!(fabsf(f) <= 65504.f)) bad = 1.f;
-        }
-    }
-    if (blockIdx.x == 0)
-        for (int64_t i = n8 * 8 + threadIdx.x; i < n; i += blockDim.x) {
-            const float f = (float)g[i];
-            s += f * f;
+    for (int64_t i = (int64_t)block * blockDim.x + threadIdx.x; i < n8; i += (int64_t)nblocks * blockDim.x) sumsq_add8(ld8(g + i * 8), s, bad);
+    if (block == 0)
+        for (int64_t j = n8 * 8 + threadIdx.x; j < n; j += blockDim.x) {
+            const float f = (float)g[j];
+            s = fmaf(f, f, s);
             if (!(fabsf(f) <= 65504.f)) bad = 1.f;
         }
     s = wave_sum(s);
     bad = wave_max(bad);
     const int w = threadIdx.x >> 6, l = threadIdx.x & 63;
-    if (l == 0) { sh[w] = s; shb[w] = bad; }
+    if (l == 0) { sh[w] = s; sh[4 + w] = bad; }
     __syncthreads();
     if (threadIdx.x == 0) {
-        partial[blockIdx.x] = sh[0] + sh[1] + sh[2] + sh[3];
-        partial[SQ_BLOCKS + blockIdx.x] = fmaxf(fmaxf(shb[0], shb[1]), fmaxf(shb[2], shb[3]));
-    }
-}
-__global__ __launch_bounds__(256) void sumsq_finish_kernel(const float* __restrict__ partial, int nblocks, float* __restrict__ out2, int accumulate) {
-    __shared__ float sh[4], shb[4];
+        const float tot = sh[0] + sh[1] + sh[2] + sh[3], b = fmaxf(fmaxf(sh[4], sh[5]), fmaxf(sh[6], sh[7]));
+        if constexpr (WT) {
+            __hip_atomic_store(partial + block, tot, __ATOMIC_RELAXED, __HIP_MEMORY_SCOPE_AGENT);
+            __hip_atomic_store(partial + SQ_BLOCKS + block, b, __ATOMIC_RELAXED, __HIP_MEMORY_SCOPE_AGENT);
+        } else {
+            partial[block] = tot;
+            partial[SQ_BLOCKS + block] = b;
+        }
+    }
+}
+DEVFN void sumsq_total(const float* partial, int nblocks, float* sh, float& tot, float& b) {
     float s = 0.f, bad = 0.f;
     for (int i = threadIdx.x; i < nblocks; i += blockDim.x) { s += partial[i]; bad = fmaxf(bad, partial[SQ_BLOCKS + i]); }
     s = wave_sum(s);
     bad = wave_max(bad);
     const int w = threadIdx.x >> 6, l = threadIdx.x & 63;
-    if (l == 0) { sh[w] = s; shb[w] = bad; }
+    if (l == 0) { sh[w] = s; sh[4 + w] = bad; }
     __syncthreads();
+    tot = sh[0] + sh[1] + sh[2] + sh[3];
+    b = fmaxf(fmaxf(sh[4], sh[5]), fmaxf(sh[6], sh[7]));
+    if (!(tot <= 3.0e38f)) b = 1.f;
+}
+__global__ __launch_bounds__(256) void sumsq_kernel(const f16* __restrict__ g, int64_t n, float* __restrict__ partial) {
+    __shared__ float sh[8];
+    sumsq_block<false>(g, n, blockIdx.x, gridDim.x, partial, sh);
+}
+__global__ __launch_bounds__(256) void sumsq_finish_kernel(const float* __restrict__ partial, int nblocks, float* __restrict__ out2, int accumulate) {
+    __shared__ float sh[8];
+    float tot, b;
+    sumsq_total(partial, nblocks, sh, tot, b);
     if (threadIdx.x == 0) {
-        const float tot = sh[0] + sh[1] + sh[2] + sh[3];
-        float b = fmaxf(fmaxf(shb[0], shb[1]), fmaxf(shb[2], shb[3]));
-        if (!(tot <= 3.0e38f)) b = 1.f;
         out2[0] = accumulate ? out2[0] + tot : tot;
         out2[1] = accumulate ? fmaxf(out2[1], b) : b;
     }
+}
+static int sumsq_blocks(int64_t n) {
+    int blocks = (int)((n / 8 + 255) / 256);
+    if (blocks > SQ_BLOCKS) blocks = SQ_BLOCKS;
+    return blocks < 1 ? 1 : blocks;
 }
 static int sumsq_launch(const void* g, int64_t n, float* out2, float* partial, int accumulate, void* stream);
 extern "C" int vlp_sumsq(const void* g, int64_t n, float* out2, float* partial, void* stream) { return sumsq_launch(g, n, out2, partial, 0, stream); }
@@ -55,9 +76,7 @@
 static int sumsq_launch(const void* g, int64_t n, float* out2, float* partial, int accumulate, void* stream) {
     VLP_CHECK_ARG(g && out2 && partial && n > 0 && (uintptr_t)g % 16 == 0, "vlp_sumsq: bad args (partial must hold 2048 floats)");
     VLP_ENTER(g, "vlp_sumsq");
-    int blocks = (int)((n / 8 + 255) / 256);
-    if (blocks > SQ_BLOCKS) blocks = SQ_BLOCKS;
-    if (blocks < 1) blocks = 1;
+    const int blocks = sumsq_blocks(n);
     hipStream_t s = (hipStream_t)stream;
     hipLaunchKernelGGL(sumsq_kernel, dim3(blocks), dim3(256), 0, s, (const f16*)g, n, partial);
     VLP_CHECK_LAUNCH("vlp_sumsq");
@@ -66,13 +85,8 @@
     return VLP_OK;
 }
 
-__global__ void adam_hyper_kernel(const float* sumsq2, const float* any_overflow, const float* scale_state, float max_grad_norm, float step_size,
-                                  float* hyper) {
-    if (threadIdx.x != 0 || blockIdx.x != 0) return;
-    const float scale = scale_state[0];
-    float overflow = sumsq2[1];
-    if (any_overflow) overflow = fmaxf(overflow, any_overflow[0]);
-    const float norm = sqrtf(sumsq2[0]);
+DEVFN void adam_hyper_set(float sumsq, float overflow, float scale, float max_grad_norm, float step_size, float* hyper) {
+    const float norm = sqrtf(sumsq);
     float combined = scale;
     if (max_grad_norm > 0.f) {
         const float clip = (norm / scale + 1e-6f) / max_grad_norm;
@@ -81,6 +95,13 @@
     hyper[0] = combined;
     hyper[1] = step_size;
     hyper[2] = overflow;
+}
+__global__ void adam_hyper_kernel(const float* sumsq2, const float* any_overflow, const float* scale_state, float max_grad_norm, float step_size,
+                                  float* hyper) {
+    if (threadIdx.x != 0 || blockIdx.x != 0) return;
+    float overflow = sumsq2[1];
+    if (any_overflow) overflow = fmaxf(overflow, any_overflow[0]);
+    adam_hyper_set(sumsq2[0], overflow, scale_state[0], max_grad_norm, step_size, hyper);
 }
 extern "C" int vlp_adam_hyper(const float* sumsq2, const float* any_overflow, const float* scale_state, float max_grad_norm, float step_size,
                               float* hyper3, void* stream) {
@@ -88,6 +109,48 @@
     VLP_ENTER(sumsq2, "vlp_adam_hyper");
     hipLaunchKernelGGL(adam_hyper_kernel, dim3(1), dim3(64), 0, (hipStream_t)stream, sumsq2, any_overflow, scale_state, max_grad_norm, step_size, hyper3);
     VLP_CHECK_LAUNCH("vlp_adam_hyper");
+    return VLP_OK;
+}
+
+__global__ __launch_bounds__(256) void grad_norms_kernel(vlp_grad_norms_args a, int blocks0, int blocks1) {
+    __shared__ float sh[9];
+    if ((int)blockIdx.x >= blocks0) sumsq_block<true>((const f16*)a.g[1], a.n[1], blockIdx.x - blocks0, blocks1, a.partial + 2 * SQ_BLOCKS, sh);
+    else sumsq_block<true>((const f16*)a.g[0], a.n[0], blockIdx.x, blocks0, a.partial, sh);
+    if (threadIdx.x == 0) {
+        asm volatile("s_waitcnt vmcnt(0)" ::: "memory");
+        const unsigned t = __hip_atomic_fetch_add(a.ticket, 1u, __ATOMIC_RELAXED, __HIP_MEMORY_SCOPE_AGENT);
+        const bool last = t == (unsigned)(blocks0 + blocks1 - 1);
+        if (last) {
+            __builtin_amdgcn_fence(__ATOMIC_ACQUIRE, "agent");
+            asm volatile("s_waitcnt vmcnt(0)" ::: "memory");
+            __hip_atomic_store(a.ticket, 0u, __ATOMIC_RELAXED, __HIP_MEMORY_SCOPE_AGENT);
+        }
+        sh[8] = last ? 1.f : 0.f;
+    }
+    __syncthreads();
+    if (sh[8] == 0.f) return;
+    float tot0, b0, tot1, b1;
+    sumsq_total(a.partial, blocks0, sh, tot0, b0);
+    __syncthreads();
+    sumsq_total(a.partial + 2 * SQ_BLOCKS, blocks1, sh, tot1, b1);
+    if (threadIdx.x != 0) return;
+    a.out2[0][0] = tot0; a.out2[0][1] = b0;
+    a.out2[1][0] = tot1; a.out2[1][1] = b1;
+    const float any = fmaxf(b0, b1);
+    a.any_overflow[0] = any;
+    const float scale = a.scale_state[0];
+    adam_hyper_set(tot0, any, scale, a.max_grad_norm[0], a.step_size[0], a.hyper[0]);
+    adam_hyper_set(tot1, any, scale, a.max_grad_norm[1], a.step_size[1], a.hyper[1]);
+}
+extern "C" int vlp_grad_norms(const vlp_grad_norms_args* a, void* stream) {
+    VLP_CHECK_ARG(a && a->partial && a->ticket && a->any_overflow && a->scale_state, "vlp_grad_norms: null operand");
+    VLP_ENTER(a->partial, "vlp_grad_norms");
+    for (int k = 0; k < 2; ++k)
+        VLP_CHECK_ARG(a->g[k] && a->out2[k] && a->hyper[k] && a->n[k] > 0 && (uintptr_t)a->g[k] % 16 == 0,
+                      "vlp_grad_norms: bad args of group %d (g 16-byte aligned, n > 0)", k);
+    const int blocks0 = sumsq_blocks(a->n[0]), blocks1 = sumsq_blocks(a->n[1]);
+    hipLaunchKernelGGL(grad_norms_kernel, dim3(blocks0 + blocks1), dim3(256), 0, (hipStream_t)stream, *a, blocks0, blocks1);
+    VLP_CHECK_LAUNCH("vlp_grad_norms");
     return VLP_OK;
 }
 
diff --git a/vlp_amd/csrc/elementwise.hip b/vlp_amd/csrc/elementwise.hip
--- a/vlp_amd/csrc/elementwise.hip
+++ b/vlp_amd/csrc/elementwise.hip
@@ -114,11 +114,11 @@
     __syncthreads();
     return n;
 }
-__global__ __launch_bounds__(256) void embed_word_partial_kernel(EwbGeom g, const f16* dpre, int H, int* rank, float* partial) {
+DEVFN void embed_word_partial(const EwbGeom& g, const f16* dpre, int H, int* rank, float* partial, int t) {
     __shared__ int list[256 + EWB_G];
     __shared__ int wcnt[4];
     __shared__ float wsum[4];
-    const int tid = threadIdx.x, t = blockIdx.x;
+    const int tid = threadIdx.x;
     const int id = g.id_of(t);
     float c = 0.f;
     for (int u = tid; u < t; u += 256) c += (g.id_of(u) == id) ? 1.f : 0.f;
@@ -156,10 +156,10 @@
         *reinterpret_cast<f32x4*>(dst + 4) = (f32x4){acc[4], acc[5], acc[6], acc[7]};
     }
 }
-__global__ __launch_bounds__(256) void embed_word_reduce_kernel(EwbGeom g, int H, const int* rank, const float* partial, f16* dword) {
+DEVFN void embed_word_reduce(const EwbGeom& g, int H, const int* rank, const float* partial, f16* dword, int t) {
     __shared__ int list[EWB_LIST + 256];
     __shared__ int wcnt[4];
-    const int tid = threadIdx.x, t = blockIdx.x;
+    const int tid = threadIdx.x;
     if (rank[t] != 0) return;
     const int id = g.id_of(t);
     const int nch = H >> 3;
@@ -190,10 +190,10 @@
         st8(dst, o);
     }
 }
-__global__ void embed_bwd_pos_kernel(const f16* dpre, f16* dpos, int B, int L, int Nv, int H) {
+DEVFN void embed_bwd_pos(const f16* dpre, f16* dpos, int B, int L, int Nv, int H, int blk, int nblk) {
     const int nch = H >> 3;
     const int64_t total = (int64_t)L * nch;
-    for (int64_t i = (int64_t)blockIdx.x * blockDim.x + threadIdx.x; i < total; i += (int64_t)gridDim.x * blockDim.x) {
+    for (int64_t i = (int64_t)blk * blockDim.x + threadIdx.x; i < total; i += (int64_t)nblk * blockDim.x) {
         const int c = (int)(i % nch);
         const int l = (int)(i / nch);
         if (l >= 1 && l <= Nv) continue;
@@ -212,12 +212,12 @@
         st8(dst, o);
     }
 }
-__global__ __launch_bounds__(256) void embed_bwd_type_kernel(const f16* dpre, const int64_t* seg, float* part, int64_t rows, int H, int T) {
+DEVFN void embed_bwd_type(const f16* dpre, const int64_t* seg, float* part, int64_t rows, int H, int T, int bx, int split, int nsplits) {
     __shared__ float red[8][256];
     const int tx = threadIdx.x & 31, ty = threadIdx.x >> 5;
-    const int c0 = blockIdx.x * 256 + tx * 8;
-    const int64_t rows_per = (rows + gridDim.y - 1) / gridDim.y;
-    const int64_t r0 = blockIdx.y * rows_per, r1 = min(rows, r0 + rows_per);
+    const int c0 = bx * 256 + tx * 8;
+    const int64_t rows_per = (rows + nsplits - 1) / nsplits;
+    const int64_t r0 = split * rows_per, r1 = min(rows, r0 + rows_per);
     float acc[EMB_MAXT][8];
 #pragma unroll
     for (int t = 0; t < EMB_MAXT; ++t)
@@ -245,26 +245,36 @@
         float s = 0.f;
 #pragma unroll
         for (int y = 0; y < 8; ++y) s += red[y][threadIdx.x];
-        const int col = blockIdx.x * 256 + threadIdx.x;
-        if (col < H && t < T) part[((int64_t)blockIdx.y * EMB_MAXT + t) * H + col] = s;
+        const int col = bx * 256 + threadIdx.x;
+        if (col < H && t < T) part[((int64_t)split * EMB_MAXT + t) * H + col] = s;
     }
 }
 __global__ void embed_bwd_type_reduce_kernel(const float* part, int nsplits, f16* dtyp, int T, int H) {
     const int i = blockIdx.x * blockDim.x + threadIdx.x;
     if (i >= T * H) return;
     const int t = i / H, c = i % H;
+    const float* src = part + (int64_t)t * H + c;
+    const int64_t slab = (int64_t)EMB_MAXT * H;
     float s = 0.f;
-    for (int p = 0; p < nsplits; ++p) s += part[((int64_t)p * EMB_MAXT + t) * H + c];
+    int p = 0;
+    for (; p + 8 <= nsplits; p += 8) {
+        float v[8];
+#pragma unroll
+        for (int k = 0; k < 8; ++k) v[k] = src[(p + k) * slab];
+#pragma unroll
+        for (int k = 0; k < 8; ++k) s += v[k];
+    }
+    for (; p < nsplits; ++p) s += src[p * slab];
     dtyp[i] = (f16)((float)dtyp[i] + s);
 }
 extern "C" int64_t vlp_embed_bwd_workspace_floats(int32_t B, int32_t L, int32_t Nv, int32_t H) {
     const int64_t nt = (int64_t)B * (L - Nv);
     return (int64_t)EMB_TSPLITS * EMB_MAXT * H + nt * H + nt;
 }
-__global__ __launch_bounds__(256) void embed_bwd_pos_ids_kernel(const f16* dpre, const int64_t* pid, f16* dpos, int B, int L, int Nv, int H, int max_pos) {
+DEVFN void embed_bwd_pos_ids(const f16* dpre, const int64_t* pid, f16* dpos, int B, int L, int Nv, int H, int max_pos, int r) {
     __shared__ int list[256];
     __shared__ int wcnt[4];
-    const int r = blockIdx.x, tid = threadIdx.x, nch = H >> 3;
+    const int tid = threadIdx.x, nch = H >> 3;
     const int NT = B * L;
     auto pred = [&](int u) {
         const int l = u % L;
@@ -294,6 +304,27 @@
 #pragma unroll
     for (int e = 0; e < 8; ++e) o[e] = (f16)((float)o[e] + acc[e]);
     st8(dst, o);
+}
+struct EmbTablesGeom {
+    EwbGeom w;
+    const f16* dpre;
+    int B, H, T, max_pos, pos_blocks, tsplits;
+    const int64_t* pid;
+    const int64_t* seg;
+    int* rank;
+    float *wpartial, *tpart;
+    f16 *dword, *dpos;
+};
+__global__ __launch_bounds__(256) void embed_tables_stage1_kernel(EmbTablesGeom a) {
+    const int b = blockIdx.x;
+    if (b >= a.pos_blocks) embed_word_partial(a.w, a.dpre, a.H, a.rank, a.wpartial, b - a.pos_blocks);
+    else if (a.pid) embed_bwd_pos_ids(a.dpre, a.pid, a.dpos, a.B, a.w.L, a.w.Nv, a.H, a.max_pos, b);
+    else embed_bwd_pos(a.dpre, a.dpos, a.B, a.w.L, a.w.Nv, a.H, b, a.pos_blocks);
+}
+__global__ __launch_bounds__(256) void embed_tables_stage2_kernel(EmbTablesGeom a) {
+    const int b = blockIdx.x, cx = (a.H + 255) / 256;
+    if (b < cx * a.tsplits) embed_bwd_type(a.dpre, a.seg, a.tpart, (int64_t)a.B * a.w.L, a.H, a.T, b % cx, b / cx, a.tsplits);
+    else embed_word_reduce(a.w, a.H, a.rank, a.wpartial, a.dword, b - cx * a.tsplits);
 }
 static int embed_bwd_run(const vlp_embed_bwd_args* a, const int64_t* position_ids, int max_pos, void* stream) {
     VLP_CHECK_ARG(a && a->dpre && a->input_ids && a->segment_ids && a->d_word_emb && a->d_pos_emb && a->d_type_emb && a->acc32, "vlp_embed_bwd: null operand");
@@ -312,31 +343,22 @@
         VLP_CHECK_LAUNCH("vlp_embed_bwd");
     }
     if (a->parts == 1) return VLP_OK;
-    {
-        EwbGeom g;
-        g.ids = a->input_ids; g.L = a->L; g.Nv = a->Nv; g.T = a->L - a->Nv; g.NT = a->B * g.T; g.vocab = a->vocab;
-        float* partial = a->acc32 + (int64_t)EMB_TSPLITS * EMB_MAXT * a->H;
-        int* rank = reinterpret_cast<int*>(partial + (int64_t)g.NT * a->H);
-        hipLaunchKernelGGL(embed_word_partial_kernel, dim3(g.NT), dim3(256), 0, s, g, (const f16*)a->dpre, a->H, rank, partial);
-        VLP_CHECK_LAUNCH("vlp_embed_word_partial");
-        hipLaunchKernelGGL(embed_word_reduce_kernel, dim3(g.NT), dim3(256), 0, s, g, a->H, (const int*)rank, (const float*)partial, (f16*)a->d_word_emb);
-        VLP_CHECK_LAUNCH("vlp_embed_word_reduce");
-    }
-    if (position_ids) {
-        hipLaunchKernelGGL(embed_bwd_pos_ids_kernel, dim3(max_pos), dim3(256), 0, s, (const f16*)a->dpre, position_ids, (f16*)a->d_pos_emb,
-                           a->B, a->L, a->Nv, a->H, max_pos);
-        VLP_CHECK_LAUNCH("vlp_embed_bwd_pos(ids)");
-    } else {
-        hipLaunchKernelGGL(embed_bwd_pos_kernel, dim3(cdiv((int64_t)a->L * (a->H / 8), 256)), dim3(256), 0, s, (const f16*)a->dpre,
-                           (f16*)a->d_pos_emb, a->B, a->L, a->Nv, a->H);
-        VLP_CHECK_LAUNCH("vlp_embed_bwd_pos");
-    }
+    EmbTablesGeom g;
+    g.w.ids = a->input_ids; g.w.L = a->L; g.w.Nv = a->Nv; g.w.T = a->L - a->Nv; g.w.NT = a->B * g.w.T; g.w.vocab = a->vocab;
+    g.dpre = (const f16*)a->dpre; g.B = a->B; g.H = a->H; g.T = a->type_vocab; g.max_pos = max_pos;
+    g.pid = position_ids; g.seg = a->segment_ids;
+    g.tpart = a->acc32;
+    g.wpartial = a->acc32 + (int64_t)EMB_TSPLITS * EMB_MAXT * a->H;
+    g.rank = reinterpret_cast<int*>(g.wpartial + (int64_t)g.w.NT * a->H);
+    g.dword = (f16*)a->d_word_emb; g.dpos = (f16*)a->d_pos_emb;
+    g.pos_blocks = position_ids ? max_pos : cdiv((int64_t)a->L * (a->H / 8), 256);
     const int64_t rows = (int64_t)a->B * a->L;
-    int splits = rows >= EMB_TSPLITS * 8 ? EMB_TSPLITS : (int)((rows + 7) / 8);
-    hipLaunchKernelGGL(embed_bwd_type_kernel, dim3(cdiv(a->H, 256), splits), dim3(256), 0, s, (const f16*)a->dpre, a->segment_ids, a->acc32,
-                       rows, a->H, a->type_vocab);
-    VLP_CHECK_LAUNCH("vlp_embed_bwd_type");
-    hipLaunchKernelGGL(embed_bwd_type_reduce_kernel, dim3(cdiv((int64_t)a->type_vocab * a->H, 256)), dim3(256), 0, s, a->acc32, splits,
+    g.tsplits = rows >= EMB_TSPLITS * 8 ? EMB_TSPLITS : (int)((rows + 7) / 8);
+    hipLaunchKernelGGL(embed_tables_stage1_kernel, dim3(g.pos_blocks + g.w.NT), dim3(256), 0, s, g);
+    VLP_CHECK_LAUNCH("vlp_embed_bwd(pos, word partial)");
+    hipLaunchKernelGGL(embed_tables_stage2_kernel, dim3(cdiv(a->H, 256) * g.tsplits + g.w.NT), dim3(256), 0, s, g);
+    VLP_CHECK_LAUNCH("vlp_embed_bwd(type, word reduce)");
+    hipLaunchKernelGGL(embed_bwd_type_reduce_kernel, dim3(cdiv((int64_t)a->type_vocab * a->H, 256)), dim3(256), 0, s, a->acc32, g.tsplits,
                        (f16*)a->d_type_emb, a->type_vocab, a->H);
     VLP_CHECK_LAUNCH("vlp_embed_bwd_type_reduce");
     return VLP_OK;
@@ -348,15 +370,45 @@
     return embed_bwd_run(&a->base, a->position_ids, a->max_pos, stream);
 }
 
-__global__ void copy2d_kernel(const void* src, int64_t lds, int src_f32, f16* dst, int64_t ldd, int rows, int cols_src, int cols_dst, int beta) {
-    const int64_t total = (int64_t)rows * cols_dst;
-    for (int64_t i = (int64_t)blockIdx.x * blockDim.x + threadIdx.x; i < total; i += (int64_t)gridDim.x * blockDim.x) {
-        const int64_t r = i / cols_dst;
-        const int c = (int)(i % cols_dst);
-        float v = 0.f;
-        if (c < cols_src) v = src_f32 ? ((const float*)src)[r * lds + c] : (float)((const f16*)src)[r * lds + c];
-        f16* d = dst + r * ldd + c;
-        *d = (f16)(beta ? (float)*d + v : v);
+template <typename T>
+DEVFN void copy2d_one(const T* s, f16* d, int c, int cols_src, int beta) {
+    const float v = c < cols_src ? (float)s[c] : 0.f;
+    d[c] = (f16)(beta ? (float)d[c] + v : v);
+}
+template <typename T>
+__global__ __launch_bounds__(256) void copy2d_kernel(const T* __restrict__ src, int64_t lds, f16* __restrict__ dst, int64_t ldd, int rows, int cols_src, int cols_dst, int beta) {
+    const int j = blockIdx.y * 256 + threadIdx.x;
+    for (int r = blockIdx.x; r < rows; r += gridDim.x) {
+        const T* s = src + (int64_t)r * lds;
+        f16* d = dst + (int64_t)r * ldd;
+        int head = (int)(((16u - (unsigned)((uintptr_t)d & 15u)) & 15u) >> 1);
+        if (head > cols_dst) head = cols_dst;
+        const int nv = (cols_dst - head) >> 3;
+        if (j < nv) {
+            const int c = head + 8 * j;
+            float v[8];
+            if (c + 8 <= cols_src) {
+                T t[8];
+                __builtin_memcpy(t, s + c, sizeof(t));
+#pragma unroll
+                for (int e = 0; e < 8; ++e) v[e] = (float)t[e];
+            } else {
+#pragma unroll
+                for (int e = 0; e < 8; ++e) v[e] = c + e < cols_src ? (float)s[c + e] : 0.f;
+            }
+            f16x8 o;
+            if (beta) {
+                const f16x8 old = ld8(d + c);
+#pragma unroll
+                for (int e = 0; e < 8; ++e) o[e] = (f16)((float)old[e] + v[e]);
+            } else {
+#pragma unroll
+                for (int e = 0; e < 8; ++e) o[e] = (f16)v[e];
+            }
+            st8(d + c, o);
+        }
+        if (blockIdx.y == 0 && (int)threadIdx.x < cols_dst - 8 * nv)
+            copy2d_one(s, d, (int)threadIdx.x < head ? (int)threadIdx.x : 8 * nv + (int)threadIdx.x, cols_src, beta);
     }
 }
 extern "C" int vlp_copy2d(const void* src, int64_t lds, int32_t src_f32, void* dst, int64_t ldd, int32_t rows, int32_t cols_src,
@@ -364,11 +416,12 @@
     VLP_CHECK_ARG(src && dst && rows > 0 && cols_src > 0 && cols_dst > 0, "vlp_copy2d: bad args");
     VLP_ENTER(src, "vlp_copy2d");
     VLP_CHECK_ARG(lds >= (cols_src < cols_dst ? cols_src : cols_dst) && ldd >= cols_dst, "vlp_copy2d: leading dims");
-    const int64_t total = (int64_t)rows * cols_dst;
-    int blocks = (int)((total + 255) / 256);
-    if (blocks > 8192) blocks = 8192;
-    hipLaunchKernelGGL(copy2d_kernel, dim3(blocks), dim3(256), 0, (hipStream_t)stream, src, lds, src_f32, (f16*)dst, ldd, rows,
-                       cols_src < cols_dst ? cols_src : cols_dst, cols_dst, beta);
+    VLP_CHECK_ARG((uintptr_t)dst % 2 == 0 && (uintptr_t)src % (src_f32 ? 4 : 2) == 0, "vlp_copy2d: operands must be element-aligned");
+    const int cs = cols_src < cols_dst ? cols_src : cols_dst;
+    const dim3 grid(rows < 16384 ? rows : 16384, (cols_dst / 8 + 255) / 256 > 0 ? (cols_dst / 8 + 255) / 256 : 1);
+    VLP_CHECK_ARG(grid.y <= 65535u, "vlp_copy2d: cols_dst=%d too wide", cols_dst);
+    if (src_f32) hipLaunchKernelGGL(copy2d_kernel<float>, grid, dim3(256), 0, (hipStream_t)stream, (const float*)src, lds, (f16*)dst, ldd, rows, cs, cols_dst, beta);
+    else hipLaunchKernelGGL(copy2d_kernel<f16>, grid, dim3(256), 0, (hipStream_t)stream, (const f16*)src, lds, (f16*)dst, ldd, rows, cs, cols_dst, beta);
     VLP_CHECK_LAUNCH("vlp_copy2d");
     return VLP_OK;
 }
diff --git a/vlp_amd/optimization_fp16.py b/vlp_amd/optimization_fp16.py
--- a/vlp_amd/optimization_fp16.py
+++ b/vlp_amd/optimization_fp16.py
@@ -81,7 +81,8 @@
         self._v = [torch.zeros_like(t) for t in self.fp32_groups_flat]
         self._sumsq = [torch.zeros(2, device=dev) for _ in self._group_key]
         self._hyper = [torch.zeros(3, device=dev) for _ in self._group_key]
-        self._partial = torch.zeros(2048, device=dev)
+        self._partial = torch.zeros(4096, device=dev)
+        self._ticket = torch.zeros(1, device=dev, dtype=torch.int32)
         self._ovf = torch.zeros(1, device=dev)
         self.dynamic_loss_scale = bool(dynamic_loss_scale)
         if dynamic_loss_scale:
@@ -191,17 +192,15 @@
             return self._step_pipelined()
         eng.wait_params()
         self._grad_norms()
-        torch.maximum(self._sumsq[0][1:2], self._sumsq[1][1:2], out=self._ovf)
-        for i, key in enumerate(self._group_key):
-            g = self.param_groups[i]
-            K.adam_hyper(self._sumsq[i], self._ovf, self._scale_state, g["max_grad_norm"], self._step_size(g), self._hyper[i])
+        for i, key in enumerate(self._group_key):
             self._adam_range(i, key, 0, eng.sizes[key])
         K.loss_scale_update(self._scale_state, self._ovf)
 
     def _grad_norms(self):
         eng = self.engine
-        for i, key in enumerate(self._group_key):
-            K.sumsq(eng.gflat[key], eng.sizes[key], self._sumsq[i], self._partial)
+        gs = self.param_groups
+        K.grad_norms([eng.gflat[k] for k in self._group_key], [eng.sizes[k] for k in self._group_key], self._sumsq, self._hyper,
+                     [g["max_grad_norm"] for g in gs], [self._step_size(g) for g in gs], self._partial, self._ticket, self._ovf, self._scale_state)
 
     def _step_size(self, g):
         if g["bias_correction"]:
@@ -226,10 +225,6 @@
         events = {}
         with torch.cuda.stream(st):
             self._grad_norms()
-            torch.maximum(self._sumsq[0][1:2], self._sumsq[1][1:2], out=self._ovf)
-            for i, key in enumerate(self._group_key):
-                g = self.param_groups[i]
-                K.adam_hyper(self._sumsq[i], self._ovf, self._scale_state, g["max_grad_norm"], self._step_size(g), self._hyper[i])
             i_nd, i_d = self._group_key.index("nodecay"), self._group_key.index("decay")
             self._adam_range(i_nd, "nodecay", 0, eng.sizes["nodecay"])
             ev = torch.cuda.Event()
```

Result: no change. 6862 samples/s (median of 6 runs) (+0.3%).
